# dwani-ai/tts-indic-server-f5

Hardware: AMD Instinct MI355X
Metric: mel-frames/sec + RTF, F5-TTS-Base 32-NFE, 10s utterance (higher is better)
Workload: dtype fp16/bf16 MFMA, fp32 accumulate

## Files before the change

include/f5hip.h:

```cpp
#ifndef F5HIP_H
#define F5HIP_H

#include <stdint.h>

#ifdef __cplusplus
extern "C" {
#endif

#define F5HIP_ABI_VERSION 1

int f5hip_abi_version(void);
const char* f5hip_last_error(void);


typedef struct f5hip_dit_config {
    int32_t dim, depth, heads, ff_mult, text_dim, conv_layers, mel_dim, text_num_embeds;
    int32_t gemm_planes;
    int32_t arch;
} f5hip_dit_config;

typedef struct f5hip_dit f5hip_dit;

f5hip_dit* f5hip_dit_create(const f5hip_dit_config* cfg);
void f5hip_dit_destroy(f5hip_dit* m);

int f5hip_dit_load_param(f5hip_dit* m, const char* name, const float* data, int64_t numel);
int f5hip_dit_finalize(f5hip_dit* m);

int f5hip_dit_forward(f5hip_dit* m, int32_t n_seq, const int32_t* seq_len, const int32_t* kv_len,
                      const float* x_dev, const float* cond_dev, const int32_t* text, int32_t nt_max, float time,
                      const uint8_t* drop_audio_cond, const uint8_t* drop_text, int32_t n_blocks,
                      float* out_dev, float* h_out_dev, void* stream);

int f5hip_dit_read_tap(f5hip_dit* m, const char* tap, float* dst_dev, int64_t numel, void* stream);

int f5hip_cfm_sample(f5hip_dit* m, int32_t n_utt, const int32_t* dur, const float* cond_dev,
                     const uint8_t* cond_mask, const int32_t* text, int32_t nt_max, const float* y0_dev,
                     const float* t_grid, int32_t steps, float cfg_strength, float* out_dev, void* stream);

int f5hip_cfm_sample_masked(f5hip_dit* m, int32_t n_utt, const int32_t* dur, const int32_t* kv_len, const float* cond_dev,
                            const uint8_t* cond_mask, const int32_t* text, int32_t nt_max, const float* y0_dev,
                            const float* t_grid, int32_t steps, float cfg_strength, float* out_dev, void* stream);

int f5hip_cfm_sample_units(f5hip_dit* m, int32_t n_utt, const int32_t* dur, const int32_t* kv_len, const float* cond_dev,
                           const uint8_t* cond_mask, const int32_t* text, int32_t nt_max, const float* y0_dev,
                           const float* t_grid, int32_t steps, const float* cfg_strength, float* out_dev, void* stream);

int f5hip_cfm_sample_grids(f5hip_dit* m, int32_t n_utt, const int32_t* dur, const int32_t* kv_len, const float* cond_dev,
                           const uint8_t* cond_mask, const int32_t* text, int32_t nt_max, const float* y0_dev,
                           const int32_t* steps, const float* t_grids, const float* cfg_strength, float* out_dev, void* stream);

int f5hip_cfm_sample_span(f5hip_dit* m, int32_t n_utt, const int32_t* dur, const int32_t* kv_len, const float* cond_dev,
                          const uint8_t* cond_mask, const int32_t* text, int32_t nt_max, const float* y0_dev,
                          const int32_t* steps, const float* t_grids, const float* cfg_strength, const uint8_t* last,
                          float* out_dev, void* stream);

int f5hip_cfm_sample_methods(f5hip_dit* m, int32_t n_utt, const int32_t* dur, const int32_t* kv_len, const float* cond_dev,
                             const uint8_t* cond_mask, const int32_t* text, int32_t nt_max, const float* y0_dev,
                             const int32_t* steps, const float* t_grids, const float* cfg_strength,
                             const int32_t* method ,
                             const uint8_t* last ,
                             float* out_dev, void* stream);

int f5hip_dit_set_ode_method(f5hip_dit* m, int32_t method);

int f5hip_set_attention_shape_invariant(int32_t on);
int f5hip_dit_set_attention_shape_invariant(f5hip_dit* m, int32_t on);
int f5hip_dit_set_profiling(f5hip_dit* m, int32_t enabled);
int f5hip_dit_get_profile(f5hip_dit* m, const char* kernel_class, double* total_ms, int64_t* launches);
int f5hip_set_profiling(int32_t enabled);
int f5hip_get_profile(const char* kernel_class, double* total_ms, int64_t* launches);
int f5hip_get_counter(const char* name, int64_t* value);

int f5hip_op_gemm(int32_t M, int32_t N, int32_t K, const float* a_dev, const float* w_dev, const float* bias_dev, int32_t prec,
                  int32_t act, const float* mul_dev, const float* res_dev, const uint8_t* row_keep_host, float* out_dev,
                  uint16_t* out16_dev, int32_t w_copies, int32_t iters, double* avg_us, void* stream, int32_t bn);
int f5hip_op_gemm_rowmul(int32_t M, int32_t N, int32_t K, const float* a_dev, const float* w_dev, const float* bias_dev, int32_t prec,
                         const float* mul_dev, const int32_t* row_mod_host, int32_t mod_ld, int32_t n_mod_rows, const float* res_dev,
                         const uint8_t* row_keep_host, float* out_dev, void* stream, int32_t bn);
int f5hip_op_qkv(int32_t M, int32_t D, const float* a_dev, const float* w_dev, const float* bias_dev, const int32_t* row_pos,
                 int32_t prec, uint16_t* qk_dev, uint16_t* vt_dev, int32_t iters, double* avg_us, void* stream);
int f5hip_op_attention(int32_t n_seq, const int32_t* seq_len, const int32_t* kv_len, int32_t heads, const float* q_dev, const float* k_dev,
                       const float* v_dev, float* out_dev, int32_t impl, int32_t iters, double* avg_us, void* stream, int32_t shape_invariant,
                       int32_t out_format);
int f5hip_op_joint_attention(int32_t n_seq, const int32_t* x_len, const int32_t* x_kvlen, const int32_t* c_len, int32_t heads,
                             const float* q_dev, const float* k_dev, const float* v_dev, float* out_dev, void* stream, int32_t shape_invariant,
                             int32_t out_format);
int f5hip_op_layernorm(int32_t M, int32_t D, const float* x_dev, const float* scale_dev, const float* shift_dev, float gain_off, float eps,
                       int32_t rms, float* out_dev, void* stream);
int f5hip_op_layernorm_planes(int32_t M, int32_t D, const float* x_dev, const float* scale_dev, const float* shift_dev,
                              const int32_t* row_mod_host, int32_t mod_ld, int32_t n_mod_rows, float gain_off, float eps, int32_t out_format,
                              float* out_dev, void* stream);
int f5hip_op_cfg_step(int32_t method, int32_t stage, int32_t U, int32_t mel, int32_t rows, float* xout_dev, float* xbase_dev,
                      const float* pred_dev, const int32_t* urow_c_host, const int32_t* urow_u_host, float cfg, const float* cfg_frame_dev,
                      float dt, const int32_t* frame_unit_host, const float* unit_dt_host, int32_t n_units, int32_t n_act, float* k1_dev,
                      float* k2_dev, float* k3_dev, float* xs_dev, const uint8_t* final_flags_host, const float* cond_dev, float* out_dev,
                      void* stream);
int f5hip_op_cfg_mixed(int32_t U, int32_t mel, int32_t rows, float* xstate_dev, const float* pred_dev, const int32_t* urow_c_host,
                       const int32_t* urow_u_host, const float* cfg_frame_dev, const int32_t* frame_unit_host, const int32_t* unit_op_host,
                       const float* unit_dt_host, int32_t n_units, int32_t n_act, float* k1_dev, float* k2_dev, float* k3_dev, float* xs_dev,
                       void* stream);
int f5hip_op_row_tp(int32_t R, const int32_t* row_unit_host, int32_t n_units, const int32_t* unit_tp_host, int32_t* row_tp_host,
                    void* stream);
int f5hip_op_time_table(f5hip_dit* m, const float* t_host, int32_t n_t, float* sinus_dev, float* mod_dev, int32_t mod_cols, float* temb_dev,
                        void* stream);
int f5hip_op_conv1d(int32_t batch, int32_t P, int32_t T, int32_t c_in, int32_t c_out, int32_t k, int32_t dil, const float* x_dev,
                    const float* w_host, const float* bias_host, const float* res_dev, float* out_dev, int32_t prec, int32_t impl,
                    int32_t iters, double* avg_us, uint64_t* stamps_host, int32_t stamp_blocks, void* stream);
int f5hip_op_bigvgan_snake(int32_t batch, int32_t P, int32_t T, int32_t C, const float* x_dev, const float* alpha_log_dev,
                           const float* beta_log_dev, int32_t out_format, float* out_dev, int64_t out_rows, void* stream);
int f5hip_op_bigvgan_upsample(int32_t batch, int32_t P, int32_t T, int32_t c_in, int32_t c_out, int32_t r, const float* x_dev,
                              const float* w_host, const float* bias_host, float* out_dev, int32_t prec, void* stream);
int f5hip_op_bigvgan_conv_post(int32_t batch, int32_t P, int32_t T, int32_t C, const float* a_dev, const float* w_dev, int32_t variant,
                               float* wave_dev, void* stream);
int f5hip_op_conv1d_ragged(int32_t n_items, const int32_t* item_row0, const int32_t* item_rows, const int32_t* item_valid, int32_t M,
                           int32_t blk, int32_t c_in, int32_t c_out, int32_t k, int32_t dil, int32_t ups_rate, const float* x_dev,
                           const float* w_host, const float* bias_host, const float* res_dev, float* out_dev, int32_t prec, int32_t impl,
                           void* stream);
int f5hip_op_bigvgan_snake_ragged(int32_t n_items, const int32_t* item_row0, const int32_t* item_valid, int32_t scale, int32_t M, int32_t C,
                                  const float* x_dev, const float* alpha_log_dev, const float* beta_log_dev, int32_t out_format,
                                  float* out_dev, int64_t out_rows, void* stream);
int f5hip_op_bigvgan_conv_post_ragged(int32_t n_items, const int32_t* item_row0, const int32_t* item_valid, const int32_t* item_wave_off,
                                      int32_t scale, int32_t M, int32_t C, const float* a_dev, const float* w_dev, int32_t variant,
                                      float* wave_dev, int64_t wave_len, void* stream);
int f5hip_op_bigvgan_mean3(int64_t rows, int32_t C, int32_t n_in, const float* y0_dev, const float* y1_dev, const float* y2_dev, int32_t mode,
                           int32_t ldo, float* out_f32_dev, float* planes_dev, void* stream);
int f5hip_op_bigvgan_mel_rows(int32_t n, const int32_t* item_row0, const int32_t* item_frames, int32_t T, int32_t M0, int32_t C,
                              const float* mel_dev, int32_t f16, float* out_dev, void* stream);
int f5hip_op_conv_pos_embed(int32_t n_seq, const int32_t* seq_len, int32_t lead, int32_t D, const float* x_dev, const float* w1_host,
                            const float* b1_host, const float* w2_host, const float* b2_host, int32_t impl, int32_t prec, int32_t pad_nan,
                            float* out_dev, float* c1_dev, void* stream);
int f5hip_op_convnext_block(int32_t n_seq, const int32_t* seq_len, int32_t Td, const float* x_dev, const float* const* params_host,
                            int32_t pad_nan, float* out_dev, float* tap_ln_dev, float* tap_ty_dev, float* tap_grn_dev, void* stream);


typedef struct f5hip_vocos_config {
    int32_t in_channels, dim, intermediate_dim, num_layers, n_fft, hop_length;
    int32_t gemm_planes;
} f5hip_vocos_config;
typedef struct f5hip_vocos f5hip_vocos;

f5hip_vocos* f5hip_vocos_create(const f5hip_vocos_config* cfg);
void f5hip_vocos_destroy(f5hip_vocos* v);
int f5hip_vocos_load_param(f5hip_vocos* v, const char* name, const float* data, int64_t numel);
int f5hip_vocos_finalize(f5hip_vocos* v);
int f5hip_vocos_decode(f5hip_vocos* v, int32_t batch, int32_t frames, const float* mel_dev, float* wave_dev,
                       void* stream);
int f5hip_vocos_decode_ragged(f5hip_vocos* v, int32_t n, const int32_t* frames, const float* mel_dev, float* wave_dev,
                              void* stream);
int f5hip_vocos_decode_taps(f5hip_vocos* v, int32_t n, const int32_t* frames, const float* mel_dev, int32_t n_blocks,
                            float* x_dev, float* y_dev, float* fw_dev, float* wave_dev, void* stream);


typedef struct f5hip_bigvgan_config {
    int32_t num_mels, num_upsamples;
    int32_t upsample_rates[8], upsample_kernel_sizes[8];
    int32_t upsample_initial_channel;
    int32_t resblock_kernel_sizes[3];
    int32_t resblock_dilations[9];
    int32_t gemm_planes;
} f5hip_bigvgan_config;
typedef struct f5hip_bigvgan f5hip_bigvgan;

f5hip_bigvgan* f5hip_bigvgan_create(const f5hip_bigvgan_config* cfg);
void f5hip_bigvgan_destroy(f5hip_bigvgan* v);
int f5hip_bigvgan_load_param(f5hip_bigvgan* v, const char* name, const float* data, int64_t numel);
int f5hip_bigvgan_finalize(f5hip_bigvgan* v);
int f5hip_bigvgan_forward(f5hip_bigvgan* v, int32_t batch, int32_t frames, const float* mel_dev, float* wave_dev, void* stream);
int f5hip_bigvgan_forward_ragged(f5hip_bigvgan* v, int32_t n, const int32_t* frames, const float* mel_dev, float* wave_dev,
                                 void* stream);


int f5hip_mel_spectrogram(int32_t batch, int32_t n_samples, const float* wave_dev, float* mel_dev, int32_t n_fft,
                          int32_t hop_length, int32_t n_mels, int32_t sample_rate, void* stream);

int f5hip_mel_spectrogram_bigvgan(int32_t batch, int32_t n_samples, const float* wave_dev, float* mel_dev, int32_t n_fft,
                                  int32_t hop_length, int32_t n_mels, int32_t sample_rate, void* stream);

int f5hip_mel_spectrogram_ragged(int32_t n, const int32_t* n_samples, const float* const* wave_dev, float* mel_dev, int32_t n_fft, int32_t hop_length,
                                 int32_t n_mels, int32_t sample_rate, int32_t variant, void* stream);


int f5hip_ref_frontend(int32_t n, const int32_t* n_in, const int32_t* channels, const float* wave_dev, int32_t orig_freq, int32_t new_freq,
                       const float* taps_dev, float rms_floor, float* out_dev, float* rms_dev, void* stream);


int f5hip_wave_finish(int32_t n, const int32_t* chunks_per_request, const float* const* chunk_dev, const int32_t* chunk_len, int32_t fade,
                      const uint8_t* remove_silence, int32_t sample_rate, int16_t* pcm_dev, int32_t* len_dev, void* stream);

int f5hip_wave_finish_joins(int32_t n, const int32_t* chunks_per_request, const float* const* chunk_dev, const int32_t* chunk_len, int32_t fade,
                            const uint8_t* chunk_fade, const uint8_t* remove_silence, int32_t sample_rate, int16_t* pcm_dev, int32_t* len_dev,
                            void* stream);

int f5hip_wave_encode(int32_t n, const int16_t* pcm_dev, const int64_t* in_off, const int32_t* max_len, const int32_t* len_dev, int32_t new_freq,
                      int32_t encoding, const float* taps_dev, uint8_t* out_dev, const int64_t* out_off, int32_t* out_len_dev, void* stream);

int f5hip_wave_encode_tile(int32_t new_freq);

int f5hip_wave_flac(int32_t n, const int16_t* pcm_dev, const int64_t* in_off, const int32_t* max_len, const int32_t* len_dev, int32_t sample_rate,
                    uint8_t* out_dev, const int64_t* out_off, int32_t* out_len_dev, void* stream);

int f5hip_wave_flac_levels(int32_t n, const int16_t* pcm_dev, const int64_t* in_off, const int32_t* max_len, const int32_t* len_dev,
                           int32_t sample_rate, const int32_t* level, uint8_t* out_dev, const int64_t* out_off, int32_t* out_len_dev, void* stream);

int64_t f5hip_wave_flac_bound(int32_t max_len);

int f5hip_wave_loudness(int32_t n, int16_t* pcm_dev, const int64_t* in_off, const int32_t* max_len, const int32_t* len_dev, const double* gain_k,
                        int64_t* stats_dev, void* stream);

int f5hip_wave_loudness_tile(void);

int f5hip_wave_prosody(int32_t n, const int16_t* pcm_dev, const int64_t* in_off, const int32_t* max_len, const int32_t* len_dev,
                       const int32_t* stretch_p, const int32_t* stretch_q, const int32_t* pitch, const float* taps_dev, int16_t* out_dev,
                       const int64_t* out_off, int32_t* out_len_dev, void* stream);

int64_t f5hip_wave_prosody_tap_offset(int32_t pitch);

int f5hip_flac_decode(int32_t n, const uint8_t* data_dev, int64_t nbytes, const int64_t* begin, const int64_t* end, const int32_t* info,
                      const int64_t* total, const int64_t* max_samples, int32_t* out_dev, const int64_t* out_off, int32_t* status_dev, void* stream);

int64_t f5hip_flac_decode_bound(int64_t total, int64_t stream_bytes, int64_t max_samples);

int f5hip_ref_prestep(int32_t n, const int32_t* n_in, const int32_t* channels, const uint8_t* clip_short, const int16_t* frames_dev, int64_t n_samples,
                      int32_t rate, float* out_dev, int32_t* info_dev, void* stream);

int64_t f5hip_ref_prestep_bound(int32_t n, const int32_t* n_in, const int32_t* channels, int32_t rate);

int f5hip_ref_denoise(int32_t n, const int64_t* offset, const int32_t* n_samples, float* wave_dev, void* stream);

int f5hip_wave_mark(int32_t n, int16_t* pcm_dev, const int64_t* in_off, const int32_t* max_len, const int32_t* len_dev, const int32_t* key_index,
                    const int16_t* carriers_dev, int32_t n_keys, void* stream);

int f5hip_wave_mark_tile(void);

int f5hip_watermark_carrier(uint64_t key, int16_t* carrier);

int f5hip_watermark_detect(int32_t n, const float* wave_dev, const int64_t* offset, const int32_t* n_samples, int32_t n_keys,
                           const int16_t* carriers_dev, float* scores_dev, void* stream);

int f5hip_watermark_detect_launches(void);

int f5hip_ref_assess(int32_t n, const float* raw_dev, const int64_t* raw_offset, const int32_t* channels, const int32_t* raw_len,
                     const float* wave_dev, const int64_t* offset, const int32_t* n_samples, int64_t* rows_dev, void* stream);

int f5hip_ref_assess_launches(void);

#ifdef __cplusplus
}
#endif
#endif
```

tts-indic-server-f5_amd/_lib.py:

```python
from __future__ import annotations

import ctypes as C
import os

HERE = os.path.dirname(os.path.abspath(__file__))
LIB_PATH = os.environ.get("F5HIP_LIB") or os.path.join(HERE, "csrc", "libf5hip.so")

_lib = None


class DitConfig(C.Structure):
    _fields_ = [(n, C.c_int32) for n in ("dim", "depth", "heads", "ff_mult", "text_dim", "conv_layers", "mel_dim",
                                          "text_num_embeds", "gemm_planes", "arch")]


class VocosConfig(C.Structure):
    _fields_ = [(n, C.c_int32) for n in ("in_channels", "dim", "intermediate_dim", "num_layers", "n_fft", "hop_length",
                                          "gemm_planes")]


class BigVGANConfig(C.Structure):
    _fields_ = [("num_mels", C.c_int32), ("num_upsamples", C.c_int32), ("upsample_rates", C.c_int32 * 8),
                ("upsample_kernel_sizes", C.c_int32 * 8), ("upsample_initial_channel", C.c_int32),
                ("resblock_kernel_sizes", C.c_int32 * 3), ("resblock_dilations", C.c_int32 * 9), ("gemm_planes", C.c_int32)]


SYMBOLS = {
    "f5hip_abi_version": (C.c_int, []),
    "f5hip_last_error": (C.c_char_p, []),
    "f5hip_dit_create": (C.c_void_p, [C.POINTER(DitConfig)]),
    "f5hip_dit_destroy": (None, [C.c_void_p]),
    "f5hip_dit_load_param": (C.c_int, [C.c_void_p, C.c_char_p, C.c_void_p, C.c_int64]),
    "f5hip_dit_finalize": (C.c_int, [C.c_void_p]),
    "f5hip_dit_forward": (C.c_int, [C.c_void_p, C.c_int32, C.c_void_p, C.c_void_p, C.c_void_p, C.c_void_p, C.c_void_p,
                                    C.c_int32, C.c_float, C.c_void_p, C.c_void_p, C.c_int32, C.c_void_p, C.c_void_p,
                                    C.c_void_p]),
    "f5hip_dit_read_tap": (C.c_int, [C.c_void_p, C.c_char_p, C.c_void_p, C.c_int64, C.c_void_p]),
    "f5hip_cfm_sample": (C.c_int, [C.c_void_p, C.c_int32, C.c_void_p, C.c_void_p, C.c_void_p, C.c_void_p, C.c_int32,
                                   C.c_void_p, C.c_void_p, C.c_int32, C.c_float, C.c_void_p, C.c_void_p]),
    "f5hip_cfm_sample_masked": (C.c_int, [C.c_void_p, C.c_int32, C.c_void_p, C.c_void_p, C.c_void_p, C.c_void_p, C.c_void_p, C.c_int32,
                                          C.c_void_p, C.c_void_p, C.c_int32, C.c_float, C.c_void_p, C.c_void_p]),
    "f5hip_cfm_sample_units": (C.c_int, [C.c_void_p, C.c_int32, C.c_void_p, C.c_void_p, C.c_void_p, C.c_void_p, C.c_void_p, C.c_int32,
                                         C.c_void_p, C.c_void_p, C.c_int32, C.c_void_p, C.c_void_p, C.c_void_p]),
    "f5hip_cfm_sample_grids": (C.c_int, [C.c_void_p, C.c_int32, C.c_void_p, C.c_void_p, C.c_void_p, C.c_void_p, C.c_void_p, C.c_int32,
                                         C.c_void_p, C.c_void_p, C.c_void_p, C.c_void_p, C.c_void_p, C.c_void_p]),
    "f5hip_cfm_sample_span": (C.c_int, [C.c_void_p, C.c_int32, C.c_void_p, C.c_void_p, C.c_void_p, C.c_void_p, C.c_void_p, C.c_int32,
                                        C.c_void_p, C.c_void_p, C.c_void_p, C.c_void_p, C.c_void_p, C.c_void_p, C.c_void_p]),
    "f5hip_cfm_sample_methods": (C.c_int, [C.c_void_p, C.c_int32, C.c_void_p, C.c_void_p, C.c_void_p, C.c_void_p, C.c_void_p, C.c_int32,
                                           C.c_void_p, C.c_void_p, C.c_void_p, C.c_void_p, C.c_void_p, C.c_void_p, C.c_void_p, C.c_void_p]),
    "f5hip_dit_set_ode_method": (C.c_int, [C.c_void_p, C.c_int32]),
    "f5hip_dit_set_attention_shape_invariant": (C.c_int, [C.c_void_p, C.c_int32]),
    "f5hip_dit_set_profiling": (C.c_int, [C.c_void_p, C.c_int32]),
    "f5hip_dit_get_profile": (C.c_int, [C.c_void_p, C.c_char_p, C.POINTER(C.c_double), C.POINTER(C.c_int64)]),
    "f5hip_set_profiling": (C.c_int, [C.c_int32]),
    "f5hip_set_attention_shape_invariant": (C.c_int, [C.c_int32]),
    "f5hip_get_profile": (C.c_int, [C.c_char_p, C.POINTER(C.c_double), C.POINTER(C.c_int64)]),
    "f5hip_get_counter": (C.c_int, [C.c_char_p, C.POINTER(C.c_int64)]),
    "f5hip_op_gemm": (C.c_int, [C.c_int32, C.c_int32, C.c_int32, C.c_void_p, C.c_void_p, C.c_void_p, C.c_int32, C.c_int32, C.c_void_p, C.c_void_p,
                                C.c_void_p, C.c_void_p, C.c_void_p, C.c_int32, C.c_int32, C.POINTER(C.c_double), C.c_void_p, C.c_int32]),
    "f5hip_op_qkv": (C.c_int, [C.c_int32, C.c_int32, C.c_void_p, C.c_void_p, C.c_void_p, C.c_void_p, C.c_int32, C.c_void_p, C.c_void_p, C.c_int32,
                               C.POINTER(C.c_double), C.c_void_p]),
    "f5hip_op_attention": (C.c_int, [C.c_int32, C.c_void_p, C.c_void_p, C.c_int32, C.c_void_p, C.c_void_p, C.c_void_p, C.c_void_p, C.c_int32, C.c_int32,
                                     C.POINTER(C.c_double), C.c_void_p, C.c_int32, C.c_int32]),
    "f5hip_op_layernorm": (C.c_int, [C.c_int32, C.c_int32, C.c_void_p, C.c_void_p, C.c_void_p, C.c_float, C.c_float, C.c_int32, C.c_void_p, C.c_void_p]),
    "f5hip_op_gemm_rowmul": (C.c_int, [C.c_int32] * 3 + [C.c_void_p] * 3 + [C.c_int32, C.c_void_p, C.c_void_p, C.c_int32, C.c_int32] + [C.c_void_p] * 4 +
                             [C.c_int32]),
    "f5hip_op_layernorm_planes": (C.c_int, [C.c_int32, C.c_int32] + [C.c_void_p] * 4 + [C.c_int32, C.c_int32, C.c_float, C.c_float, C.c_int32, C.c_void_p,
                                            C.c_void_p]),
    "f5hip_op_cfg_step": (C.c_int, [C.c_int32] * 5 + [C.c_void_p] * 5 + [C.c_float, C.c_void_p, C.c_float, C.c_void_p, C.c_void_p, C.c_int32, C.c_int32] +
                          [C.c_void_p] * 8),
    "f5hip_op_cfg_mixed": (C.c_int, [C.c_int32] * 3 + [C.c_void_p] * 8 + [C.c_int32, C.c_int32] + [C.c_void_p] * 5),
    "f5hip_op_row_tp": (C.c_int, [C.c_int32, C.c_void_p, C.c_int32, C.c_void_p, C.c_void_p, C.c_void_p]),
    "f5hip_op_time_table": (C.c_int, [C.c_void_p, C.c_void_p, C.c_int32, C.c_void_p, C.c_void_p, C.c_int32, C.c_void_p, C.c_void_p]),
    "f5hip_op_joint_attention": (C.c_int, [C.c_int32, C.c_void_p, C.c_void_p, C.c_void_p, C.c_int32, C.c_void_p, C.c_void_p, C.c_void_p, C.c_void_p, C.c_void_p,
                                           C.c_int32, C.c_int32]),
    "f5hip_op_conv1d": (C.c_int, [C.c_int32] * 7 + [C.c_void_p] * 5 + [C.c_int32] * 3 + [C.c_void_p, C.c_void_p, C.c_int32, C.c_void_p]),
    "f5hip_op_bigvgan_snake": (C.c_int, [C.c_int32] * 4 + [C.c_void_p] * 3 + [C.c_int32, C.c_void_p, C.c_int64, C.c_void_p]),
    "f5hip_op_bigvgan_upsample": (C.c_int, [C.c_int32] * 6 + [C.c_void_p] * 4 + [C.c_int32, C.c_void_p]),
    "f5hip_op_bigvgan_conv_post": (C.c_int, [C.c_int32] * 4 + [C.c_void_p] * 2 + [C.c_int32, C.c_void_p, C.c_void_p]),
    "f5hip_op_conv1d_ragged": (C.c_int, [C.c_int32] + [C.c_void_p] * 3 + [C.c_int32] * 7 + [C.c_void_p] * 5 + [C.c_int32, C.c_int32, C.c_void_p]),
    "f5hip_op_bigvgan_snake_ragged": (C.c_int, [C.c_int32, C.c_void_p, C.c_void_p] + [C.c_int32] * 3 + [C.c_void_p] * 3 +
                                      [C.c_int32, C.c_void_p, C.c_int64, C.c_void_p]),
    "f5hip_op_bigvgan_conv_post_ragged": (C.c_int, [C.c_int32] + [C.c_void_p] * 3 + [C.c_int32] * 3 + [C.c_void_p] * 2 +
                                          [C.c_int32, C.c_void_p, C.c_int64, C.c_void_p]),
    "f5hip_op_bigvgan_mean3": (C.c_int, [C.c_int64, C.c_int32, C.c_int32] + [C.c_void_p] * 3 + [C.c_int32, C.c_int32] + [C.c_void_p] * 3),
    "f5hip_op_bigvgan_mel_rows": (C.c_int, [C.c_int32, C.c_void_p, C.c_void_p] + [C.c_int32] * 3 + [C.c_void_p, C.c_int32, C.c_void_p, C.c_void_p]),
    "f5hip_op_conv_pos_embed": (C.c_int, [C.c_int32, C.c_void_p, C.c_int32, C.c_int32] + [C.c_void_p] * 5 + [C.c_int32] * 3 + [C.c_void_p] * 3),
    "f5hip_op_convnext_block": (C.c_int, [C.c_int32, C.c_void_p, C.c_int32, C.c_void_p, C.c_void_p, C.c_int32] + [C.c_void_p] * 5),
    "f5hip_vocos_create": (C.c_void_p, [C.POINTER(VocosConfig)]),
    "f5hip_vocos_destroy": (None, [C.c_void_p]),
    "f5hip_vocos_load_param": (C.c_int, [C.c_void_p, C.c_char_p, C.c_void_p, C.c_int64]),
    "f5hip_vocos_finalize": (C.c_int, [C.c_void_p]),
    "f5hip_vocos_decode": (C.c_int, [C.c_void_p, C.c_int32, C.c_int32, C.c_void_p, C.c_void_p, C.c_void_p]),
    "f5hip_vocos_decode_ragged": (C.c_int, [C.c_void_p, C.c_int32, C.c_void_p, C.c_void_p, C.c_void_p, C.c_void_p]),
    "f5hip_vocos_decode_taps": (C.c_int, [C.c_void_p, C.c_int32, C.c_void_p, C.c_void_p, C.c_int32] + [C.c_void_p] * 5),
    "f5hip_bigvgan_create": (C.c_void_p, [C.POINTER(BigVGANConfig)]),
    "f5hip_bigvgan_destroy": (None, [C.c_void_p]),
    "f5hip_bigvgan_load_param": (C.c_int, [C.c_void_p, C.c_char_p, C.c_void_p, C.c_int64]),
    "f5hip_bigvgan_finalize": (C.c_int, [C.c_void_p]),
    "f5hip_bigvgan_forward": (C.c_int, [C.c_void_p, C.c_int32, C.c_int32, C.c_void_p, C.c_void_p, C.c_void_p]),
    "f5hip_bigvgan_forward_ragged": (C.c_int, [C.c_void_p, C.c_int32, C.c_void_p, C.c_void_p, C.c_void_p, C.c_void_p]),
    "f5hip_mel_spectrogram_bigvgan": (C.c_int, [C.c_int32, C.c_int32, C.c_void_p, C.c_void_p, C.c_int32, C.c_int32, C.c_int32,
                                                C.c_int32, C.c_void_p]),
    "f5hip_mel_spectrogram_ragged": (C.c_int, [C.c_int32, C.c_void_p, C.c_void_p, C.c_void_p, C.c_int32, C.c_int32, C.c_int32, C.c_int32, C.c_int32,
                                               C.c_void_p]),
    "f5hip_mel_spectrogram": (C.c_int, [C.c_int32, C.c_int32, C.c_void_p, C.c_void_p, C.c_int32, C.c_int32, C.c_int32,
                                        C.c_int32, C.c_void_p]),
    "f5hip_ref_frontend": (C.c_int, [C.c_int32, C.c_void_p, C.c_void_p, C.c_void_p, C.c_int32, C.c_int32, C.c_void_p, C.c_float, C.c_void_p, C.c_void_p,
                                     C.c_void_p]),
    "f5hip_wave_finish": (C.c_int, [C.c_int32, C.c_void_p, C.c_void_p, C.c_void_p, C.c_int32, C.c_void_p, C.c_int32, C.c_void_p, C.c_void_p, C.c_void_p]),
    "f5hip_wave_finish_joins": (C.c_int, [C.c_int32, C.c_void_p, C.c_void_p, C.c_void_p, C.c_int32, C.c_void_p, C.c_void_p, C.c_int32, C.c_void_p, C.c_void_p,
                                          C.c_void_p]),
    "f5hip_wave_encode": (C.c_int, [C.c_int32, C.c_void_p, C.c_void_p, C.c_void_p, C.c_void_p, C.c_int32, C.c_int32, C.c_void_p, C.c_void_p, C.c_void_p,
                                    C.c_void_p, C.c_void_p]),
    "f5hip_wave_encode_tile": (C.c_int, [C.c_int32]),
    "f5hip_wave_flac": (C.c_int, [C.c_int32, C.c_void_p, C.c_void_p, C.c_void_p, C.c_void_p, C.c_int32, C.c_void_p, C.c_void_p, C.c_void_p, C.c_void_p]),
    "f5hip_wave_flac_levels": (C.c_int, [C.c_int32, C.c_void_p, C.c_void_p, C.c_void_p, C.c_void_p, C.c_int32, C.c_void_p, C.c_void_p, C.c_void_p, C.c_void_p,
                                         C.c_void_p]),
    "f5hip_wave_flac_bound": (C.c_int64, [C.c_int32]),
    "f5hip_wave_loudness": (C.c_int, [C.c_int32, C.c_void_p, C.c_void_p, C.c_void_p, C.c_void_p, C.c_void_p, C.c_void_p, C.c_void_p]),
    "f5hip_wave_loudness_tile": (C.c_int, []),
    "f5hip_wave_prosody": (C.c_int, [C.c_int32] + [C.c_void_p] * 12),
    "f5hip_wave_prosody_tap_offset": (C.c_int64, [C.c_int32]),
    "f5hip_flac_decode": (C.c_int, [C.c_int32, C.c_void_p, C.c_int64] + [C.c_void_p] * 9),
    "f5hip_flac_decode_bound": (C.c_int64, [C.c_int64, C.c_int64, C.c_int64]),
    "f5hip_ref_prestep": (C.c_int, [C.c_int32, C.c_void_p, C.c_void_p, C.c_void_p, C.c_void_p, C.c_int64, C.c_int32, C.c_void_p, C.c_void_p, C.c_void_p]),
    "f5hip_ref_prestep_bound": (C.c_int64, [C.c_int32, C.c_void_p, C.c_void_p, C.c_int32]),
    "f5hip_ref_denoise": (C.c_int, [C.c_int32, C.c_void_p, C.c_void_p, C.c_void_p, C.c_void_p]),
    "f5hip_wave_mark": (C.c_int, [C.c_int32, C.c_void_p, C.c_void_p, C.c_void_p, C.c_void_p, C.c_void_p, C.c_void_p, C.c_int32, C.c_void_p]),
    "f5hip_wave_mark_tile": (C.c_int, []),
    "f5hip_watermark_carrier": (C.c_int, [C.c_uint64, C.c_void_p]),
    "f5hip_watermark_detect": (C.c_int, [C.c_int32, C.c_void_p, C.c_void_p, C.c_void_p, C.c_int32, C.c_void_p, C.c_void_p, C.c_void_p]),
    "f5hip_watermark_detect_launches": (C.c_int, []),
    "f5hip_ref_assess": (C.c_int, [C.c_int32, C.c_void_p, C.c_void_p, C.c_void_p, C.c_void_p, C.c_void_p, C.c_void_p, C.c_void_p, C.c_void_p, C.c_void_p]),
    "f5hip_ref_assess_launches": (C.c_int, []),
}


class F5HipError(RuntimeError):
    pass


def lib():
    global _lib
    if _lib is None:
        if not os.path.exists(LIB_PATH):
            raise F5HipError(f"{LIB_PATH} is missing: run `python -c 'import __graft_entry__ as g; g.build()'` "
                             "(this package has no CPU fallback)")
        import torch
        l = C.CDLL(LIB_PATH)
        for name, (res, args) in SYMBOLS.items():
            fn = getattr(l, name)
            fn.restype = res
            fn.argtypes = args
        if l.f5hip_abi_version() != 1:
            raise F5HipError("libf5hip ABI version mismatch")
        _lib = l
    return _lib


def check(rc: int, what: str):
    if rc != 0:
        raise F5HipError(f"{what} failed ({rc}): {lib().f5hip_last_error().decode(errors='replace')}")


def current_stream_ptr():
    import torch
    return C.c_void_p(torch.cuda.current_stream().cuda_stream)
```

tts-indic-server-f5_amd/csrc/cfm_sample.h:

```cpp
#pragma once

struct OdeRule { const char* name; int forwards, points; };
static const OdeRule kOdeRules[3] = {{"euler", 1, 1}, {"midpoint", 2, 2}, {"rk4", 4, 3}};

static void stage_times(int method, float t0, float t1, float t[4]) {
#pragma clang fp contract(off)
    const float dt = t1 - t0;
    t[0] = t0;
    if (method == 1) t[1] = t0 + 0.5f * dt;
    if (method == 2) { t[1] = t0 + dt * (1.0f / 3.0f); t[2] = t0 + dt * (2.0f / 3.0f); t[3] = t1; }
}

struct SampleArgs {
    int32_t n_utt; const int32_t *dur, *kv_len; const float* cond_dev; const uint8_t* cond_mask; const int32_t* text; int32_t nt_max;
    const float* y0_dev; float* out_dev; void* stream;
    const uint8_t* last = nullptr;
    bool ok() const { return n_utt > 0 && dur && cond_dev && cond_mask && text && y0_dev && out_dev; }
};

struct UnitLayout {
    std::vector<SeqDesc> seqs;
    std::vector<float> frame_cfg;
    std::vector<int> frame_unit;
    std::vector<uint8_t> frame_final;
// ... 34 lines not shown
            L.seq_unit.push_back(k);
            m->h_seq_len.push_back(a.dur[u]);
        }
        L.seq_end[k] = (int)L.seqs.size();
    }
    return 0;
}

struct TimePlan {
    int forwards = 0, cols = 1;
    std::vector<float> pts, dt;
    std::vector<int> tp, op;
};

static int unit_forwards(const int32_t* steps, const int32_t* method, int u) { return steps[u] * kOdeRules[method[u]].forwards; }

static int plan_times(const std::vector<int>& order, const int32_t* steps, const int32_t* method, const float* t_grid, bool per_unit, TimePlan& P) {
    static const int kFirstOp[3] = {CFG_OP_EULER, CFG_OP_MID_HALF, CFG_OP_RK4_1};
    const int n = (int)order.size();
    bool mixed = false;
    for (int u = 0; u < n; u++) mixed = mixed || method[u] != method[0];
    if (!per_unit) {
        const OdeRule& rule = kOdeRules[method[0]];
        const int end_pt = rule.forwards > rule.points ? 1 : 0;
        if ((long long)steps[0] * rule.points + end_pt > kMaxGridPoints) {
            if (method[0] == 0) return fail(-8, "at most %d time points per call (got %d)", kMaxGridPoints, steps[0]);
            return fail(-8, "%s: at most %d steps per call (got %d)", rule.name, (kMaxGridPoints - end_pt) / rule.points, steps[0]);
        }
    }
    std::map<uint32_t, int> pt_index;
    auto point = [&](float v) {
        uint32_t bits;
        memcpy(&bits, &v, sizeof(bits));
        auto it = pt_index.find(bits);
        if (it != pt_index.end()) return it->second;
        pt_index[bits] = (int)P.pts.size();
        P.pts.push_back(v);
        return (int)P.pts.size() - 1;
    };
    P.cols = per_unit ? n : 1;
    P.forwards = unit_forwards(steps, method, order[0]);
    const size_t cells = (size_t)P.forwards * P.cols;
    P.tp.assign(cells, 0);
    P.op.assign(cells, CFG_OP_NONE);
    P.dt.assign(cells, 0.0f);
    std::vector<size_t> grid0(n, 0);
    for (int u = 1; per_unit && u < n; u++) grid0[u] = grid0[u - 1] + (size_t)steps[u - 1] + 1;
    float t[4];
    for (int k = 0; k < P.cols; k++) {
        const int u = order[k], mu = method[u];
        const OdeRule& rule = kOdeRules[mu];
        const float* tg = t_grid + grid0[u];
        for (int i = 0; i < steps[u]; i++) {
            const float dt = tg[i + 1] - tg[i];
            stage_times(mu, tg[i], tg[i + 1], t);
            for (int s = 0; s < rule.forwards; s++) {
                const size_t at = ((size_t)i * rule.forwards + s) * P.cols + k;
                if (per_unit) P.tp[at] = point(t[s]);
                else {
                    if (s < rule.points) P.pts.push_back(t[s]);
                    P.tp[at] = i * rule.points + s;
                }
                P.op[at] = kFirstOp[mu] + s;
                P.dt[at] = mu == 1 && s == 0 ? 0.5f * dt : dt;
            }
        }
        if (!per_unit && rule.forwards > rule.points) P.pts.push_back(tg[steps[u]]);
    }
    if ((int)P.pts.size() > kMaxTimePoints)
        return fail(-8, "%s: the units' grids need %d distinct time points, at most %d per call", mixed ? "cfm_sample_methods" : "cfm_sample_grids",
                    (int)P.pts.size(), kMaxTimePoints);
    return 0;
}

struct GridLayout {
    size_t row_unit, frame_unit, tp, op, dt, row_tp, total = 0;
    GridLayout(size_t R, size_t U, size_t cells) {
        auto take = [&](size_t n) { const size_t at = total; total += n; return at; };
        row_unit = take(R); frame_unit = take(U); tp = take(cells); op = take(cells); dt = take(cells); row_tp = take(R);
    }
};
struct GridTables { const int *row_unit = nullptr, *frame_unit = nullptr, *tp = nullptr, *op = nullptr; const float* dt = nullptr; int* row_tp = nullptr; };

static int upload_grid_tables(f5hip_dit* m, const UnitLayout& L, const TimePlan& P, hipStream_t st, GridTables& T) {
    const int R = m->Rtot, S = (int)L.seqs.size();
    const GridLayout g(R, L.n_frames, P.tp.size());
    if (g.total > m->grid_cap) {
        dev_free(m->grid_meta);
        m->grid_cap = 0;
        if (hipMalloc((void**)&m->grid_meta, sizeof(int) * g.total) != hipSuccess) { m->grid_meta = nullptr; return fail(-5, "hipMalloc grid tables"); }
        m->grid_cap = g.total;
    }
    std::vector<int> hb(g.row_tp, 0);
    for (int s = 0; s < S; s++) {
        for (int r = m->h_seq_row0[s]; r < m->h_seq_row0[s + 1]; r++) hb[g.row_unit + r] = L.seq_unit[s];
        for (int r = m->h_seqc_row0[s]; r < m->h_seqc_row0[s + 1]; r++) hb[g.row_unit + r] = L.seq_unit[s];
    }
    memcpy(&hb[g.frame_unit], L.frame_unit.data(), sizeof(int) * L.frame_unit.size());
    memcpy(&hb[g.tp], P.tp.data(), sizeof(int) * P.tp.size());
    memcpy(&hb[g.op], P.op.data(), sizeof(int) * P.op.size());
    memcpy(&hb[g.dt], P.dt.data(), sizeof(float) * P.dt.size());
    CK(m->up_grid.upload(m->grid_meta, hb.data(), sizeof(int) * hb.size(), st));
    int* const d = m->grid_meta;
    T = {d + g.row_unit, d + g.frame_unit, d + g.tp, d + g.op, reinterpret_cast<const float*>(d + g.dt), d + g.row_tp};
    return 0;
}

struct CfgBufs {
    float *xstate, *k1, *k2, *k3;
    const float* pred;
    const int *urow_c, *urow_u;
    const float* frame_cfg;
    Plane2 xs;
    int mel;
};
static CfgBufs cfg_bufs(const f5hip_dit* m) {
    return {m->xstate, m->xmid, m->rk_k2, m->rk_k3, m->pred, m->d_urow_c, m->d_urow_u, m->d_frame_cfg, m->xs, m->cfg.mel_dim};
}

static void launch_cfg_step(const CfgBufs& b, int f0, int op, float dt, const int* frame_unit, const int* unit_op, const float* unit_dt, int n_act,
                            hipStream_t st) {
    auto* kernel = frame_unit ? cfg_step_kernel<true> : cfg_step_kernel<false>;
    hipLaunchKernelGGL(kernel, dim3(f0), dim3(128), 0, st, b.xstate, b.mel, f0, b.pred, 128, b.urow_c, b.urow_u, b.frame_cfg, op, dt, b.k1, b.k2, b.k3,
                       b.xs.hi, b.xs.lo, 128, frame_unit, unit_op, unit_dt, n_act);
}

struct GridScope {
    f5hip_dit* m;
    ~GridScope() { m->d_row_tp = nullptr; m->M = m->row_c0; m->Mc = m->Rtot - m->row_c0; m->n_seq = (int)m->h_seq_row0.size() - 1; }
};

static int run_sampler(f5hip_dit* m, const SampleArgs& a, const int32_t* steps, const int32_t* method, const float* t_grid, bool per_unit,
                       float cfg_strength, const float* cfg_unit) {
    const int n = a.n_utt;
    std::vector<int> order(n);
    for (int u = 0; u < n; u++) order[u] = u;
    std::stable_sort(order.begin(), order.end(), [&](int x, int y) { return unit_forwards(steps, method, x) > unit_forwards(steps, method, y); });
    ProfScope prof_scope(m->prof);
    hipStream_t st = (hipStream_t)a.stream;
    UnitLayout L;
    TimePlan P;
    CK(layout_units(m, a, order, cfg_strength, cfg_unit, L));
    CK(plan_times(order, steps, method, t_grid, per_unit, P));
    const int mel = m->cfg.mel_dim, U = L.n_frames;
    CK(setup_sequences(m, L.seqs, U, a.text, a.nt_max, a.cond_mask, st, L.frame_cfg.data(), a.last ? L.frame_final.data() : nullptr));
    GridScope scope{m};
    GridTables T;
    if (per_unit) CK(upload_grid_tables(m, L, P, st, T));

    if (hipMemcpyAsync(m->xstate, a.y0_dev, sizeof(float) * (size_t)U * mel, hipMemcpyDeviceToDevice, st) != hipSuccess) return fail(-6, "y0 copy");
    hipLaunchKernelGGL(split_rows_kernel, dim3(m->M), dim3(256), 0, st, m->xstate, mel, mel, m->M, m->d_row_frame, m->xs.hi, m->xs.lo, 128, 0);
    CKL("split x");
    CK(precompute_text_and_ce(m, a.cond_dev, st));
    CK(precompute_time(m, P.pts.data(), (int)P.pts.size(), st));

    m->d_row_tp = T.row_tp;
    int n_act = n;
    for (int f = 0; f < P.forwards; f++) {
        const size_t at = (size_t)f * P.cols;
        if (per_unit) {
            while (P.op[at + n_act - 1] == CFG_OP_NONE) n_act--;
            const int s_act = L.seq_end[n_act - 1];
            m->M = m->h_seq_row0[s_act]; m->Mc = m->h_seqc_row0[s_act] - m->row_c0; m->n_seq = s_act;
            prof_begin(PROF_OTHER, st);
            hipLaunchKernelGGL(row_tp_kernel, dim3((m->Rtot + 255) / 256), dim3(256), 0, st, T.row_unit, T.tp + at, m->Rtot, T.row_tp);
            prof_end(PROF_OTHER, st);
            CKL("row_tp");
        }
        CK(forward_step(m, per_unit ? 0 : P.tp[at], -1, st));
        prof_begin(PROF_OTHER, st);
        launch_cfg_step(cfg_bufs(m), U, P.op[at], P.dt[at], T.frame_unit, per_unit ? T.op + at : nullptr, per_unit ? T.dt + at : nullptr, n_act, st);
        prof_end(PROF_OTHER, st);
        CKL("cfg step");
    }
    hipLaunchKernelGGL(final_select_kernel, dim3(U), dim3(128), 0, st, m->xstate, a.cond_dev, m->d_frame_is_cond, mel, U, a.out_dev);
    CKL("final_select");
    return 0;
}

static int sample_one_grid(f5hip_dit* m, const SampleArgs& a, int method, const float* t_grid, int32_t steps, float cfg_strength, const float* cfg_unit) {
    if (!m || !m->finalized) return fail(-1, "model not finalized");
    if (!a.ok() || !t_grid || steps <= 0) return fail(-1, "cfm_sample: bad argument");
    const std::vector<int32_t> unit_steps(a.n_utt, steps), unit_method(a.n_utt, method);
    return run_sampler(m, a, unit_steps.data(), unit_method.data(), t_grid, false, cfg_strength, cfg_unit);
}

int f5hip_cfm_sample(f5hip_dit* m, int32_t n_utt, const int32_t* dur, const float* cond_dev, const uint8_t* cond_mask,
                     const int32_t* text, int32_t nt_max, const float* y0_dev, const float* t_grid, int32_t steps,
                     float cfg_strength, float* out_dev, void* stream) {
    return sample_one_grid(m, {n_utt, dur, nullptr, cond_dev, cond_mask, text, nt_max, y0_dev, out_dev, stream}, m ? m->ode_method : 0, t_grid, steps, cfg_strength, nullptr);
}

int f5hip_cfm_sample_masked(f5hip_dit* m, int32_t n_utt, const int32_t* dur, const int32_t* kv_len, const float* cond_dev, const uint8_t* cond_mask,
                            const int32_t* text, int32_t nt_max, const float* y0_dev, const float* t_grid, int32_t steps,
                            float cfg_strength, float* out_dev, void* stream) {
    return sample_one_grid(m, {n_utt, dur, kv_len, cond_dev, cond_mask, text, nt_max, y0_dev, out_dev, stream}, m ? m->ode_method : 0, t_grid, steps, cfg_strength, nullptr);
}

int f5hip_cfm_sample_units(f5hip_dit* m, int32_t n_utt, const int32_t* dur, const int32_t* kv_len, const float* cond_dev, const uint8_t* cond_mask,
                           const int32_t* text, int32_t nt_max, const float* y0_dev, const float* t_grid, int32_t steps,
                           const float* cfg_strength, float* out_dev, void* stream) {
    if (!cfg_strength) return fail(-1, "cfm_sample_units: cfg_strength is null");
    return sample_one_grid(m, {n_utt, dur, kv_len, cond_dev, cond_mask, text, nt_max, y0_dev, out_dev, stream}, m ? m->ode_method : 0, t_grid, steps, 0.0f, cfg_strength);
}

static int sample_grids(const char* name, f5hip_dit* m, const SampleArgs& a, const int32_t* steps, const float* t_grids, const float* cfg_strength,
                        const int32_t* unit_method) {
    if (!m || !m->finalized) return fail(-1, "model not finalized");
    if (!a.ok() || !steps || !t_grids || !cfg_strength) return fail(-1, "%s: bad argument", name);
    const std::vector<int32_t> handle_method(a.n_utt, m->ode_method);
    const int32_t* method = unit_method ? unit_method : handle_method.data();
    bool one = true;
    size_t g0 = 0;
    for (int u = 0; u < a.n_utt; u++) {
        if (method[u] < 0 || method[u] > 2) return fail(-1, "%s: method[%d] = %d (0 euler, 1 midpoint, 2 rk4)", name, u, method[u]);
        one = one && method[u] == method[0];
    }
    for (int u = 0; u < a.n_utt; u++) {
        if (steps[u] < 1) return fail(-1, "%s: steps[%d] = %d (need >= 1)", name, u, steps[u]);
        one = one && steps[u] == steps[0] && !memcmp(t_grids + g0, t_grids, sizeof(float) * ((size_t)steps[0] + 1));
        g0 += (size_t)steps[u] + 1;
    }
    if (one) return sample_one_grid(m, a, method[0], t_grids, steps[0], 0.0f, cfg_strength);
    return run_sampler(m, a, steps, method, t_grids, true, 0.0f, cfg_strength);
}

int f5hip_cfm_sample_grids(f5hip_dit* m, int32_t n_utt, const int32_t* dur, const int32_t* kv_len, const float* cond_dev, const uint8_t* cond_mask,
                           const int32_t* text, int32_t nt_max, const float* y0_dev, const int32_t* steps, const float* t_grids,
                           const float* cfg_strength, float* out_dev, void* stream) {
    return sample_grids("cfm_sample_grids", m, {n_utt, dur, kv_len, cond_dev, cond_mask, text, nt_max, y0_dev, out_dev, stream}, steps, t_grids, cfg_strength, nullptr);
}

int f5hip_cfm_sample_span(f5hip_dit* m, int32_t n_utt, const int32_t* dur, const int32_t* kv_len, const float* cond_dev, const uint8_t* cond_mask,
                          const int32_t* text, int32_t nt_max, const float* y0_dev, const int32_t* steps, const float* t_grids,
                          const float* cfg_strength, const uint8_t* last, float* out_dev, void* stream) {
    if (!last) return fail(-1, "cfm_sample_span: last is null");
    return sample_grids("cfm_sample_span", m, {n_utt, dur, kv_len, cond_dev, cond_mask, text, nt_max, y0_dev, out_dev, stream, last}, steps, t_grids, cfg_strength, nullptr);
}

int f5hip_cfm_sample_methods(f5hip_dit* m, int32_t n_utt, const int32_t* dur, const int32_t* kv_len, const float* cond_dev, const uint8_t* cond_mask,
                             const int32_t* text, int32_t nt_max, const float* y0_dev, const int32_t* steps, const float* t_grids,
                             const float* cfg_strength, const int32_t* method, const uint8_t* last, float* out_dev, void* stream) {
    if (!method) return fail(-1, "cfm_sample_methods: method is null");
    return sample_grids("cfm_sample_methods", m, {n_utt, dur, kv_len, cond_dev, cond_mask, text, nt_max, y0_dev, out_dev, stream, last}, steps, t_grids,
                        cfg_strength, method);
}
```

tts-indic-server-f5_amd/csrc/elementwise.h:

```cpp
#pragma once
#include "common.h"

#include "ln_row.h"

template <int NV, bool ROW_MOD = false>
__global__ __launch_bounds__(256) void ln_kernel(const LnArgs p) {
    unsigned b = blockIdx.x;
    if ((gridDim.x & 7) == 0) b = (b & 7) * (gridDim.x >> 3) + (b >> 3);
    ln_row<NV, ROW_MOD>(p, b * 4 + (threadIdx.x >> 6), threadIdx.x & 63);
}

__global__ __launch_bounds__(256) void row_tp_kernel(const int* row_unit, const int* unit_tp, int R, int* row_tp) {
    const int r = blockIdx.x * 256 + threadIdx.x;
    if (r < R) row_tp[r] = unit_tp[row_unit[r]];
}

__global__ __launch_bounds__(256) void rope_rows_kernel(const int* row_pos, const float* rope_cos, const float* rope_sin, int R, int max_pos, float* out_cos, float* out_sin) {
    const int i = blockIdx.x * 256 + threadIdx.x;
    if (i >= R * 32) return;
    const int r = i >> 5, j = i & 31;
    const int pos = min(max(row_pos[r], 0), max_pos - 1);
    out_cos[i] = rope_cos[pos * 32 + j];
    out_sin[i] = rope_sin[pos * 32 + j];
}

__global__ __launch_bounds__(256) void grn_stats_kernel(const float* y, int ldy, int C, const int* seq_row0,
                                                        const int* seq_len, float* gx ) {
    const int seq = blockIdx.y, c = blockIdx.x * 256 + threadIdx.x;
    if (c >= C) return;
    const int r0 = seq_row0[seq], n = seq_len[seq];
    float a8[8] = {0.f, 0.f, 0.f, 0.f, 0.f, 0.f, 0.f, 0.f};
    const float* col = y + (size_t)r0 * ldy + c;
    int r = 0;
    for (; r + 8 <= n; r += 8) {
        float t[8];
#pragma unroll
        for (int u = 0; u < 8; u++) t[u] = col[(size_t)(r + u) * ldy];
#pragma unroll
        for (int u = 0; u < 8; u++) a8[u] += t[u] * t[u];
    }
    for (; r < n; r++) {
        const float t = col[(size_t)r * ldy];
        a8[0] += t * t;
    }
    const float acc = ((a8[0] + a8[1]) + (a8[2] + a8[3])) + ((a8[4] + a8[5]) + (a8[6] + a8[7]));
    gx[(size_t)seq * C + c] = sqrtf(acc);
}

__global__ __launch_bounds__(256) void grn_apply_kernel(const float* y, int ldy, int C, int M, const int* row_seq,
                                                        const float* gx, const float* gamma, const float* beta,
                                                        __bf16* out_hi, __bf16* out_lo, int ldo) {
    const int lane = threadIdx.x & 63;
    const int row = blockIdx.x * 4 + (threadIdx.x >> 6);
    if (row >= M) return;
    const int seq = row_seq[row];
    if (seq < 0) return;
    const float* g = gx + (size_t)seq * C;
    float s = 0.0f;
    for (int c = lane; c < C; c += 64) s += g[c];
    const float denom = wave_sum(s) / (float)C + 1e-6f;
    for (int c = lane * 4; c < C; c += 256) {
        const float4 yv = *reinterpret_cast<const float4*>(y + (size_t)row * ldy + c);
        const float yy[4] = {yv.x, yv.y, yv.z, yv.w};
        bf16x4 hi, lo;
        float ov[4];
#pragma unroll
        for (int e = 0; e < 4; e++) {
            const float nx = g[c + e] / denom;
            ov[e] = gamma[c + e] * (yy[e] * nx) + beta[c + e] + yy[e];
        }
        split_bf16x4(ov, hi, lo);
        *reinterpret_cast<bf16x4*>(out_hi + (size_t)row * ldo + c) = hi;
        if (out_lo) *reinterpret_cast<bf16x4*>(out_lo + (size_t)row * ldo + c) = lo;
    }
}

__global__ __launch_bounds__(256) void text_gather_kernel(const float* emb, const float* pos_table, int C, int M,
                                                          const int* row_token, const int* row_pos, int add_pos,
                                                          float* out, int ldo, int max_pos) {
    const int row = blockIdx.x;
    if (row >= M) return;
    const int tok = row_token[row];
    if (tok < 0) return;
    const int pos = min(row_pos[row], max_pos);
    for (int c = threadIdx.x; c < C; c += 256) {
        float v = emb[(size_t)tok * C + c];
        if (add_pos) v += pos_table[(size_t)pos * C + c];
        out[(size_t)row * ldo + c] = v;
    }
}

__global__ __launch_bounds__(256) void split_rows_kernel(const float* x, int ldx, int C, int M, const int* row_src,
                                                         __bf16* out_hi, __bf16* out_lo, int ldo, int col0) {
    const int row = blockIdx.x;
    if (row >= M) return;
    const int src = row_src ? row_src[row] : row;
    for (int c = threadIdx.x; c < C; c += 256) {
        __bf16 hi, lo;
        const float v = src >= 0 ? x[(size_t)src * ldx + c] : 0.0f;
        split_bf16(v, hi, lo);
        out_hi[(size_t)row * ldo + col0 + c] = hi;
        if (out_lo) out_lo[(size_t)row * ldo + col0 + c] = lo;
    }
}

enum CfgOp : int {
    CFG_OP_NONE = 0,
    CFG_OP_EULER = 1,
    CFG_OP_MID_HALF = 2,
    CFG_OP_MID_FULL = 3,
    CFG_OP_RK4_1 = 4,
    CFG_OP_COUNT = 8
};

__device__ __forceinline__ float cfg_velocity(const float* pred, int ldp, int rc, int ru, int c, float cfg) {
    const float pc = pred[(size_t)rc * ldp + c];
    float v = pc;
    if (ru >= 0) v = pc + (pc - pred[(size_t)ru * ldp + c]) * cfg;
    return v;
}

__device__ __forceinline__ float euler_update(float* xout, const float* xbase, size_t i, float dt, float v) {
    const float xn = xbase[i] + dt * v;
    xout[i] = xn;
    return xn;
}

__device__ __forceinline__ float rk4_stage_update(float* xstate, float* k1, float* k2, float* k3, size_t i, int stage, float dt, float v) {
    const float y0 = xstate[i];
    float xn;
    if (stage == 1) {
        k1[i] = v;
        xn = y0 + dt * v * (1.0f / 3.0f);
    } else if (stage == 2) {
        k2[i] = v;
        xn = y0 + dt * (v - k1[i] * (1.0f / 3.0f));
    } else if (stage == 3) {
        k3[i] = v;
        xn = y0 + dt * (k1[i] - k2[i] + v);
    } else {
        xn = y0 + (k1[i] + 3.0f * (k2[i] + k3[i]) + v) * dt * 0.125f;
        xstate[i] = xn;
    }
    return xn;
}

__device__ __forceinline__ void store_x_split(__bf16* xs_hi, __bf16* xs_lo, int ldx, int rc, int ru, int c, float xn) {
    __bf16 hi, lo;
    split_bf16(xn, hi, lo);
    xs_hi[(size_t)rc * ldx + c] = hi;
    xs_lo[(size_t)rc * ldx + c] = lo;
    if (ru >= 0) {
        xs_hi[(size_t)ru * ldx + c] = hi;
        xs_lo[(size_t)ru * ldx + c] = lo;
    }
}

template <bool kPerUnit>
__global__ __launch_bounds__(128) void cfg_step_kernel(float* xstate , int mel, int U, const float* pred, int ldp, const int* urow_c,
                                                       const int* urow_u, const float* cfg_frame, int op, float dt, float* k1, float* k2, float* k3,
                                                       __bf16* xs_hi, __bf16* xs_lo, int ldx, const int* frame_unit, const int* unit_op,
                                                       const float* unit_dt, int n_act) {
    const int u = blockIdx.x;
    if (u >= U) return;
    const int c = threadIdx.x;
    if (c >= mel) return;
    if (kPerUnit) {
        const int un = frame_unit[u];
        if (un >= n_act) return;
        op = unit_op[un];
        dt = unit_dt[un];
    }
    if (op <= CFG_OP_NONE || op >= CFG_OP_COUNT) return;
    const int rc = urow_c[u], ru = urow_u[u];
    const float v = cfg_velocity(pred, ldp, rc, ru, c, cfg_frame[u]);
    const size_t i = (size_t)u * mel + c;
    float xn;
    if (op >= CFG_OP_RK4_1) xn = rk4_stage_update(xstate, k1, k2, k3, i, op - CFG_OP_RK4_1 + 1, dt, v);
    else xn = euler_update(op == CFG_OP_MID_HALF ? k1 : xstate, xstate, i, dt, v);
    store_x_split(xs_hi, xs_lo, ldx, rc, ru, c, xn);
}

__global__ __launch_bounds__(128) void final_select_kernel(const float* xstate, const float* cond, const int* frame_is_cond,
                                                           int mel, int U, float* out) {
    const int u = blockIdx.x, c = threadIdx.x;
    if (u >= U || c >= mel) return;
    out[(size_t)u * mel + c] = frame_is_cond[u] ? cond[(size_t)u * mel + c] : xstate[(size_t)u * mel + c];
}

__global__ __launch_bounds__(256) void pack_weight_kernel(const float* w, int R, int C, int ldw, __bf16* hi, __bf16* lo,
                                                          int C_pad) {
    const int r = blockIdx.x;
    for (int c = threadIdx.x; c < C_pad; c += 256) {
        float v = (r < R && c < C) ? w[(size_t)r * ldw + c] : 0.0f;
        if (!lo) {
            reinterpret_cast<_Float16*>(hi)[(size_t)r * C_pad + c] = sat_f16(v);
            continue;
        }
        __bf16 h, l;
// ... 37 lines not shown
```

tts-indic-server-f5_amd/csrc/f5hip.hip:

```cpp
#include "../../include/f5hip.h"

#include <math.h>
#include <stdio.h>
#include <stdlib.h>
#include <string.h>

#include <map>
#include <string>
#include <algorithm>
#include <vector>

#include "common.h"
#include "elementwise.h"
#include "gemm_launch.h"
#include "host_util.h"

static constexpr int kMaxTimePoints = 256;
static constexpr int kMaxGridPoints = 128;
static_assert(kMaxGridPoints <= kMaxTimePoints, "a one-grid call's points are rows of the same tables");


struct TextBlock {
    float *dw_w = nullptr, *dw_b = nullptr, *ln_w = nullptr, *ln_b = nullptr, *gamma = nullptr, *beta = nullptr;
    PackedW pw1, pw2;
};

struct BlockWeights {
    std::vector<PackedW> qkv, out, ff1, ff2;
    void resize(int n) { qkv.resize(n); out.resize(n); ff1.resize(n); ff2.resize(n); }
};

struct f5hip_dit {
    f5hip_dit_config cfg;
    int nsplit = 2;
    int attn_invariant = -1;
    ProfState* prof = nullptr;
    HostStage up_meta, up_time[2], up_grid;
    bool blk_f16 = false;
    ParamStore params;
    bool finalized = false;
    PackedW time1, time2, adaln, wx, wct, conv1, conv2, proj_out;
    BlockWeights blk;
    BlockWeights blk_c;
    std::vector<PackedW> wskip;
    std::vector<int> mod_c, mod_x;
    int mod_final = 0;
    std::vector<float*> g_attn, g_ff;
    float *g_out = nullptr, *zeros = nullptr;
    std::vector<TextBlock> tblk;
    float *text_emb = nullptr, *text_pos = nullptr, *rope_cos = nullptr, *rope_sin = nullptr;
    float *rope_row_cos = nullptr, *rope_row_sin = nullptr;
    int rope_max_pos = 0;
    int arch = 0;
    int td_pad = 0;
    int gw = 0;
    int n_adaln = 0;
    int cap_rows = 0, cap_frames = 0, cap_seq = 0;
    DevBuf ws;
    float *h = nullptr, *h0 = nullptr, *ce = nullptr, *pred = nullptr, *te = nullptr, *ty = nullptr, *gx = nullptr,
          *mod = nullptr, *xstate = nullptr, *xmid = nullptr, *temb = nullptr, *rk_k2 = nullptr, *rk_k3 = nullptr;
    int ode_method = 0;
    std::vector<Plane2> skipbuf;
    Plane2 hn, c1, ao, ff, xs, tn, tg, act, sinp, t1, st;
    __bf16 *qk = nullptr, *vt = nullptr;
    int *meta = nullptr;
    int meta_cap = 0;
    int *d_row_pos, *d_row_start, *d_row_end, *d_row_seq, *d_row_token, *d_row_frame, *d_row_condframe, *d_row_keep,
        *d_seq_row0, *d_seq_len, *d_seq_kvlen, *d_urow_c, *d_urow_u, *d_frame_is_cond;
    float* d_frame_cfg = nullptr;
    int M = 0, n_seq = 0, n_frames = 0, max_len = 0;
    int Mc = 0, Rtot = 0;
    int row_c0 = 0;
    std::vector<int> h_seq_row0, h_seqc_row0;
    int* d_row_tp = nullptr;
    int* grid_meta = nullptr;
    size_t grid_cap = 0;
    int *d_j_row0 = nullptr, *d_j_len = nullptr, *d_j_kvlen = nullptr, *d_j_kv_row0 = nullptr, *d_j_kv2_row0 = nullptr, *d_j_kv2_len = nullptr;
    bool any_masked = false;
    std::vector<int> h_seq_len;
};

static int ceil_to(int v, int m) { return (v + m - 1) / m * m; }

f5hip_dit* f5hip_dit_create(const f5hip_dit_config* cfg) {
    if (!cfg) { set_error("null config"); return nullptr; }
    if (cfg->dim % 128 || cfg->dim != cfg->heads * 64 || cfg->dim % 16 || cfg->text_dim % 4 || cfg->mel_dim > 128 || cfg->mel_dim % 4 ||
        cfg->dim / 16 > 64 || cfg->gemm_planes < 1 || cfg->gemm_planes > 3 || cfg->arch < 0 || cfg->arch > 2 ||
        (cfg->arch == 1 && (cfg->conv_layers != 0 || cfg->depth % 2)) || (cfg->conv_layers > 0 && cfg->text_dim % 32) ||
        (cfg->arch == 2 && (cfg->conv_layers != 0 || cfg->text_dim != cfg->dim || cfg->depth < 1))) {
        set_error("unsupported backbone geometry (need dim %% 128 == 0, dim == 64*heads, dim/16 <= 64, mel_dim <= 128, text conv needs text_dim %% 32 == 0; UNetT: even depth, no text conv)");
        return nullptr;
    }
    int dev_count = 0;
    if (hipGetDeviceCount(&dev_count) != hipSuccess || dev_count == 0) {
        set_error("no HIP device: libf5hip has no CPU fallback");
        return nullptr;
    }
    f5hip_dit* m = new f5hip_dit();
    m->cfg = *cfg;
    m->nsplit = cfg->gemm_planes == 3 ? 2 : cfg->gemm_planes;
    m->blk_f16 = cfg->gemm_planes == 3;
    m->arch = cfg->arch;
    m->td_pad = cfg->arch == 2 ? 0 : ceil_to(cfg->text_dim, 32);
    m->gw = cfg->dim / 16;
    if (cfg->arch != 1) {
        int off = 0;
        for (int l = 0; l < cfg->depth; l++) {
            if (cfg->arch == 2) { m->mod_c.push_back(off); off += (l == cfg->depth - 1 ? 2 : 6) * cfg->dim; }
            m->mod_x.push_back(off); off += 6 * cfg->dim;
        }
        m->mod_final = off;
        m->n_adaln = off + 2 * cfg->dim;
    }
    return m;
}

static void free_packed(PackedW& w) { dev_free(w.hi); dev_free(w.lo); dev_free(w.bias); dev_free(w.frag); w = PackedW(); }

void f5hip_dit_destroy(f5hip_dit* m) {
    if (!m) return;
    for (PackedW* w : {&m->time1, &m->time2, &m->adaln, &m->wx, &m->wct, &m->conv1, &m->conv2, &m->proj_out}) free_packed(*w);
    for (BlockWeights* b : {&m->blk, &m->blk_c})
        for (auto* v : {&b->qkv, &b->out, &b->ff1, &b->ff2}) for (auto& w : *v) free_packed(w);
    for (auto& w : m->wskip) free_packed(w);
    for (auto* v : {&m->g_attn, &m->g_ff}) for (float* g : *v) dev_free(g);
    dev_free(m->g_out); dev_free(m->zeros);
    for (auto& b : m->tblk) {
        for (float* p : {b.dw_w, b.dw_b, b.ln_w, b.ln_b, b.gamma, b.beta}) dev_free(p);
        free_packed(b.pw1); free_packed(b.pw2);
    }
    for (float* p : {m->text_emb, m->text_pos, m->rope_cos, m->rope_sin}) dev_free(p);
    dev_free(m->ws.ptr);
    dev_free(m->meta);
    delete m->prof;
    dev_free(m->grid_meta);
    m->up_meta.release(); m->up_time[0].release(); m->up_time[1].release(); m->up_grid.release();
    delete m;
}

int f5hip_dit_load_param(f5hip_dit* m, const char* name, const float* data, int64_t numel) {
    return m ? m->params.load(m->finalized, name, data, numel) : fail(-1, "load_param: bad argument");
}

#define CK(x) do { int _r = (x); if (_r) return _r; } while (0)
#define CKL(name) do { hipError_t _e = hipGetLastError(); if (_e != hipSuccess) return fail(-7, "%s launch: %s", name, hipGetErrorString(_e)); } while (0)

static int pack_conv_pos(PackedW& out, const float* w, const float* b, int D) {
    const int gw = D / 16, K = 31 * 64;
    std::vector<float> wp((size_t)16 * 64 * K, 0.0f), bp(16 * 64, 0.0f);
    for (int g = 0; g < 16; g++)
        for (int co = 0; co < gw; co++) {
            bp[g * 64 + co] = b[g * gw + co];
            for (int ci = 0; ci < gw; ci++)
                for (int tap = 0; tap < 31; tap++)
                    wp[((size_t)(g * 64 + co)) * K + tap * 64 + ci] = w[((size_t)(g * gw + co) * gw + ci) * 31 + tap];
        }
    return pack_linear(out, wp.data(), 16 * 64, K, K, bp.data());
}

static int pack_block(f5hip_dit* m, BlockWeights& w, int l, const std::string& attn, const char* qkv_sfx, const std::string& out, const std::string& ff) {
    const int D = m->cfg.dim, F = m->cfg.ff_mult * D;
    const ParamStore& P = m->params;
    std::vector<float> wq((size_t)3 * D * D), bq(3 * D);
    const char* nm[3] = {"to_q", "to_k", "to_v"};
    for (int i = 0; i < 3; i++) {
        GET_PARAM(wi, P, attn + nm[i] + qkv_sfx + ".weight", (int64_t)D * D);
        GET_PARAM(bi, P, attn + nm[i] + qkv_sfx + ".bias", D);
        memcpy(&wq[(size_t)i * D * D], wi->data(), sizeof(float) * D * D);
        memcpy(&bq[(size_t)i * D], bi->data(), sizeof(float) * D);
    }
    if (pack_linear(w.qkv[l], wq.data(), 3 * D, D, D, bq.data(), 128, m->blk_f16) || pack_frag(w.qkv[l])) return -4;
    if (out.empty()) return 0;
    GET_PARAM(wo, P, out + ".weight", (int64_t)D * D); GET_PARAM(bo, P, out + ".bias", D);
    if (pack_linear(w.out[l], wo->data(), D, D, D, bo->data(), 128, m->blk_f16)) return -4;
    GET_PARAM(w1, P, ff + "ff.0.0.weight", (int64_t)F * D); GET_PARAM(b1, P, ff + "ff.0.0.bias", F);
    if (pack_linear(w.ff1[l], w1->data(), F, D, D, b1->data(), 128, m->blk_f16) || pack_frag(w.ff1[l])) return -4;
    GET_PARAM(w2, P, ff + "ff.2.weight", (int64_t)D * F); GET_PARAM(b2, P, ff + "ff.2.bias", D);
    if (pack_linear(w.ff2[l], w2->data(), D, F, F, b2->data(), 128, m->blk_f16)) return -4;
    return 0;
}

static void rope_tables(std::vector<float>& rc, std::vector<float>& rs) {
    rc.resize((size_t)4097 * 32); rs.resize((size_t)4097 * 32);
    for (int pos = 0; pos < 4097; pos++)
        for (int i = 0; i < 32; i++) {
            float inv = 1.0f / powf(10000.0f, (float)(2 * i) / 64.0f);
            float ang = (float)pos * inv;
            rc[(size_t)pos * 32 + i] = (float)cos((double)ang);
            rs[(size_t)pos * 32 + i] = (float)sin((double)ang);
        }
}

int f5hip_dit_finalize(f5hip_dit* m) {
    if (!m) return fail(-1, "null model");
    if (m->finalized) return 0;
    const f5hip_dit_config& c = m->cfg;
    const ParamStore& P = m->params;
    const int D = c.dim, Td = c.text_dim, mel = c.mel_dim;
    const std::string T = "transformer.";
    {
        GET_PARAM(w0, P, T + "time_embed.time_mlp.0.weight", (int64_t)D * 256);
        GET_PARAM(b0, P, T + "time_embed.time_mlp.0.bias", D);
        GET_PARAM(w2, P, T + "time_embed.time_mlp.2.weight", (int64_t)D * D);
        GET_PARAM(b2, P, T + "time_embed.time_mlp.2.bias", D);
        if (pack_linear(m->time1, w0->data(), D, 256, 256, b0->data())) return -4;
        if (pack_linear(m->time2, w2->data(), D, D, D, b2->data())) return -4;
    }
    if (m->arch != 1) {
        std::vector<float> wa((size_t)m->n_adaln * D), ba(m->n_adaln);
        auto put = [&](int off, const std::string& name, int rows) {
            const std::vector<float>* w = P.get(name + "weight", (int64_t)rows * D);
            const std::vector<float>* b = w ? P.get(name + "bias", rows) : nullptr;
            if (!b) return false;
            memcpy(&wa[(size_t)off * D], w->data(), sizeof(float) * (size_t)rows * D);
            memcpy(&ba[off], b->data(), sizeof(float) * rows);
            return true;
        };
        for (int l = 0; l < c.depth; l++) {
            const std::string p = T + "transformer_blocks." + std::to_string(l) + ".";
            if (m->arch == 2 && !put(m->mod_c[l], p + "attn_norm_c.linear.", (l == c.depth - 1 ? 2 : 6) * D)) return -3;
            if (!put(m->mod_x[l], p + (m->arch == 2 ? "attn_norm_x.linear." : "attn_norm.linear."), 6 * D)) return -3;
        }
        if (!put(m->mod_final, T + "norm_out.linear.", 2 * D)) return -3;
        if (pack_linear(m->adaln, wa.data(), m->n_adaln, D, D, ba.data())) return -4;
    }
    {
        GET_PARAM(e, P, T + "text_embed.text_embed.weight", (int64_t)(c.text_num_embeds + 1) * Td);
        if (upload_f32(&m->text_emb, e->data(), e->size())) return -4;
        std::vector<float> tab((size_t)4096 * Td);
        for (int pos = 0; pos < 4096; pos++)
            for (int j = 0; j < Td / 2; j++) {
                float w = 1.0f / powf(10000.0f, (float)(2 * j) / (float)Td);
                float ang = (float)pos * w;
                tab[(size_t)pos * Td + j] = (float)cos((double)ang);
                tab[(size_t)pos * Td + Td / 2 + j] = (float)sin((double)ang);
            }
        if (upload_f32(&m->text_pos, tab.data(), tab.size())) return -4;
        m->tblk.resize(c.conv_layers);
        for (int i = 0; i < c.conv_layers; i++) {
            std::string p = T + "text_embed.text_blocks." + std::to_string(i) + ".";
            TextBlock& b = m->tblk[i];
            GET_PARAM(dw, P, p + "dwconv.weight", (int64_t)Td * 7); GET_PARAM(db, P, p + "dwconv.bias", Td);
            GET_PARAM(lw, P, p + "norm.weight", Td); GET_PARAM(lb, P, p + "norm.bias", Td);
            GET_PARAM(w1, P, p + "pwconv1.weight", (int64_t)2 * Td * Td); GET_PARAM(b1, P, p + "pwconv1.bias", 2 * Td);
            GET_PARAM(gg, P, p + "grn.gamma", 2 * Td); GET_PARAM(gb, P, p + "grn.beta", 2 * Td);
            GET_PARAM(w2, P, p + "pwconv2.weight", (int64_t)2 * Td * Td); GET_PARAM(b2, P, p + "pwconv2.bias", Td);
            if (upload_f32(&b.dw_w, dw->data(), dw->size()) || upload_f32(&b.dw_b, db->data(), db->size()) ||
                upload_f32(&b.ln_w, lw->data(), lw->size()) || upload_f32(&b.ln_b, lb->data(), lb->size()) ||
                upload_f32(&b.gamma, gg->data(), gg->size()) || upload_f32(&b.beta, gb->data(), gb->size())) return -4;
            if (pack_linear(b.pw1, w1->data(), 2 * Td, Td, Td, b1->data())) return -4;
            if (pack_linear(b.pw2, w2->data(), Td, 2 * Td, 2 * Td, b2->data())) return -4;
        }
    }
    {
        const bool mm = m->arch == 2;
        const int Kin = 2 * mel + (mm ? 0 : Td);
        GET_PARAM(w, P, T + (mm ? "audio_embed.linear.weight" : "input_embed.proj.weight"), (int64_t)D * Kin);
        GET_PARAM(b, P, T + (mm ? "audio_embed.linear.bias" : "input_embed.proj.bias"), D);
        const int Kct = 128 + m->td_pad;
        std::vector<float> wx((size_t)D * 128, 0.0f), wct((size_t)D * Kct, 0.0f);
        for (int n = 0; n < D; n++) {
            for (int k = 0; k < mel; k++) {
                wx[(size_t)n * 128 + k] = (*w)[(size_t)n * Kin + k];
                wct[(size_t)n * Kct + k] = (*w)[(size_t)n * Kin + mel + k];
            }
            for (int k = 0; k < (mm ? 0 : Td); k++) wct[(size_t)n * Kct + 128 + k] = (*w)[(size_t)n * Kin + 2 * mel + k];
        }
        if (pack_linear(m->wx, wx.data(), D, 128, 128, nullptr)) return -4;
        if (pack_linear(m->wct, wct.data(), D, Kct, Kct, b->data())) return -4;
    }
    for (int which = 0; which < 2; which++) {
        std::string p = T + (m->arch == 2 ? "audio_embed" : "input_embed") + ".conv_pos_embed.conv1d." + std::to_string(which * 2) + ".";
        GET_PARAM(w, P, p + "weight", (int64_t)D * m->gw * 31);
        GET_PARAM(b, P, p + "bias", D);
        if (pack_conv_pos(which ? m->conv2 : m->conv1, w->data(), b->data(), D)) return -4;
    }
    m->blk.resize(c.depth);
    if (m->arch == 2) m->blk_c.resize(c.depth);
    if (m->arch == 1) { m->wskip.resize(c.depth); m->g_attn.assign(c.depth, nullptr); m->g_ff.assign(c.depth, nullptr); }
    for (int l = 0; l < c.depth; l++) {
        const std::string p = T + (m->arch != 1 ? "transformer_blocks." : "layers.") + std::to_string(l) + ".";
        const std::string pa = p + (m->arch != 1 ? "attn." : "2."), pf = p + (m->arch == 0 ? "ff." : (m->arch == 2 ? "ff_x." : "4."));
        CK(pack_block(m, m->blk, l, pa, "", pa + "to_out.0", pf));
        if (m->arch == 2) CK(pack_block(m, m->blk_c, l, pa, "_c", l < c.depth - 1 ? pa + "to_out_c" : "", p + "ff_c."));
        if (m->arch == 1) {
            GET_PARAM(ga, P, p + "1.g", D); GET_PARAM(gf, P, p + "3.g", D);
            if (upload_f32(&m->g_attn[l], ga->data(), D) || upload_f32(&m->g_ff[l], gf->data(), D)) return -4;
            if (l >= c.depth / 2) {
                GET_PARAM(ws, P, p + "0.weight", (int64_t)D * 2 * D);
                if (pack_linear(m->wskip[l], ws->data(), D, 2 * D, 2 * D, nullptr)) return -4;
            }
        }
    }
    if (m->arch == 1) {
        GET_PARAM(go, P, T + "norm_out.g", D);
        if (upload_f32(&m->g_out, go->data(), D)) return -4;
    }
    {
        std::vector<float> z(std::max(D, 4096), 0.0f);
        if (upload_f32(&m->zeros, z.data(), z.size())) return -4;
    }
    {
        GET_PARAM(w, P, T + "proj_out.weight", (int64_t)mel * D); GET_PARAM(b, P, T + "proj_out.bias", mel);
        if (pack_linear(m->proj_out, w->data(), mel, D, D, b->data())) return -4;
    }
    {
        std::vector<float> rc, rs;
        rope_tables(rc, rs);
        if (upload_f32(&m->rope_cos, rc.data(), rc.size()) || upload_f32(&m->rope_sin, rs.data(), rs.size())) return -4;
    }
    const hipError_t e = hipDeviceSynchronize();
    if (e != hipSuccess) return fail(-4, "finalize: weight packing: %s", hipGetErrorString(e));
    m->params.host.clear();
    m->finalized = true;
    return 0;
}

struct MetaLayout {
    size_t row_pos, row_start, row_end, row_seq, row_token, row_frame, row_condframe, row_keep;
    size_t seq_row0, seq_len, seq_kvlen;
    size_t urow_c, urow_u, frame_is_cond;
    size_t j_row0, j_len, j_kvlen, j_kv_row0, j_kv2_row0, j_kv2_len;
    size_t frame_cfg;
    size_t total = 0;
    MetaLayout(size_t R, size_t S, size_t U, bool mmdit) {
        auto take = [&](size_t n) { const size_t at = total; total += n; return at; };
        for (size_t* o : {&row_pos, &row_start, &row_end, &row_seq, &row_token, &row_frame, &row_condframe, &row_keep}) *o = take(R);
        for (size_t* o : {&seq_row0, &seq_len, &seq_kvlen}) *o = take(S);
        for (size_t* o : {&urow_c, &urow_u, &frame_is_cond}) *o = take(U);
        for (size_t* o : {&j_row0, &j_len, &j_kvlen, &j_kv_row0, &j_kv2_row0, &j_kv2_len}) *o = take(mmdit ? 2 * S : 0);
        frame_cfg = take(U);
    }
};
static_assert(sizeof(float) == sizeof(int), "frame_cfg rides in the int arena");

static int ensure_workspace(f5hip_dit* m, int rows_pad, int frames, int n_seq) {
    if (rows_pad <= m->cap_rows && frames <= m->cap_frames && n_seq <= m->cap_seq) return 0;
    const f5hip_dit_config& c = m->cfg;
    const int D = c.dim, Td = c.text_dim, F = c.ff_mult * D;
    const size_t R = (size_t)std::max(rows_pad, m->cap_rows), U = (size_t)std::max(frames, m->cap_frames),
                 S = (size_t)std::max(n_seq, m->cap_seq);
    if (alloc_workspace(&m->ws.ptr, "workspace", [&](Arena& a) {
            m->h = a.f32(R * D); m->h0 = a.f32(R * D); m->ce = a.f32(R * D); m->pred = a.f32(R * 128);
            m->te = a.f32(R * Td); m->ty = a.f32(R * 2 * Td); m->gx = a.f32(S * 2 * Td);
            m->rope_row_cos = a.f32(R * 32); m->rope_row_sin = a.f32(R * 32);
            m->mod = a.f32((size_t)kMaxTimePoints * m->n_adaln + 64); m->xstate = a.f32(U * c.mel_dim); m->xmid = a.f32(U * c.mel_dim);
            m->temb = a.f32((size_t)kMaxTimePoints * D);
            m->hn = a.plane2(R * D + 256); m->c1 = a.plane2(R * D + 256); m->ao = a.plane2(R * D); m->ff = a.plane2(R * F);
            m->xs = a.plane2(R * 128); m->tn = a.plane2(R * Td); m->tg = a.plane2(R * 2 * Td); m->act = a.plane2(R * (128 + m->td_pad));
            m->sinp = a.plane2(kMaxTimePoints * 256); m->t1 = a.plane2((size_t)kMaxTimePoints * D); m->st = a.plane2((size_t)kMaxTimePoints * D);
            m->skipbuf.resize(m->arch == 1 ? c.depth / 2 : 0);
            for (auto& sb : m->skipbuf) sb = a.plane2(R * 2 * D);
            m->qk = a.bf16((R + 256) * 2 * D); m->vt = a.bf16((size_t)D * R);
            m->rk_k2 = a.f32(U * c.mel_dim); m->rk_k3 = a.f32(U * c.mel_dim);
        })) { m->cap_rows = 0; return -5; }
    m->cap_rows = (int)R; m->cap_frames = (int)U; m->cap_seq = (int)S;
    const int need = (int)MetaLayout(R, S, U, m->arch == 2).total;
    if (need > m->meta_cap) {
        dev_free(m->meta);
        if (hipMalloc((void**)&m->meta, sizeof(int) * need) != hipSuccess) { m->meta = nullptr; m->meta_cap = 0; return fail(-5, "hipMalloc meta"); }
        m->meta_cap = need;
    }
    return 0;
}

static int seq_rows(int len, int lead) { return ceil_to(len + lead, 128); }
static void set_seq_bounds(int* row_start, int* row_end, int* row_seq, int r0, int lead, int len, int s) {
    for (int j = 0; j < lead; j++) row_seq[r0 + j] = s;
    for (int i = 0; i < len; i++) {
        const int r = r0 + lead + i;
        row_start[r] = r0 + lead; row_end[r] = r0 + lead + len; row_seq[r] = s;
    }
}

struct SeqDesc { int len, kvlen, frame0 , text_row, drop_audio, drop_text, branch ;
                 int c_len = 0 ; };

static int setup_sequences(f5hip_dit* m, const std::vector<SeqDesc>& seqs, int n_frames, const int32_t* text, int nt_max,
                           const uint8_t* frame_is_cond, hipStream_t st, const float* frame_cfg = nullptr, const uint8_t* frame_final = nullptr) {
    const int extra = m->arch == 1 ? 1 : 0;
    const bool mm = m->arch == 2;
    int rows = 0, rows_x = 0;
    for (auto& s : seqs) rows += seq_rows(s.len, extra);
    rows_x = rows;
    if (mm) for (auto& s : seqs) {
        if (s.c_len <= 0 || s.c_len > 4096) return fail(-1, "MMDiT: a sequence needs 1..4096 text positions (got %d)", s.c_len);
        rows += seq_rows(s.c_len, 0);
    }
    if (ensure_workspace(m, rows, n_frames, (int)seqs.size())) return -5;
    const int R = rows, S = (int)seqs.size(), U = n_frames;
    const MetaLayout ml(R, S, U, mm);
    std::vector<int> hbuf(ml.total, 0);
    if (frame_cfg) memcpy(&hbuf[ml.frame_cfg], frame_cfg, sizeof(float) * U);
    int* const hb = hbuf.data();
    int* row_pos = hb + ml.row_pos; int* row_start = hb + ml.row_start; int* row_end = hb + ml.row_end; int* row_seq = hb + ml.row_seq;
    int* row_token = hb + ml.row_token; int* row_frame = hb + ml.row_frame; int* row_condframe = hb + ml.row_condframe; int* row_keep = hb + ml.row_keep;
    int* seq_row0 = hb + ml.seq_row0; int* seq_len = hb + ml.seq_len; int* seq_kvlen = hb + ml.seq_kvlen;
    int* urow_c = hb + ml.urow_c; int* urow_u = hb + ml.urow_u; int* fic = hb + ml.frame_is_cond;
    int r0 = 0;
    m->any_masked = false;
    m->h_seq_row0.assign(S + 1, 0); m->h_seqc_row0.assign(S + 1, rows_x);
    for (int r = 0; r < R; r++) { row_seq[r] = -1; row_token[r] = -1; row_frame[r] = -1; row_condframe[r] = -1; }
    for (int u = 0; u < U; u++) { urow_c[u] = -1; urow_u[u] = -1; fic[u] = frame_final ? frame_final[u] : frame_is_cond ? frame_is_cond[u] : 0; }
    m->max_len = 0;
    for (int s = 0; s < S; s++) {
        const SeqDesc& q = seqs[s];
        seq_row0[s] = r0; seq_len[s] = q.len + extra; seq_kvlen[s] = q.kvlen + extra;
        m->max_len = std::max(m->max_len, q.len + extra);
        if (q.kvlen < q.len) m->any_masked = true;
        if (extra) { row_pos[r0] = 0; row_keep[r0] = 1; }
        set_seq_bounds(row_start, row_end, row_seq, r0, extra, q.len, s);
        for (int i = 0; i < q.len; i++) {
            const int r = r0 + extra + i;
            row_pos[r] = i + extra;
            int tok = 0;
            if (!q.drop_text && i < nt_max) tok = text[(size_t)q.text_row * nt_max + i] + 1;
            if (tok < 0 || tok > m->cfg.text_num_embeds) return fail(-1, "text token %d of sequence %d is outside the vocabulary (0..%d)", tok - 1, s, m->cfg.text_num_embeds - 1);
            row_token[r] = tok;
            row_frame[r] = q.frame0 + i;
            const bool is_c = frame_is_cond ? frame_is_cond[q.frame0 + i] != 0 : true;
            row_condframe[r] = (!q.drop_audio && is_c) ? q.frame0 + i : -1;
            row_keep[r] = i < q.kvlen ? 1 : 0;
            (q.branch ? urow_u : urow_c)[q.frame0 + i] = r;
        }
        r0 += seq_rows(q.len, extra);
        m->h_seq_row0[s + 1] = r0;
    }
    if (mm) {
        int rc0 = rows_x;
        for (int s = 0; s < S; s++) {
            const SeqDesc& q = seqs[s];
            set_seq_bounds(row_start, row_end, row_seq, rc0, 0, q.c_len, s);
            for (int i = 0; i < q.c_len; i++) {
                const int r = rc0 + i;
                int tok = 0;
                if (!q.drop_text && i < nt_max) tok = text[(size_t)q.text_row * nt_max + i] + 1;
                if (tok < 0 || tok > m->cfg.text_num_embeds) return fail(-1, "text token %d of sequence %d is outside the vocabulary (0..%d)", tok - 1, s, m->cfg.text_num_embeds - 1);
                row_pos[r] = i; row_token[r] = tok; row_keep[r] = 1;
            }
            for (int qd = 0; qd < 2; qd++) {
                const int j = 2 * s + qd;
                hb[ml.j_row0 + j] = qd ? rc0 : seq_row0[s];
                hb[ml.j_len + j] = qd ? q.c_len : q.len;
                hb[ml.j_kvlen + j] = q.kvlen;
                hb[ml.j_kv_row0 + j] = seq_row0[s];
                hb[ml.j_kv2_row0 + j] = rc0;
                hb[ml.j_kv2_len + j] = q.c_len;
            }
            m->max_len = std::max(m->max_len, q.c_len);
            rc0 += seq_rows(q.c_len, 0);
            m->h_seqc_row0[s + 1] = rc0;
        }
    }
    if (const int r_ = m->up_meta.upload(m->meta, hbuf.data(), sizeof(int) * hbuf.size(), st)) return r_;
    int* const d = m->meta;
    m->d_row_pos = d + ml.row_pos; m->d_row_start = d + ml.row_start; m->d_row_end = d + ml.row_end; m->d_row_seq = d + ml.row_seq;
    m->d_row_token = d + ml.row_token; m->d_row_frame = d + ml.row_frame; m->d_row_condframe = d + ml.row_condframe; m->d_row_keep = d + ml.row_keep;
    m->d_seq_row0 = d + ml.seq_row0; m->d_seq_len = d + ml.seq_len; m->d_seq_kvlen = d + ml.seq_kvlen;
    m->d_urow_c = d + ml.urow_c; m->d_urow_u = d + ml.urow_u; m->d_frame_is_cond = d + ml.frame_is_cond;
    m->d_j_row0 = d + ml.j_row0; m->d_j_len = d + ml.j_len; m->d_j_kvlen = d + ml.j_kvlen; m->d_j_kv_row0 = d + ml.j_kv_row0;
    m->d_j_kv2_row0 = d + ml.j_kv2_row0; m->d_j_kv2_len = d + ml.j_kv2_len;
    m->d_frame_cfg = reinterpret_cast<float*>(d + ml.frame_cfg);
    hipLaunchKernelGGL(rope_rows_kernel, dim3((R * 32 + 255) / 256), dim3(256), 0, st, m->d_row_pos, m->rope_cos, m->rope_sin, R, 4097, m->rope_row_cos, m->rope_row_sin);
    if (hipGetLastError() != hipSuccess) return fail(-7, "rope_rows_kernel launch");
    m->M = rows_x; m->Mc = R - rows_x; m->Rtot = R; m->n_seq = S; m->n_frames = U; m->row_c0 = rows_x;
    return 0;
}

static Plane2 rows_from(const Plane2& p, size_t off) { return {p.hi + off, p.lo + off}; }

static GemmArgs gemm_base(const Plane2& A, int lda, const PackedW& W, int M) {
    GemmArgs a;
    memset(&a, 0, sizeof(a));
    a.A[0] = A.hi; a.A[1] = A.lo; a.lda = lda;
    a.W[0] = W.hi; a.W[1] = W.lo; a.Wf = W.frag;
    a.M = M; a.N = W.n; a.K = W.k_pad; a.ldw = W.ld;
    a.bias = W.bias;
    return a;
}

enum { CNT_GEMM5_RB11, CNT_GEMM5_RB8, CNT_GEMM5_WIDE, CNT_GEMM3_WIDE, CNT_CONV5, CNT_GEMM6, CNT_GEMM6_R176, CNT_GEMM6_R256, CNT_GEMM5_CB12,
       CNT_GEMM3, CNT_GEMM_REG_BN64, CNT_GEMM_REG_BN128, CNT_DIT_ROWS, CNT_REF_LAUNCHES, CNT_REF_TAPS_LDS, CNT_REF_TAPS_L2, CNT_WAVE_LAUNCHES,
       CNT_WAVE_REQUESTS, CNT_WAVE_ENCODE_LAUNCHES, CNT_WAVE_ENCODE_REQUESTS, CNT_MEL_RAGGED_LAUNCHES, CNT_MEL_RAGGED_ITEMS, CNT_WAVE_FLAC_LAUNCHES,
       CNT_WAVE_FLAC_REQUESTS, CNT_WAVE_LOUDNESS_LAUNCHES, CNT_WAVE_LOUDNESS_REQUESTS, CNT_FLAC_DECODE_LAUNCHES, CNT_FLAC_DECODE_STREAMS,
       CNT_REF_PRESTEP_LAUNCHES, CNT_REF_PRESTEP_CLIPS, CNT_WAVE_PROSODY_LAUNCHES, CNT_WAVE_PROSODY_REQUESTS,
       CNT_REF_DENOISE_LAUNCHES, CNT_REF_DENOISE_CLIPS, CNT_WAVE_MARK_LAUNCHES, CNT_WAVE_MARK_REQUESTS, CNT_WATERMARK_DETECT_LAUNCHES,
       CNT_WATERMARK_DETECT_CLIPS, CNT_REF_ASSESS_LAUNCHES, CNT_REF_ASSESS_CLIPS, CNT_COUNT };
static long long g_counters[CNT_COUNT] = {};

static int run_gemm_n(int nsplit, int mp, GemmArgs& a, const PackedW& W, int epi, bool conv, int bn, hipStream_t st) {
    hipError_t e;
    const int np = W.n_pad;
    if (mp % 128 || np % bn || a.K % 32) return fail(-7, "gemm: bad padded shape %d x %d x %d", mp, np, a.K);
    prof_begin(PROF_GEMM, st);
    const long long tiles128 = (long long)(mp / 128) * (np / 128);
    if (nsplit == 3 && !conv) {
        const Gemm5Choice c5 = gemm5_choose(a.M, np);
        const bool legal6 = a.K % 64 == 0 && np % 256 == 0 && (epi != EPI_QKV || a.D % 256 == 0);
        const int rows6 = legal6 ? gemm6_choose_rows(a.M, np) : 0;
        if (rows6) {
            e = f5_launch_gemm6(epi, rows6, a, np, st);
            g_counters[CNT_GEMM6]++;
            g_counters[rows6 == 176 ? CNT_GEMM6_R176 : CNT_GEMM6_R256]++;
        } else if (a.K % 64 == 0 && c5.rb) {
            e = epi == EPI_QKV ? f5_launch_gemm5_qkv(a, c5.rb, c5.cb, np, st)
              : epi == EPI_GENERIC_ROWMUL ? f5_launch_gemm5_rowmul(a, c5.rb, c5.cb, np, st) : f5_launch_gemm5_generic(a, c5.rb, c5.cb, np, st);
            g_counters[c5.rb == 11 ? CNT_GEMM5_RB11 : CNT_GEMM5_RB8]++;
            if (c5.cb >= 8) g_counters[CNT_GEMM5_WIDE]++;
            if (c5.cb == 12) g_counters[CNT_GEMM5_CB12]++;
        } else {
            const bool wide = tiles128 >= 1024 && np % 256 == 0;
            if (wide) g_counters[CNT_GEMM3_WIDE]++;
            g_counters[CNT_GEMM3]++;
            e = f5_launch_gemm3(3, epi, wide ? 256 : 128, a, mp, np, st);
        }
    } else if (!conv && tiles128 <= 256 && epi != EPI_QKV) {
        g_counters[CNT_GEMM3]++;
        e = f5_launch_gemm3(nsplit, epi, 128, a, mp, np, st);
    } else {
        g_counters[bn == 64 ? CNT_GEMM_REG_BN64 : CNT_GEMM_REG_BN128]++;
        e = f5_launch_gemm_reg(nsplit, bn, conv, epi, a, mp, np, st);
    }
    prof_end(PROF_GEMM, st);
    if (e != hipSuccess) return fail(-7, "gemm launch: %s", hipGetErrorString(e));
    return 0;
}
static int run_conv(int nsplit, GemmArgs& g, const PackedW& W, bool conv5, bool fallback, int bn, hipStream_t st) {
    if (conv5) {
        prof_begin(PROF_GEMM, st);
        const hipError_t e = f5_launch_conv5(nsplit, g, W.n_pad, st);
        prof_end(PROF_GEMM, st);
        if (e == hipSuccess) { g_counters[CNT_CONV5]++; return 0; }
        if (e != hipErrorInvalidValue || !fallback)
            return fail(-7, "conv5 launch: %s", e == hipErrorInvalidValue ? "does not cover this shape" : hipGetErrorString(e));
    }
    return run_gemm_n(nsplit, g.M, g, W, EPI_GENERIC, true, bn, st);
}
static int run_gemm(f5hip_dit* m, GemmArgs& a, const PackedW& W, int epi, bool conv, int bn, hipStream_t st, int m_pad = -1) {
    return run_gemm_n(W.f16 ? 3 : m->nsplit, m_pad > 0 ? m_pad : m->M, a, W, epi, conv, bn, st);
}

static LnArgs ln_args(const float* x, int ldx, int M, int D, const float* scale, const float* shift, float gain_off, float eps) {
    LnArgs a;
    memset(&a, 0, sizeof(a));
    a.x = x; a.ldx = ldx; a.M = M; a.D = D; a.scale = scale; a.shift = shift; a.gain_off = gain_off; a.eps = eps;
    return a;
}

template <bool ROW_MOD>
static bool launch_ln(const LnArgs& a, hipStream_t st) {
    dim3 grid((a.M + 3) / 4), blk(256);
    switch ((a.D + 255) / 256) {
        case 1: hipLaunchKernelGGL((ln_kernel<1, ROW_MOD>), grid, blk, 0, st, a); return true;
        case 2: hipLaunchKernelGGL((ln_kernel<2, ROW_MOD>), grid, blk, 0, st, a); return true;
        case 3: hipLaunchKernelGGL((ln_kernel<3, ROW_MOD>), grid, blk, 0, st, a); return true;
        case 4: hipLaunchKernelGGL((ln_kernel<4, ROW_MOD>), grid, blk, 0, st, a); return true;
        case 5: case 6: hipLaunchKernelGGL((ln_kernel<6, ROW_MOD>), grid, blk, 0, st, a); return true;
        default: return false;
    }
}

static int run_ln(const LnArgs& a, hipStream_t st, bool row_mod = false) {
    prof_begin(PROF_LN, st);
    const bool launched = row_mod ? launch_ln<true>(a, st) : launch_ln<false>(a, st);
    prof_end(PROF_LN, st);
    if (!launched) return fail(-7, "ln: D=%d unsupported", a.D);
    hipError_t e = hipGetLastError();
    if (e != hipSuccess) return fail(-7, "ln launch: %s", hipGetErrorString(e));
    return 0;
}

extern "C" int f5hip_get_counter(const char* name, int64_t* value) {
    static const char* names[CNT_COUNT] = {"gemm5_rb11", "gemm5_rb8", "gemm5_wide", "gemm3_wide", "conv5", "gemm6", "gemm6_r176", "gemm6_r256",
                                           "gemm5_cb12", "gemm3", "gemm_reg_bn64", "gemm_reg_bn128", "dit_rows", "ref_frontend_launches",
                                           "ref_taps_lds", "ref_taps_l2", "wave_finish_launches", "wave_finish_requests",
                                           "wave_encode_launches", "wave_encode_requests", "mel_ragged_launches", "mel_ragged_items",
                                           "wave_flac_launches", "wave_flac_requests", "wave_loudness_launches", "wave_loudness_requests",
                                           "flac_decode_launches", "flac_decode_streams", "ref_prestep_launches", "ref_prestep_clips",
                                           "wave_prosody_launches", "wave_prosody_requests", "ref_denoise_launches", "ref_denoise_clips",
                                           "wave_mark_launches", "wave_mark_requests", "watermark_detect_launches", "watermark_detect_clips",
                                           "ref_assess_launches", "ref_assess_clips"};
    static const char* attn_names[F5_ATTN_CNT_COUNT] = {"attn_bal8", "attn_nw8_deep", "attn_nw8", "attn_nw6_deep", "attn_nw6", "attn_nw4", "attn_seg2"};
    long long* attn = f5_attn_counters();
    if (!name) return fail(-1, "get_counter: null name");
    if (!strcmp(name, "reset")) {
        for (auto& c : g_counters) c = 0;
        for (int i = 0; i < F5_ATTN_CNT_COUNT; i++) attn[i] = 0;
        return 0;
    }
    for (int i = 0; i < CNT_COUNT; i++)
        if (!strcmp(name, names[i])) { if (value) *value = g_counters[i]; return 0; }
    for (int i = 0; i < F5_ATTN_CNT_COUNT; i++)
        if (!strcmp(name, attn_names[i])) { if (value) *value = attn[i]; return 0; }
    return fail(-1, "unknown counter %s", name);
}

static int run_text_block(int nsplit, const TextBlock& b, int Td, int M, int n_seq, float* te, const Plane2& tn, float* ty, const Plane2& tg,
                          float* gx, const int* row_start, const int* row_end, const int* row_seq, const int* seq_row0, const int* seq_len,
                          __bf16* out_hi, __bf16* out_lo, int ldob, hipStream_t st) {
    LnArgs ln = ln_args(te, Td, M, Td, b.ln_w, b.ln_b, 0.0f, 1e-6f);
    ln.dw_w = b.dw_w; ln.dw_b = b.dw_b; ln.row_seq_start = row_start; ln.row_seq_end = row_end;
    ln.out_hi = tn.hi; ln.out_lo = tn.lo; ln.ldo = Td;
    CK(run_ln(ln, st));
    GemmArgs g1 = gemm_base(tn, Td, b.pw1, M);
    g1.act = ACT_GELU_ERF; g1.out_f32 = ty; g1.ldo = 2 * Td;
    CK(run_gemm_n(b.pw1.f16 ? 3 : nsplit, M, g1, b.pw1, EPI_GENERIC, false, 128, st));
    prof_begin(PROF_OTHER, st);
    hipLaunchKernelGGL(grn_stats_kernel, dim3((2 * Td + 255) / 256, n_seq), dim3(256), 0, st, ty, 2 * Td, 2 * Td, seq_row0, seq_len, gx);
    CKL("grn_stats");
    hipLaunchKernelGGL(grn_apply_kernel, dim3((M + 3) / 4), dim3(256), 0, st, ty, 2 * Td, 2 * Td, M, row_seq, gx, b.gamma, b.beta, tg.hi, tg.lo,
                       2 * Td);
    CKL("grn_apply");
    prof_end(PROF_OTHER, st);
    GemmArgs g2 = gemm_base(tg, 2 * Td, b.pw2, M);
    g2.res = te; g2.ldres = Td; g2.out_f32 = te; g2.ldo = Td;
    if (out_hi) { g2.out_hi = out_hi; g2.out_lo = out_lo; g2.ldob = ldob; }
    return run_gemm_n(b.pw2.f16 ? 3 : nsplit, M, g2, b.pw2, EPI_GENERIC, false, 128, st);
}

static int precompute_text_and_ce(f5hip_dit* m, const float* cond_dev, hipStream_t st) {
    const f5hip_dit_config& c = m->cfg;
    const int D = c.dim, Td = c.text_dim, M = m->M, Kct = 128 + m->td_pad;
    prof_begin(PROF_OTHER, st);
    if (m->arch == 2) {
        const int C0 = m->row_c0;
        hipLaunchKernelGGL(text_gather_kernel, dim3(m->Mc), dim3(256), 0, st, m->text_emb, m->text_pos, D, m->Mc, m->d_row_token + C0,
                           m->d_row_pos + C0, 1, m->te + (size_t)C0 * D, D, 1023);
    } else {
        hipLaunchKernelGGL(text_gather_kernel, dim3(M), dim3(256), 0, st, m->text_emb, m->text_pos, Td, M, m->d_row_token,
                           m->d_row_pos, c.conv_layers > 0 ? 1 : 0, m->te, Td, 4095);
    }
    CKL("text_gather");
    hipLaunchKernelGGL(split_rows_kernel, dim3(M), dim3(256), 0, st, cond_dev, c.mel_dim, c.mel_dim, M, m->d_row_condframe,
                       m->act.hi, m->act.lo, Kct, 0);
    CKL("split cond");
    prof_end(PROF_OTHER, st);
    for (int i = 0; i < c.conv_layers; i++) {
        const bool last = i == c.conv_layers - 1;
        CK(run_text_block(m->nsplit, m->tblk[i], Td, M, m->n_seq, m->te, m->tn, m->ty, m->tg, m->gx, m->d_row_start, m->d_row_end, m->d_row_seq,
                          m->d_seq_row0, m->d_seq_len, last ? m->act.hi + 128 : nullptr, last ? m->act.lo + 128 : nullptr, Kct, st));
    }
    if (c.conv_layers == 0 && m->arch != 2) {
        prof_begin(PROF_OTHER, st);
        hipLaunchKernelGGL(split_rows_kernel, dim3(M), dim3(256), 0, st, m->te, Td, Td, M, (const int*)nullptr, m->act.hi,
                           m->act.lo, Kct, 128);
        CKL("split text");
        prof_end(PROF_OTHER, st);
    }
    GemmArgs g = gemm_base(m->act, Kct, m->wct, M);
    g.out_f32 = m->ce; g.ldo = D;
    CK(run_gemm(m, g, m->wct, EPI_GENERIC, false, 128, st));
    return 0;
}

static int precompute_time(f5hip_dit* m, const float* t_host, int n_t, hipStream_t st) {
    const f5hip_dit_config& c = m->cfg;
    const int D = c.dim;
    if (n_t > kMaxTimePoints) return fail(-8, "at most %d time points per call (got %d)", kMaxTimePoints, n_t);
    const int t_pad = ceil_to(n_t, 128);
    std::vector<uint16_t> hi((size_t)t_pad * 256, 0), lo((size_t)t_pad * 256, 0);
    const float emb = logf(10000.0f) / (float)(128 - 1);
    for (int i = 0; i < n_t; i++)
        for (int k = 0; k < 128; k++) {
            const float f = expf((float)k * -emb);
            const float e = 1000.0f * t_host[i] * f;
            const float sv = (float)sin((double)e), cv = (float)cos((double)e);
            host_split_bf16(sv, hi[(size_t)i * 256 + k], lo[(size_t)i * 256 + k]);
            host_split_bf16(cv, hi[(size_t)i * 256 + 128 + k], lo[(size_t)i * 256 + 128 + k]);
        }
    CK(m->up_time[0].upload(m->sinp.hi, hi.data(), hi.size() * 2, st));
    CK(m->up_time[1].upload(m->sinp.lo, lo.data(), lo.size() * 2, st));
    for (int t0 = 0; t0 < n_t; t0 += 128) {
        const int nb = std::min(128, n_t - t0);
        GemmArgs g1 = gemm_base(rows_from(m->sinp, (size_t)t0 * 256), 256, m->time1, nb);
        g1.act = ACT_SILU; g1.out_hi = m->t1.hi + (size_t)t0 * D; g1.out_lo = m->t1.lo + (size_t)t0 * D; g1.ldob = D;
        CK(run_gemm(m, g1, m->time1, EPI_GENERIC, false, 128, st, 128));
        GemmArgs g2 = gemm_base(rows_from(m->t1, (size_t)t0 * D), D, m->time2, nb);
        if (m->arch == 1) {
            g2.out_f32 = m->temb + (size_t)t0 * D; g2.ldo = D;
            CK(run_gemm(m, g2, m->time2, EPI_GENERIC, false, 128, st, 128));
            continue;
        }
        g2.act = ACT_SILU; g2.out_hi = m->st.hi + (size_t)t0 * D; g2.out_lo = m->st.lo + (size_t)t0 * D; g2.ldob = D;
        CK(run_gemm(m, g2, m->time2, EPI_GENERIC, false, 128, st, 128));
        GemmArgs g3 = gemm_base(rows_from(m->st, (size_t)t0 * D), D, m->adaln, nb);
        g3.out_f32 = m->mod + (size_t)t0 * m->n_adaln; g3.ldo = m->n_adaln;
        CK(run_gemm(m, g3, m->adaln, EPI_GENERIC, false, 128, st, 128));
    }
    return 0;
}

static void set_rope(GemmArgs& q, const f5hip_dit* m, int row_off) {
    q.row_pos = nullptr; q.rope_cos = m->rope_row_cos + (size_t)row_off * 32; q.rope_sin = m->rope_row_sin + (size_t)row_off * 32;
}

struct Stream { int row0, rows; const BlockWeights* w; bool keep; };
static Stream audio_stream(const f5hip_dit* m) { return {0, m->M, &m->blk, true}; }

static int block_residual(f5hip_dit* m, const Stream& s, const Plane2& A, int lda, const PackedW& W, const float* gate, const int* keep, hipStream_t st) {
    const int D = m->cfg.dim;
    GemmArgs g = gemm_base(A, lda, W, s.rows);
    g.mul = gate; g.res = m->h + (size_t)s.row0 * D; g.ldres = D; g.out_f32 = m->h + (size_t)s.row0 * D; g.ldo = D; g.row_keep = keep;
    const bool per_row = gate && m->d_row_tp;
    if (per_row) { g.row_mod = m->d_row_tp + s.row0; g.mod_ld = m->n_adaln; }
    return run_gemm(m, g, W, per_row ? EPI_GENERIC_ROWMUL : EPI_GENERIC, false, 64, st, s.rows);
}

static int block_qkv(f5hip_dit* m, const Stream& s, int l, hipStream_t st) {
    const int D = m->cfg.dim;
    const size_t r0 = s.row0;
    GemmArgs q = gemm_base(rows_from(m->hn, r0 * D), D, s.w->qkv[l], s.rows);
    q.D = D; set_rope(q, m, s.row0); q.qk = m->qk + r0 * 2 * D; q.vt = m->vt + r0; q.ldvt = m->Rtot;
    return run_gemm(m, q, s.w->qkv[l], EPI_QKV, false, 128, st, s.rows);
}

static int block_out(f5hip_dit* m, const Stream& s, int l, const float* gate, hipStream_t st) {
    const int D = m->cfg.dim;
    return block_residual(m, s, rows_from(m->ao, (size_t)s.row0 * D), D, s.w->out[l], gate, s.keep && m->any_masked ? m->d_row_keep : nullptr, st);
}

static int block_ff(f5hip_dit* m, const Stream& s, int l, const float* gate, hipStream_t st) {
    const int D = m->cfg.dim, F = m->cfg.ff_mult * D;
    const Plane2 ff = rows_from(m->ff, (size_t)s.row0 * F);
    GemmArgs f1 = gemm_base(rows_from(m->hn, (size_t)s.row0 * D), D, s.w->ff1[l], s.rows);
    f1.act = ACT_GELU_TANH; f1.out_hi = ff.hi; f1.out_lo = ff.lo; f1.ldob = F; f1.f16_out = m->blk_f16 ? 1 : 0;
    CK(run_gemm(m, f1, s.w->ff1[l], EPI_GENERIC, false, 128, st, s.rows));
    return block_residual(m, s, ff, F, s.w->ff2[l], gate, nullptr, st);
}

static int run_adaln(f5hip_dit* m, const Stream& s, const float* shift, const float* scale, bool f16, hipStream_t st) {
    const int D = m->cfg.dim;
    LnArgs ln = ln_args(m->h + (size_t)s.row0 * D, D, s.rows, D, scale, shift, 1.0f, 1e-6f);
    ln.out_hi = m->hn.hi + (size_t)s.row0 * D; ln.out_lo = m->hn.lo + (size_t)s.row0 * D; ln.ldo = D; ln.f16_out = f16 ? 1 : 0;
    if (m->d_row_tp) { ln.row_mod = m->d_row_tp + s.row0; ln.mod_ld = m->n_adaln; }
    return run_ln(ln, st, m->d_row_tp != nullptr);
}

static int run_proj_out(f5hip_dit* m, hipStream_t st) {
    GemmArgs po = gemm_base(m->hn, m->cfg.dim, m->proj_out, m->M);
    po.out_f32 = m->pred; po.ldo = 128;
    return run_gemm(m, po, m->proj_out, EPI_GENERIC, false, 128, st);
}

static int launch_attention(f5hip_dit* m, hipStream_t st) {
    const f5hip_dit_config& c = m->cfg;
    AttnArgs at; memset(&at, 0, sizeof(at));
    at.qk = m->qk; at.vt = m->vt; at.D = c.dim; at.ldvt = m->Rtot; at.seq_row0 = m->d_seq_row0; at.seq_len = m->d_seq_len;
    at.seq_kvlen = m->d_seq_kvlen; at.out_hi = m->ao.hi; at.out_lo = m->nsplit == 2 ? m->ao.lo : nullptr; at.f16_out = m->blk_f16 ? 1 : 0;
    at.shape_invariant = m->attn_invariant;
    int n_att = m->n_seq;
    if (m->arch == 2) {
        at.seq_row0 = m->d_j_row0; at.seq_len = m->d_j_len; at.seq_kvlen = m->d_j_kvlen;
        at.seq_kv_row0 = m->d_j_kv_row0; at.seq_kv2_row0 = m->d_j_kv2_row0; at.seq_kv2_len = m->d_j_kv2_len;
        n_att = 2 * m->n_seq;
    }
    prof_begin(PROF_ATTN, st);
    const hipError_t e = f5_launch_attn3(at, m->max_len, c.heads, n_att, st);
    if (e != hipSuccess) { prof_end(PROF_ATTN, st); return fail(-7, "attention launch: %s", hipGetErrorString(e)); }
    prof_end(PROF_ATTN, st);
    CKL("attention");
    return 0;
}

static int forward_unett_layers(f5hip_dit* m, int ti, int n_blocks, hipStream_t st) {
    const f5hip_dit_config& c = m->cfg;
    const int D = c.dim, M = m->M;
    const Stream x = audio_stream(m);
    prof_begin(PROF_OTHER, st);
    if (m->d_row_tp) hipLaunchKernelGGL(set_time_token_rows_kernel, dim3(m->n_seq), dim3(256), 0, st, m->h, D, m->d_seq_row0, m->temb, (const int*)m->d_row_tp);
    else hipLaunchKernelGGL(set_time_token_kernel, dim3(m->n_seq), dim3(256), 0, st, m->h, D, m->d_seq_row0, m->temb + (size_t)ti * D);
    prof_end(PROF_OTHER, st);
    CKL("set_time_token");
    const int nb = n_blocks < 0 ? c.depth : n_blocks;
    LnArgs ln = ln_args(m->h, D, M, D, nullptr, m->zeros, 0.0f, 0.0f);
    ln.rms = 1;
    ln.out_hi = m->hn.hi; ln.out_lo = m->hn.lo; ln.ldo = D;
    for (int l = 0; l < nb; l++) {
        if (l < c.depth / 2) {
            prof_begin(PROF_OTHER, st);
            hipLaunchKernelGGL(split_rows_kernel, dim3(M), dim3(256), 0, st, m->h, D, D, M, (const int*)nullptr, m->skipbuf[l].hi, m->skipbuf[l].lo, 2 * D, D);
            prof_end(PROF_OTHER, st);
            CKL("skip save");
        } else {
            const Plane2& sk = m->skipbuf[c.depth - 1 - l];
            prof_begin(PROF_OTHER, st);
            hipLaunchKernelGGL(split_rows_kernel, dim3(M), dim3(256), 0, st, m->h, D, D, M, (const int*)nullptr, sk.hi, sk.lo, 2 * D, 0);
            prof_end(PROF_OTHER, st);
            CKL("skip concat x");
            GemmArgs sp = gemm_base(sk, 2 * D, m->wskip[l], M);
            sp.bias = nullptr; sp.out_f32 = m->h; sp.ldo = D;
            CK(run_gemm(m, sp, m->wskip[l], EPI_GENERIC, false, 64, st));
        }
        ln.scale = m->g_attn[l];
        ln.f16_out = m->blk_f16 ? 1 : 0;
        CK(run_ln(ln, st));
        CK(block_qkv(m, x, l, st));
        CK(launch_attention(m, st));
        CK(block_out(m, x, l, nullptr, st));
        ln.scale = m->g_ff[l];
        CK(run_ln(ln, st));
        CK(block_ff(m, x, l, nullptr, st));
    }
    if (n_blocks >= 0) return 0;
    ln.scale = m->g_out;
    ln.f16_out = 0;
    CK(run_ln(ln, st));
    return run_proj_out(m, st);
}

static int forward_mmdit_layers(f5hip_dit* m, int ti, int n_blocks, hipStream_t st) {
    const f5hip_dit_config& c = m->cfg;
    const int D = c.dim, M = m->M, Mc = m->Mc, C0 = m->row_c0;
    const float* mod = m->mod + (size_t)ti * m->n_adaln;
    const Stream x = audio_stream(m), tx{C0, Mc, &m->blk_c, false};
    if (hipMemcpyAsync(m->h + (size_t)C0 * D, m->te + (size_t)C0 * D, sizeof(float) * (size_t)Mc * D, hipMemcpyDeviceToDevice, st) != hipSuccess) return fail(-6, "MMDiT: text stream copy");
    const int nb = n_blocks < 0 ? c.depth : n_blocks;
    for (int l = 0; l < nb; l++) {
        const bool last = l == c.depth - 1;
        const float* mc = mod + m->mod_c[l];
        const float* mx = mod + m->mod_x[l];
        CK(last ? run_adaln(m, tx, mc + D, mc, m->blk_f16, st) : run_adaln(m, tx, mc, mc + D, m->blk_f16, st));
        CK(run_adaln(m, x, mx, mx + D, m->blk_f16, st));
        CK(block_qkv(m, x, l, st));
        CK(block_qkv(m, tx, l, st));
        CK(launch_attention(m, st));
        CK(block_out(m, x, l, mx + 2 * D, st));
        if (!last) {
            CK(block_out(m, tx, l, mc + 2 * D, st));
            CK(run_adaln(m, tx, mc + 3 * D, mc + 4 * D, m->blk_f16, st));
            CK(block_ff(m, tx, l, mc + 5 * D, st));
        }
        CK(run_adaln(m, x, mx + 3 * D, mx + 4 * D, m->blk_f16, st));
        CK(block_ff(m, x, l, mx + 5 * D, st));
    }
    if (n_blocks >= 0) return 0;
    const float* mf = mod + m->mod_final;
    CK(run_adaln(m, x, mf + D, mf, false, st));
    return run_proj_out(m, st);
}

static int run_conv_pos_embed(int nsplit, bool conv5, int D, int M, const Plane2& hn, const Plane2& c1, const float* h0, float* h,
// ... 152 lines not shown
```

tts-indic-server-f5_amd/csrc/gemm3.h:

```cpp
#pragma once
#include "gemm_epilogue.h"

template <int NSPLIT, int EPI, int BN = 128>
__global__ __launch_bounds__(512) __attribute__((amdgpu_waves_per_eu(2, 2))) void gemm3_kernel(const GemmArgs p) {
    constexpr int NPL = NSPLIT == 2 ? 2 : 1;
    constexpr bool F16 = NSPLIT == 3;
    constexpr int BM = 128, TM = 2, TN = BN / 64, NST = 4;
    constexpr int A_PLANE = BM * 64, B_PLANE = BN * 64, STAGE = NPL * (A_PLANE + B_PLANE);
    constexpr int P = STAGE / 1024 / 4;
    extern __shared__ __attribute__((aligned(16))) char smem[];

    const int tid = threadIdx.x, lane = tid & 63;
    const int wave = __builtin_amdgcn_readfirstlane(tid >> 6);
    const int m0 = blockIdx.y * BM, n0 = blockIdx.x * BN;
    const int nk = p.K >> 5;

    if (wave >= 4) {
        const int pw = wave - 4;
        const char* gsrc[P];
#pragma unroll
        for (int j = 0; j < P; j++) {
            const int off = (pw * P + j) * 1024;
            const bool isA = off < NPL * A_PLANE;
            const int rel = isA ? off : off - NPL * A_PLANE;
            const int plane_bytes = isA ? A_PLANE : B_PLANE;
            const int pl = rel / plane_bytes;
            const int row = (rel - pl * plane_bytes) / 64 + (lane >> 2);
            const int chunk = (lane & 3) ^ ((row >> 2) & 3);
            const __bf16* ap = (NPL == 2 && pl) ? p.A[1] : p.A[0];
            const __bf16* wp = (NPL == 2 && pl) ? p.W[1] : p.W[0];
            const __bf16* base = isA ? ap + (size_t)(m0 + row) * p.lda : wp + (size_t)(n0 + row) * p.ldw;
            gsrc[j] = reinterpret_cast<const char*>(base + chunk * 8);
        }
        auto issue_tile = [&](int kt) {
            char* dst = smem + (kt % NST) * STAGE + pw * (P * 1024);
#pragma unroll
            for (int j = 0; j < P; j++)
                __builtin_amdgcn_global_load_lds((const __attribute__((address_space(1))) void*)(gsrc[j] + (size_t)kt * 64),
                                                 (__attribute__((address_space(3))) void*)(dst + j * 1024), 16, 0, 0);
        };
#pragma unroll
        for (int t = 0; t < NST - 1; t++)
            if (t < nk) issue_tile(t);
        for (int kt = 0; kt < nk; kt++) {
            const int newer = min(NST - 2, nk - 1 - kt);
            if (newer >= 2) wait_vmcnt<2 * P>();
            else if (newer == 1) wait_vmcnt<P>();
            else wait_vmcnt<0>();
            __builtin_amdgcn_s_barrier();
            if (kt + NST - 1 < nk) issue_tile(kt + NST - 1);
        }
        const int cw = pw, cwm = cw >> 1, cwn = cw & 1;
        gemm_epilogue8_producer<EPI, TN>(p, reinterpret_cast<const float*>(smem) + cw * (64 * 32 * TN), m0 + cwm * 64, n0 + cwn * (32 * TN), n0, lane);
        return;
    }

    const int wm = wave >> 1, wn = wave & 1;
    const int fr = lane & 31, fh = lane >> 5;
    f32x16 acc[TM][TN];
#pragma unroll
    for (int i = 0; i < TM; i++)
#pragma unroll
        for (int j = 0; j < TN; j++)
#pragma unroll
            for (int g = 0; g < 16; g++) acc[i][j][g] = 0.0f;

    bf16x8 fa[2][NPL][TM], fb[2][NPL][TN];
    auto read_frags = [&](int buf, const char* st, int s) {
        const int chunk = s * 2 + fh;
#pragma unroll
        for (int pl = 0; pl < NPL; pl++) {
#pragma unroll
            for (int i = 0; i < TM; i++)
                fa[buf][pl][i] = *reinterpret_cast<const bf16x8*>(st + pl * A_PLANE + lds_off2(wm * 64 + i * 32 + fr, chunk));
#pragma unroll
            for (int j = 0; j < TN; j++)
                fb[buf][pl][j] = *reinterpret_cast<const bf16x8*>(st + NPL * A_PLANE + pl * B_PLANE + lds_off2(wn * (32 * TN) + j * 32 + fr, chunk));
        }
    };
    auto mfma_frags = [&](int buf) {
#pragma unroll
        for (int i = 0; i < TM; i++)
#pragma unroll
            for (int j = 0; j < TN; j++) {
                if (NSPLIT == 2) {
                    acc[i][j] = __builtin_amdgcn_mfma_f32_32x32x16_bf16(fa[buf][1][i], fb[buf][0][j], acc[i][j], 0, 0, 0);
                    acc[i][j] = __builtin_amdgcn_mfma_f32_32x32x16_bf16(fa[buf][0][i], fb[buf][1][j], acc[i][j], 0, 0, 0);
                }
                acc[i][j] = mfma_32x32x16<F16>(fa[buf][0][i], fb[buf][0][j], acc[i][j]);
            }
    };
    __builtin_amdgcn_s_barrier();
    read_frags(0, smem, 0);
    for (int kt = 0; kt < nk; kt++) {
        const char* st = smem + (kt % NST) * STAGE;
        read_frags(1, st, 1);
        __builtin_amdgcn_sched_barrier(0);
        mfma_frags(0);
        __builtin_amdgcn_sched_barrier(0);
        if (kt + 1 < nk) {
            asm volatile("s_waitcnt lgkmcnt(0)" ::: "memory");
            __builtin_amdgcn_s_barrier();
            read_frags(0, smem + ((kt + 1) % NST) * STAGE, 0);
            __builtin_amdgcn_sched_barrier(0);
        }
        mfma_frags(1);
        __builtin_amdgcn_sched_barrier(0);
    }
    gemm_epilogue8_consumer<EPI, TN>(p, acc, reinterpret_cast<float*>(smem) + wave * (64 * 32 * TN), m0 + wm * 64, n0 + wn * (32 * TN), n0, lane);
}

template <int NSPLIT, int EPI, int BN = 128>
static hipError_t launch_gemm3_t(const GemmArgs& a, int m_pad, int n_pad, hipStream_t st) {
    constexpr int NPL = NSPLIT == 2 ? 2 : 1;
    constexpr int RING = 4 * NPL * (128 + BN) * 64, SLABS = 4 * 64 * (BN / 2) * 4;
    constexpr int LDS = RING > SLABS ? RING : SLABS;
    static_assert(LDS <= 160 * 1024, "tile does not fit the LDS");
    static unsigned attr_mask = 0;
    if (hipError_t e = f5_set_lds_attr(reinterpret_cast<const void*>(&gemm3_kernel<NSPLIT, EPI, BN>), LDS, attr_mask); e != hipSuccess) return e;
    dim3 grid(n_pad / BN, m_pad / 128);
    hipLaunchKernelGGL((gemm3_kernel<NSPLIT, EPI, BN>), grid, dim3(512), LDS, st, a);
    return hipGetLastError();
}
```

tts-indic-server-f5_amd/csrc/gemm_launch.h:

```cpp
#pragma once
#include <hip/hip_runtime.h>

#include "attn_common.h"
#include "gemm_epilogue.h"

hipError_t f5_launch_gemm_reg(int prec, int bn, bool conv, int epi, const GemmArgs& a, int m_pad, int n_pad, hipStream_t st);
hipError_t f5_launch_gemm3(int prec, int epi, int bn, const GemmArgs& a, int m_pad, int n_pad, hipStream_t st);
hipError_t f5_launch_gemm5_generic(const GemmArgs& a, int rb, int cb, int n_pad, hipStream_t st);
hipError_t f5_launch_gemm5_qkv(const GemmArgs& a, int rb, int cb, int n_pad, hipStream_t st);
hipError_t f5_launch_gemm5_rowmul(const GemmArgs& a, int rb, int cb, int n_pad, hipStream_t st);
hipError_t f5_launch_gemm6(int epi, int rows, const GemmArgs& a, int n_pad, hipStream_t st);
static inline int gemm6_choose_rows(int m_rows, int n_pad) {
    const long long t256 = (long long)((m_rows + 255) / 256) * (n_pad / 256), t176 = (long long)((m_rows + 175) / 176) * (n_pad / 256);
    if (t256 < 224 && t176 < 224) return 0;
    const double c256 = (double)((t256 + 255) / 256), c176 = 0.85 * (double)((t176 + 255) / 256);
    return c176 < c256 ? 176 : 256;
}
hipError_t f5_launch_conv5(int prec, const GemmArgs& a, int n_pad, hipStream_t st);
hipError_t f5_launch_attn3(const AttnArgs& a, int max_len, int heads, int n_seq, hipStream_t st);
void f5_set_attn_shape_invariant(int on);
enum { F5_ATTN_CNT_COUNT = 7 };
long long* f5_attn_counters();

struct Gemm5Choice { int rb, cb; };
static inline Gemm5Choice gemm5_choose(int m_rows, int n_pad) {
    static const int rbs[2] = {11, 8}, cbs[3] = {4, 8, 12};
    Gemm5Choice best = {0, 0};
    double best_cost = 1e30;
    for (int rb : rbs)
        for (int cb : cbs) {
            if (n_pad % (cb * 16)) continue;
            const long long tiles = (long long)((m_rows + rb * 16 - 1) / (rb * 16)) * (n_pad / (cb * 16));
            const double rounds = (double)((tiles + 255) / 256);
            const double cost = rounds * (rb * 16 + cb * 16);
            if (cost < best_cost - 1e-9 || (cost < best_cost + 1e-9 && rb * cb > best.rb * best.cb)) { best_cost = cost; best = {rb, cb}; }
        }
    return best;
}
```

tts-indic-server-f5_amd/csrc/tu_gemm3.hip:

```cpp
#include "gemm3.h"
#include "gemm_launch.h"

hipError_t f5_launch_gemm3(int prec, int epi, int bn, const GemmArgs& a, int m_pad, int n_pad, hipStream_t st) {
    const bool qkv = epi == EPI_QKV;
    if (epi == EPI_GENERIC_ROWMUL) {
        if (bn == 256) return prec == 3 ? launch_gemm3_t<3, EPI_GENERIC_ROWMUL, 256>(a, m_pad, n_pad, st) : hipErrorInvalidValue;
        if (prec == 3) return launch_gemm3_t<3, EPI_GENERIC_ROWMUL>(a, m_pad, n_pad, st);
        if (prec == 2) return launch_gemm3_t<2, EPI_GENERIC_ROWMUL>(a, m_pad, n_pad, st);
        return launch_gemm3_t<1, EPI_GENERIC_ROWMUL>(a, m_pad, n_pad, st);
    }
    if (bn == 256) {
        if (prec == 3) return qkv ? launch_gemm3_t<3, EPI_QKV, 256>(a, m_pad, n_pad, st) : launch_gemm3_t<3, EPI_GENERIC, 256>(a, m_pad, n_pad, st);
        return hipErrorInvalidValue;
    }
    if (prec == 3) return qkv ? launch_gemm3_t<3, EPI_QKV>(a, m_pad, n_pad, st) : launch_gemm3_t<3, EPI_GENERIC>(a, m_pad, n_pad, st);
    if (prec == 2) return qkv ? launch_gemm3_t<2, EPI_QKV>(a, m_pad, n_pad, st) : launch_gemm3_t<2, EPI_GENERIC>(a, m_pad, n_pad, st);
    return qkv ? launch_gemm3_t<1, EPI_QKV>(a, m_pad, n_pad, st) : launch_gemm3_t<1, EPI_GENERIC>(a, m_pad, n_pad, st);
}
```

tts-indic-server-f5_amd/csrc/unit_ops.h:

```cpp
#pragma once

struct OpBufs {
    std::vector<void*> ptrs;
    ~OpBufs() { for (void* p : ptrs) if (p) (void)hipFree(p); }
    template <typename T> T* get(size_t n) {
        void* p = nullptr;
        if (hipMalloc(&p, n * sizeof(T)) != hipSuccess) return nullptr;
        ptrs.push_back(p);
        return (T*)p;
    }
};

template <typename T> static T* op_filled(OpBufs& b, size_t n, int pad, hipStream_t st) {
    T* p = b.get<T>(n);
    if (p) (void)hipMemsetAsync(p, pad, n * sizeof(T), st);
    return p;
}

static void op_pack_planes(const float* src, int R, int C, int R_pad, __bf16* hi, __bf16* lo, bool f16, hipStream_t st) {
    hipLaunchKernelGGL(pack_weight_kernel, dim3(R_pad), dim3(256), 0, st, src, R, C, C, hi, f16 ? (__bf16*)nullptr : lo, C);
}

template <typename Launch>
static int collect_stamps(OpBufs& b, hipStream_t st, Launch launch, std::vector<unsigned long long>& h, int& ng, unsigned long long& tmin,
                          unsigned long long& tmax) {
    const int maxg = 4096;
    unsigned long long* d = b.get<unsigned long long>((size_t)maxg * 16);
    if (!d) return 0;
    (void)hipMemsetAsync(d, 0, sizeof(unsigned long long) * maxg * 16, st);
    for (int rep = 0; rep < 3; rep++) CK(launch(d, rep));
    (void)hipStreamSynchronize(st);
    h.resize((size_t)maxg * 16);
    (void)hipMemcpy(h.data(), d, h.size() * 8, hipMemcpyDeviceToHost);
    for (int g2 = 0; g2 < maxg; g2++) if (h[(size_t)g2 * 16]) { ng = g2 + 1; tmin = std::min(tmin, h[(size_t)g2 * 16]); tmax = std::max(tmax, std::max(h[(size_t)g2 * 16 + 6], h[(size_t)g2 * 16 + 14])); }
    return 0;
}

template <typename... Head>
static void print_spread(std::vector<double> v, const char* fmt, Head... head) {
    if (v.empty()) return;
    std::sort(v.begin(), v.end());
    fprintf(stderr, fmt, head..., v.front(), v[v.size() / 2], v.back());
}

template <typename Launch>
static int gemm5_stamp_report(OpBufs& b, int M, int N, int K, hipStream_t st, Launch launch) {
    std::vector<unsigned long long> h;
    int ng = 0;
    unsigned long long tmin = ~0ull, tmax = 0;
    CK(collect_stamps(b, st, launch, h, ng, tmin, tmax));
    if (h.empty()) return 0;
    const char* names[7] = {"start", "tile0 landed (loader)", "k-loop end", "E1 passed", "E2 passed (slab done)", "row phase issued", "stores drained"};
    fprintf(stderr, "[gemm5 stamps] M %d N %d K %d: %d workgroups, first start -> last end %.2f us\n", M, N, K, ng, (tmax - tmin) * 0.01);
    for (int w = 0; w < 2; w++)
        for (int i = 0; i < 7; i++) {
            std::vector<double> v;
            for (int g2 = 0; g2 < ng; g2++) { const unsigned long long t = h[(size_t)g2 * 16 + w * 8 + i]; if (t) v.push_back((t - tmin) * 0.01); }
            print_spread(v, "[gemm5 stamps]   wave %d  %-26s min %6.2f  median %6.2f  max %6.2f us after the first workgroup started\n", w * 4, names[i]);
        }
    if (ng == 256) {
        for (int tn = 0; tn < 16; tn++) {
            std::vector<double> v;
            for (int g2 = 0; g2 < ng; g2++) {
                const int tile = (g2 & 7) * (ng >> 3) + (g2 >> 3);
                if (tile % 16 == tn) v.push_back((h[(size_t)g2 * 16 + 5] - h[(size_t)g2 * 16 + 3]) * 0.01);
            }
            print_spread(v, "[gemm5 stamps]   column slab %2d: epilogue min %5.2f median %5.2f max %5.2f us\n", tn);
        }
    }
    return 0;
}

template <typename Launch>
static int gemm6_stamp_report(OpBufs& b, int M, int N, int K, hipStream_t st, Launch launch) {
    std::vector<unsigned long long> h;
    int ng = 0;
    unsigned long long tmin = ~0ull, tmax = 0;
    CK(collect_stamps(b, st, launch, h, ng, tmin, tmax));
    if (h.empty()) return 0;
    fprintf(stderr, "[gemm6 stamps] M %d N %d K %d: %d workgroups, first start -> last end %.2f us\n", M, N, K, ng, (tmax - tmin) * 0.01);
    const char* names[6] = {"k-loop", "quarter 0", "quarter 1", "quarter 2", "quarter 3", "store drain"};
    for (int w = 0; w < 2; w++)
        for (int i = 0; i < 6; i++) {
            std::vector<double> v;
            for (int g2 = 0; g2 < ng; g2++) {
                const unsigned long long t0 = h[(size_t)g2 * 16 + w * 8 + i], t1 = h[(size_t)g2 * 16 + w * 8 + i + 1];
                if (t0 && t1) v.push_back((t1 - t0) * 0.01);
            }
            print_spread(v, "[gemm6 stamps]   wave %d  %-12s duration min %6.2f  median %6.2f  max %6.2f us\n", w * 4, names[i]);
        }
    {
        std::vector<double> v;
        for (int g2 = 0; g2 < ng; g2++) {
            const unsigned long long cyc = h[(size_t)g2 * 16 + 7], t0 = h[(size_t)g2 * 16], t1 = h[(size_t)g2 * 16 + 1];
            if (cyc && t1 > t0) v.push_back((double)cyc / ((double)(t1 - t0) * 10.0));
        }
        print_spread(v, "[gemm6 stamps]   shader clock during the k-loop: min %.2f  median %.2f  max %.2f GHz  (the 2.5 PFLOP/s roof is 2.4 GHz x 4096 FLOP / clk / CU x 256 CUs)\n");
    }
    {
        std::vector<double> v;
        for (int g2 = 0; g2 < ng; g2++) v.push_back((h[(size_t)g2 * 16] - tmin) * 0.01);
        std::sort(v.begin(), v.end());
        fprintf(stderr, "[gemm6 stamps]   workgroup start: 25 %% %.2f  50 %% %.2f  75 %% %.2f  90 %% %.2f  last %.2f us\n", v[ng / 4], v[ng / 2], v[3 * ng / 4], v[9 * ng / 10], v.back());
    }
    return 0;
}

static int op_gemm_run(int32_t M, int32_t N, int32_t K, const float* a_dev, const float* w_dev, const float* bias_dev, int32_t prec, int32_t act,
                       const float* mul_dev, const int32_t* row_mod_host, int32_t mod_ld, const float* res_dev, const uint8_t* row_keep_host,
                       float* out_dev, uint16_t* out16_dev, int32_t w_copies, int32_t iters, double* avg_us, void* stream, int32_t bn) {
    const int epi = row_mod_host ? EPI_GENERIC_ROWMUL : EPI_GENERIC;
    if (M <= 0 || N <= 0 || K <= 0 || K % 32 || N % 4 || !a_dev || !w_dev || prec < 1 || prec > 3 || (!out_dev && !out16_dev))
        return fail(-1, "op_gemm: bad argument (need K %% 32 == 0, N %% 4 == 0, prec 1..3)");
    if (bn == 0) bn = 128;
    if (bn != 64 && bn != 128) return fail(-1, "op_gemm: bn must be 0, 64 or 128 (got %d)", bn);
    if (out16_dev && (res_dev || out_dev)) return fail(-1, "op_gemm: the 16-bit output is the (no residual, no fp32 output) epilogue");
    hipStream_t st = (hipStream_t)stream;
    const int M_pad = (M + 127) / 128 * 128, N_pad = (N + 127) / 128 * 128;
    const bool f16 = prec == 3;
    if (w_copies < 1) w_copies = 1;
    OpBufs b;
    Plane2 A;
    A.hi = b.get<__bf16>((size_t)M_pad * K); A.lo = b.get<__bf16>((size_t)M_pad * K);
    float* bias = b.get<float>(N_pad);
    int *keep = nullptr, *row_mod = nullptr;
    if (!A.hi || !A.lo || !bias) return fail(-5, "op_gemm: hipMalloc");
    std::vector<PackedW> Ws(w_copies);
    for (auto& W : Ws) {
        W.hi = b.get<__bf16>((size_t)N_pad * K); W.lo = f16 ? nullptr : b.get<__bf16>((size_t)N_pad * K);
        if (!W.hi || (!f16 && !W.lo)) return fail(-5, "op_gemm: hipMalloc weights");
        W.n = N; W.k = K; W.n_pad = N_pad; W.k_pad = K; W.ld = K; W.bias = bias; W.f16 = f16;
        op_pack_planes(w_dev, N, K, N_pad, W.hi, W.lo, f16, st);
        if (f16 && N >= 2048 && pack_frag(W, st)) return -5;
        if (W.frag) b.ptrs.push_back(W.frag);
    }
    op_pack_planes(a_dev, M, K, M_pad, A.hi, A.lo, f16, st);
    (void)hipMemsetAsync(bias, 0, sizeof(float) * N_pad, st);
    if (bias_dev) (void)hipMemcpyAsync(bias, bias_dev, sizeof(float) * N, hipMemcpyDeviceToDevice, st);
    if (row_keep_host) {
        keep = b.get<int>(M_pad);
        std::vector<int> hk(M_pad, 0);
        for (int i = 0; i < M; i++) hk[i] = row_keep_host[i];
        if (!keep || upload_sync(st, keep, hk) != hipSuccess) return fail(-6, "op_gemm: row_keep upload");
    }
    if (row_mod_host) {
        row_mod = b.get<int>(M_pad);
        std::vector<int> hm(M_pad, 0);
        std::copy(row_mod_host, row_mod_host + M, hm.begin());
        if (!row_mod || upload_sync(st, row_mod, hm) != hipSuccess) return fail(-6, "op_gemm: row_mod upload");
    }
    auto args_for = [&](const PackedW& W) {
        GemmArgs g = gemm_base(A, K, W, M);
        g.act = act; g.mul = mul_dev; g.res = res_dev; g.ldres = N; g.row_keep = keep;
        if (row_mod) { g.row_mod = row_mod; g.mod_ld = mod_ld; }
        if (out16_dev) { g.out_hi = (__bf16*)out16_dev; g.ldob = N; g.f16_out = 1; }
        else { g.out_f32 = out_dev; g.ldo = N; }
        return g;
    };
    {
        GemmArgs g = args_for(Ws[0]);
        CK(run_gemm_n(prec, M_pad, g, Ws[0], epi, false, bn, st));
    }
    auto stamped = [&](unsigned long long* d, int rep) {
        GemmArgs g = args_for(Ws[rep % w_copies]);
        g.stamps = d;
        return run_gemm_n(prec, M_pad, g, Ws[rep % w_copies], epi, false, bn, st);
    };
    if (getenv("F5HIP_GEMM5_STAMPS")) CK(gemm5_stamp_report(b, M, N, K, st, stamped));
    if (getenv("F5HIP_GEMM6_STAMPS")) CK(gemm6_stamp_report(b, M, N, K, st, stamped));
    if (iters > 0 && avg_us) {
        float* scratch = b.get<float>((size_t)M * N);
        if (!scratch) return fail(-5, "op_gemm: hipMalloc scratch");
        CK(time_launches(3, iters, avg_us, st, [&](int i) {
            const PackedW& W = Ws[i % w_copies];
            GemmArgs g = args_for(W);
            if (!out16_dev) { g.out_f32 = scratch; if (res_dev) g.res = scratch; }
            return run_gemm_n(prec, M_pad, g, W, epi, false, bn, st);
        }));
    }
    if (hipStreamSynchronize(st) != hipSuccess) return fail(-7, "op_gemm: %s", hipGetErrorString(hipGetLastError()));
    return 0;
}

extern "C" int f5hip_op_gemm(int32_t M, int32_t N, int32_t K, const float* a_dev, const float* w_dev, const float* bias_dev, int32_t prec,
                             int32_t act, const float* mul_dev, const float* res_dev, const uint8_t* row_keep_host, float* out_dev,
                             uint16_t* out16_dev, int32_t w_copies, int32_t iters, double* avg_us, void* stream, int32_t bn) {
    return op_gemm_run(M, N, K, a_dev, w_dev, bias_dev, prec, act, mul_dev, nullptr, 0, res_dev, row_keep_host, out_dev, out16_dev, w_copies, iters,
                       avg_us, stream, bn);
}

extern "C" int f5hip_op_gemm_rowmul(int32_t M, int32_t N, int32_t K, const float* a_dev, const float* w_dev, const float* bias_dev, int32_t prec,
                                    const float* mul_dev, const int32_t* row_mod_host, int32_t mod_ld, int32_t n_mod_rows, const float* res_dev,
                                    const uint8_t* row_keep_host, float* out_dev, void* stream, int32_t bn) {
    if (!mul_dev || !row_mod_host || !res_dev || !out_dev || mod_ld < N || mod_ld % 4 || n_mod_rows <= 0 || ((uintptr_t)mul_dev & 15))
        return fail(-1, "op_gemm_rowmul: bad argument (need mul, row_mod, res and out; mod_ld >= N, mod_ld %% 4 == 0, mul 16-byte aligned)");
    for (int i = 0; i < M; i++)
        if (row_mod_host[i] < 0 || row_mod_host[i] >= n_mod_rows) return fail(-1, "op_gemm_rowmul: row_mod[%d] = %d out of range", i, row_mod_host[i]);
    return op_gemm_run(M, N, K, a_dev, w_dev, bias_dev, prec, ACT_NONE, mul_dev, row_mod_host, mod_ld, res_dev, row_keep_host, out_dev, nullptr, 1, 0,
                       nullptr, stream, bn);
}

extern "C" int f5hip_op_qkv(int32_t M, int32_t D, const float* a_dev, const float* w_dev, const float* bias_dev, const int32_t* row_pos,
                            int32_t prec, uint16_t* qk_dev, uint16_t* vt_dev, int32_t iters, double* avg_us, void* stream) {
    if (M <= 0 || D <= 0 || D % 128 || !a_dev || !w_dev || !bias_dev || !row_pos || !qk_dev || !vt_dev || prec < 1 || prec > 3)
        return fail(-1, "op_qkv: bad argument (need D %% 128 == 0)");
    hipStream_t st = (hipStream_t)stream;
    const int M_pad = (M + 127) / 128 * 128, N = 3 * D, N_pad = (N + 127) / 128 * 128;
    const bool f16 = prec == 3;
    OpBufs b;
    Plane2 A; PackedW W;
    A.hi = b.get<__bf16>((size_t)M_pad * D); A.lo = b.get<__bf16>((size_t)M_pad * D);
    W.hi = b.get<__bf16>((size_t)N_pad * D); W.lo = f16 ? nullptr : b.get<__bf16>((size_t)N_pad * D);
    float* bias = b.get<float>(N_pad);
    std::vector<float> hc, hs;
    rope_tables(hc, hs);
    float* rc = b.get<float>(hc.size()); float* rs = b.get<float>(hs.size());
    int* pos = b.get<int>(M_pad);
    if (!A.hi || !A.lo || !W.hi || (!f16 && !W.lo) || !bias || !rc || !rs || !pos) return fail(-5, "op_qkv: hipMalloc");
    W.n = N; W.k = D; W.n_pad = N_pad; W.k_pad = D; W.ld = D; W.bias = bias; W.f16 = f16;
    std::vector<int> hp(M_pad, 0);
    for (int i = 0; i < M; i++) { if (row_pos[i] < 0 || row_pos[i] > 4096) return fail(-1, "op_qkv: row_pos out of range"); hp[i] = row_pos[i]; }
    if (upload_sync(st, rc, hc, rs, hs, pos, hp) != hipSuccess) return fail(-6, "op_qkv: table upload");
    op_pack_planes(w_dev, N, D, N_pad, W.hi, W.lo, f16, st);
    if (f16 && pack_frag(W, st)) return -5;
    if (W.frag) b.ptrs.push_back(W.frag);
    op_pack_planes(a_dev, M, D, M_pad, A.hi, A.lo, f16, st);
    (void)hipMemsetAsync(bias, 0, sizeof(float) * N_pad, st);
    (void)hipMemcpyAsync(bias, bias_dev, sizeof(float) * N, hipMemcpyDeviceToDevice, st);
    GemmArgs g = gemm_base(A, D, W, M);
    g.D = D; g.row_pos = pos; g.rope_cos = rc; g.rope_sin = rs; g.qk = (__bf16*)qk_dev; g.vt = (__bf16*)vt_dev; g.ldvt = M_pad;
    if (getenv("F5HIP_GEMM5_STAMPS"))
        CK(gemm5_stamp_report(b, M, N, D, st, [&](unsigned long long* d, int) {
            GemmArgs g2 = g;
            g2.stamps = d;
            return run_gemm_n(prec, M_pad, g2, W, EPI_QKV, false, 128, st);
        }));
    CK(time_launches(1, iters, avg_us, st, [&](int) { return run_gemm_n(prec, M_pad, g, W, EPI_QKV, false, 128, st); }));
    if (hipStreamSynchronize(st) != hipSuccess) return fail(-7, "op_qkv: %s", hipGetErrorString(hipGetLastError()));
    return 0;
}

extern "C" int f5hip_op_layernorm(int32_t M, int32_t D, const float* x_dev, const float* scale_dev, const float* shift_dev, float gain_off, float eps,
                                  int32_t rms, float* out_dev, void* stream) {
    if (M <= 0 || D <= 0 || D % 4 || !x_dev || !scale_dev || !shift_dev || !out_dev) return fail(-1, "op_layernorm: bad argument");
    hipStream_t st = (hipStream_t)stream;
    LnArgs ln = ln_args(x_dev, D, M, D, scale_dev, shift_dev, gain_off, eps);
    ln.rms = rms; ln.out_f32 = out_dev; ln.ldof = D;
    CK(run_ln(ln, st));
    return 0;
}

__global__ __launch_bounds__(256) void op_pack_qkv_kernel(const float* q, const float* k, const float* v, int D, const int* row_src, int M_pad,
                                                          __bf16* qk, __bf16* vt) {
    const int row = blockIdx.x, src = row_src[row];
    for (int c = threadIdx.x; c < D; c += 256) {
        const float qv = src >= 0 ? q[(size_t)src * D + c] * F5_Q_SCALE : 0.0f;
        const float kv = src >= 0 ? k[(size_t)src * D + c] : 0.0f;
        const float vv = src >= 0 ? v[(size_t)src * D + c] : 0.0f;
        reinterpret_cast<_Float16*>(qk)[(size_t)row * 2 * D + c] = sat_f16(qv);
        reinterpret_cast<_Float16*>(qk)[(size_t)row * 2 * D + D + c] = sat_f16(kv);
        reinterpret_cast<_Float16*>(vt)[(size_t)c * M_pad + vt_col(row)] = sat_f16(vv);
    }
}
__global__ __launch_bounds__(256) void op_unpack_planes_kernel(const __bf16* hi, const __bf16* lo, int f16, int D, const int* frame_row, float* out) {
    const int f = blockIdx.x, row = frame_row[f];
    for (int c = threadIdx.x; c < D; c += 256) {
        const size_t i = (size_t)row * D + c;
        out[(size_t)f * D + c] = f16 ? (float)reinterpret_cast<const _Float16*>(hi)[i] : (float)hi[i] + (lo ? (float)lo[i] : 0.0f);
    }
}

extern "C" int f5hip_op_layernorm_planes(int32_t M, int32_t D, const float* x_dev, const float* scale_dev, const float* shift_dev,
                                         const int32_t* row_mod_host, int32_t mod_ld, int32_t n_mod_rows, float gain_off, float eps,
// ... 323 lines not shown
                                                 int32_t scale, int32_t M, int32_t C, const float* a_dev, const float* w_dev, int32_t variant,
                                                 float* wave_dev, int64_t wave_len, void* stream) {
    if (M <= 0 || C <= 0 || !a_dev || !w_dev || !wave_dev || !item_wave_off || wave_len <= 0 || variant < 0 || variant > 2)
        return fail(-1, "op_bigvgan_conv_post_ragged: bad argument");
    std::vector<int> h;
    int t_max = 0;
    CK(op_item_table("op_bigvgan_conv_post_ragged", n_items, item_row0, item_valid, item_wave_off, scale, M, wave_len, h, t_max));
    hipStream_t st = (hipStream_t)stream;
    OpBufs b;
    int* items = b.get<int>(h.size());
    if (!items) return fail(-5, "op_bigvgan_conv_post_ragged: hipMalloc");
    if (upload_sync(st, items, h) != hipSuccess) return fail(-6, "op_bigvgan_conv_post_ragged: upload");
    int rc = bv_conv_post(a_dev, C, C, n_items, 0, t_max, w_dev, wave_dev, variant, st, reinterpret_cast<const int4*>(items), scale);
    if (hipStreamSynchronize(st) != hipSuccess && !rc) rc = fail(-7, "op_bigvgan_conv_post_ragged: %s", hipGetErrorString(hipGetLastError()));
    return rc;
}

extern "C" int f5hip_op_bigvgan_mean3(int64_t rows, int32_t C, int32_t n_in, const float* y0_dev, const float* y1_dev, const float* y2_dev,
                                      int32_t mode, int32_t ldo, float* out_f32_dev, float* planes_dev, void* stream) {
    if (rows <= 0 || C <= 0 || C % 4 || (n_in != 1 && n_in != 3) || !y0_dev || (n_in == 3 && (!y1_dev || !y2_dev)) || mode < 0 || mode > 3 ||
        (mode == 0 ? !out_f32_dev : (!planes_dev || ldo < C || ldo % 4)) || rows * (int64_t)std::max(C, ldo) / 4 > (int64_t)256 * 2147483647)
        return fail(-1, "op_bigvgan_mean3: bad argument");
    hipStream_t st = (hipStream_t)stream;
    OpBufs b;
    __bf16 *hi = nullptr, *lo = nullptr;
    const size_t n = mode ? (size_t)rows * ldo : 0;
    if (mode) {
        hi = b.get<__bf16>(n); lo = op_filled<__bf16>(b, n, 0, st);
        if (!hi || !lo) return fail(-5, "op_bigvgan_mean3: hipMalloc");
        hipLaunchKernelGGL(bv_mean3_kernel, dim3((unsigned)((n / 4 + 255) / 256)), dim3(256), 0, st, planes_dev, planes_dev, planes_dev, 1, (size_t)rows, ldo,
                           (float*)nullptr, hi, lo, ldo, mode);
    }
    const size_t n4 = (size_t)rows * C / 4;
    hipLaunchKernelGGL(bv_mean3_kernel, dim3((unsigned)((n4 + 255) / 256)), dim3(256), 0, st, y0_dev, n_in == 3 ? y1_dev : y0_dev, n_in == 3 ? y2_dev : y0_dev, n_in,
                       (size_t)rows, C, out_f32_dev, hi, lo, ldo, mode);
    if (mode) hipLaunchKernelGGL(op_planes_to_f32_kernel, dim3((unsigned)((n + 255) / 256)), dim3(256), 0, st, hi, lo, mode == 2 ? 1 : 0, n, planes_dev);
    if (hipStreamSynchronize(st) != hipSuccess) return fail(-7, "op_bigvgan_mean3: %s", hipGetErrorString(hipGetLastError()));
    return 0;
}

extern "C" int f5hip_op_bigvgan_mel_rows(int32_t n, const int32_t* item_row0, const int32_t* item_frames, int32_t T, int32_t M0, int32_t C,
                                         const float* mel_dev, int32_t f16, float* out_dev, void* stream) {
    if (n <= 0 || T <= 0 || M0 <= 0 || C <= 0 || C > 128 || !mel_dev || !out_dev || (item_row0 ? (!item_frames || M0 % 128) : (M0 % n || M0 / n < T)))
        return fail(-1, "op_bigvgan_mel_rows: bad argument");
    hipStream_t st = (hipStream_t)stream;
    OpBufs b;
    const size_t ne = (size_t)M0 * 128;
    __bf16* hi = op_filled<__bf16>(b, ne, 0xff, st); __bf16* lo = op_filled<__bf16>(b, ne, 0xff, st);
    if (!hi || !lo) return fail(-5, "op_bigvgan_mel_rows: hipMalloc");
    if (item_row0) {
        const int nblk = M0 / 128;
        std::vector<int> tab, h((size_t)3 * nblk, 0);
        for (int i = 0; i < n; i++)
            if (item_frames[i] > T) return fail(-1, "op_bigvgan_mel_rows: item %d has %d frames, the column stride is %d", i, item_frames[i], T);
        CK(op_block_table("op_bigvgan_mel_rows", n, item_row0, nullptr, item_frames, M0, 128, 128, tab));
        std::copy(tab.begin(), tab.end(), h.begin());
        for (int i = 0; i < n; i++)
            for (int r = item_row0[i]; r < item_row0[i] + item_frames[i]; r += 128) h[(size_t)2 * nblk + r / 128] = i;
        int* d = b.get<int>(h.size());
        if (!d) return fail(-5, "op_bigvgan_mel_rows: hipMalloc");
        if (upload_sync(st, d, h) != hipSuccess) return fail(-6, "op_bigvgan_mel_rows: upload");
        hipLaunchKernelGGL(bv_mel_rows_ragged_kernel, dim3(M0), dim3(128), 0, st, mel_dev, C, T, d, d + nblk, d + 2 * nblk, hi, lo, f16 ? 1 : 0);
    } else {
        hipLaunchKernelGGL(bv_mel_rows_kernel, dim3(M0), dim3(128), 0, st, mel_dev, C, T, M0 / n, hi, lo, f16 ? 1 : 0);
    }
    hipLaunchKernelGGL(op_planes_to_f32_kernel, dim3((unsigned)((ne + 255) / 256)), dim3(256), 0, st, hi, lo, f16 ? 1 : 0, ne, out_dev);
    if (hipStreamSynchronize(st) != hipSuccess) return fail(-7, "op_bigvgan_mel_rows: %s", hipGetErrorString(hipGetLastError()));
    return 0;
}

__global__ __launch_bounds__(256) void op_scatter_rows_kernel(const float* x, int C, int n, const int* frame_row, float* dst, __bf16* hi, __bf16* lo,
                                                              int ldd) {
    const int f = blockIdx.x;
    if (f >= n) return;
    const size_t r = (size_t)frame_row[f];
    for (int c = threadIdx.x; c < C; c += 256) {
        const float v = x[(size_t)f * C + c];
        if (dst) dst[r * ldd + c] = v;
        if (hi) {
            __bf16 h, l;
            split_bf16(v, h, l);
            hi[r * ldd + c] = h;
            lo[r * ldd + c] = l;
        }
    }
}

__global__ __launch_bounds__(256) void op_gather_planes_kernel(const __bf16* hi, const __bf16* lo, int lds, int C, int n, const int* frame_row, float* dst) {
    const int f = blockIdx.x;
    if (f >= n) return;
    const size_t r = (size_t)frame_row[f];
    for (int c = threadIdx.x; c < C; c += 256) dst[(size_t)f * C + c] = (float)hi[r * lds + c] + (lo ? (float)lo[r * lds + c] : 0.0f);
}

struct OpLayout { int R = 0, frames = 0; int *row_start = nullptr, *row_end, *row_seq, *frame_row, *seq_row0, *seq_len; std::vector<int> h; };
static int op_layout(OpBufs& b, int n_seq, const int32_t* seq_len, int lead, OpLayout& L, hipStream_t st) {
    L.R = 0; L.frames = 0;
    for (int s = 0; s < n_seq; s++) {
        if (seq_len[s] <= 0 || seq_len[s] > 4096) return fail(-1, "seq_len[%d] = %d out of range", s, seq_len[s]);
        L.R += seq_rows(seq_len[s], lead); L.frames += seq_len[s];
    }
    const int R = L.R, F = L.frames;
    L.h.assign((size_t)3 * R + F + 2 * n_seq, 0);
    int *rs = L.h.data(), *re = rs + R, *rq = re + R, *fr = rq + R, *s0 = fr + F, *sl = s0 + n_seq;
    for (int r = 0; r < R; r++) rq[r] = -1;
    for (int s = 0, r0 = 0, f0 = 0; s < n_seq; s++) {
        set_seq_bounds(rs, re, rq, r0, lead, seq_len[s], s);
        for (int i = 0; i < seq_len[s]; i++) fr[f0 + i] = r0 + lead + i;
        s0[s] = r0; sl[s] = lead + seq_len[s];
        r0 += seq_rows(seq_len[s], lead); f0 += seq_len[s];
    }
    int* d = b.get<int>(L.h.size());
    if (!d) return fail(-5, "op layout: hipMalloc");
    if (hipMemcpyAsync(d, L.h.data(), sizeof(int) * L.h.size(), hipMemcpyHostToDevice, st) != hipSuccess) return fail(-6, "op layout: upload");
    L.row_start = d; L.row_end = d + R; L.row_seq = d + 2 * R; L.frame_row = d + 3 * R; L.seq_row0 = L.frame_row + F; L.seq_len = L.seq_row0 + n_seq;
    return 0;
}

extern "C" int f5hip_op_conv_pos_embed(int32_t n_seq, const int32_t* seq_len, int32_t lead, int32_t D, const float* x_dev, const float* w1_host,
                                       const float* b1_host, const float* w2_host, const float* b2_host, int32_t impl, int32_t prec, int32_t pad_nan,
                                       float* out_dev, float* c1_dev, void* stream) {
    if (n_seq <= 0 || !seq_len || lead < 0 || lead > 1 || D <= 0 || D % 128 || D / 16 > 64 || !x_dev || !w1_host || !b1_host || !w2_host || !b2_host ||
        !out_dev || (impl != 0 && impl != 5) || (prec != 1 && prec != 2) || (impl == 5 && (prec != 2 || lead)))
        return fail(-1, "op_conv_pos_embed: bad argument");
    hipStream_t st = (hipStream_t)stream;
    OpBufs b;
    OpLayout L;
    CK(op_layout(b, n_seq, seq_len, lead, L, st));
    const size_t n = (size_t)L.R * D, slack = 256;
    const int pad = pad_nan ? 0xff : 0;
    float* h0 = op_filled<float>(b, n + slack, pad, st);
    float* h = op_filled<float>(b, n + slack, pad, st);
    Plane2 hn, c1;
    hn.hi = op_filled<__bf16>(b, n + slack, pad, st); hn.lo = op_filled<__bf16>(b, n + slack, pad, st);
    c1.hi = op_filled<__bf16>(b, n + slack, pad, st); c1.lo = op_filled<__bf16>(b, n + slack, pad, st);
    if (!h0 || !h || !hn.hi || !hn.lo || !c1.hi || !c1.lo) return fail(-5, "op_conv_pos_embed: hipMalloc");
    hipLaunchKernelGGL(op_scatter_rows_kernel, dim3(L.frames), dim3(256), 0, st, x_dev, D, L.frames, L.frame_row, h0, hn.hi, hn.lo, D);
    CKL("op scatter");
    PackedW w1, w2;
    int rc = pack_conv_pos(w1, w1_host, b1_host, D);
    if (!rc) rc = pack_conv_pos(w2, w2_host, b2_host, D);
    if (!rc) rc = run_conv_pos_embed(prec, impl == 5, D, L.R, hn, c1, h0, h, w1, w2, L.row_start, L.row_end, st);
    if (!rc) {
        hipLaunchKernelGGL(gather_rows_kernel, dim3(L.frames), dim3(128), 0, st, h, D, D, L.frames, L.frame_row, out_dev, D);
        if (c1_dev) hipLaunchKernelGGL(op_gather_planes_kernel, dim3(L.frames), dim3(256), 0, st, c1.hi, prec == 2 ? c1.lo : nullptr, D, D, L.frames,
                                       L.frame_row, c1_dev);
        if (hipGetLastError() != hipSuccess) rc = fail(-7, "op_conv_pos_embed: gather launch");
    }
    if (hipStreamSynchronize(st) != hipSuccess && !rc) rc = fail(-7, "op_conv_pos_embed: %s", hipGetErrorString(hipGetLastError()));
    free_packed(w1); free_packed(w2);
    return rc;
}

extern "C" int f5hip_op_convnext_block(int32_t n_seq, const int32_t* seq_len, int32_t Td, const float* x_dev, const float* const* params_host,
                                       int32_t pad_nan, float* out_dev, float* tap_ln_dev, float* tap_ty_dev, float* tap_grn_dev, void* stream) {
    if (n_seq <= 0 || !seq_len || Td <= 0 || Td % 32 || Td > 1536 || !x_dev || !params_host || !out_dev) return fail(-1, "op_convnext_block: bad argument");
    for (int i = 0; i < 10; i++) if (!params_host[i]) return fail(-1, "op_convnext_block: parameter %d is null", i);
    hipStream_t st = (hipStream_t)stream;
    OpBufs b;
    OpLayout L;
    CK(op_layout(b, n_seq, seq_len, 0, L, st));
    const size_t n = (size_t)L.R * Td;
    const int pad = pad_nan ? 0xff : 0;
    float* te = op_filled<float>(b, n, pad, st);
    float* ty = op_filled<float>(b, 2 * n, pad, st);
    float* gx = op_filled<float>(b, (size_t)n_seq * 2 * Td, pad, st);
    Plane2 tn, tg;
    tn.hi = op_filled<__bf16>(b, n, pad, st); tn.lo = op_filled<__bf16>(b, n, pad, st);
    tg.hi = op_filled<__bf16>(b, 2 * n, pad, st); tg.lo = op_filled<__bf16>(b, 2 * n, pad, st);
    if (!te || !ty || !gx || !tn.hi || !tn.lo || !tg.hi || !tg.lo) return fail(-5, "op_convnext_block: hipMalloc");
    hipLaunchKernelGGL(op_scatter_rows_kernel, dim3(L.frames), dim3(256), 0, st, x_dev, Td, L.frames, L.frame_row, te, (__bf16*)nullptr,
                       (__bf16*)nullptr, Td);
    CKL("op scatter");
    const float* const* P = params_host;
    TextBlock tb;
    int rc = upload_f32(&tb.dw_w, P[0], (size_t)Td * 7) || upload_f32(&tb.dw_b, P[1], Td) || upload_f32(&tb.ln_w, P[2], Td) ||
             upload_f32(&tb.ln_b, P[3], Td) || upload_f32(&tb.gamma, P[6], 2 * Td) || upload_f32(&tb.beta, P[7], 2 * Td) ||
             pack_linear(tb.pw1, P[4], 2 * Td, Td, Td, P[5]) || pack_linear(tb.pw2, P[8], Td, 2 * Td, 2 * Td, P[9]) ? -4 : 0;
    if (!rc) rc = run_text_block(2, tb, Td, L.R, n_seq, te, tn, ty, tg, gx, L.row_start, L.row_end, L.row_seq, L.seq_row0, L.seq_len, nullptr,
                                 nullptr, 0, st);
    if (!rc) {
        hipLaunchKernelGGL(gather_rows_kernel, dim3(L.frames), dim3(128), 0, st, te, Td, Td, L.frames, L.frame_row, out_dev, Td);
        if (tap_ln_dev) hipLaunchKernelGGL(op_gather_planes_kernel, dim3(L.frames), dim3(256), 0, st, tn.hi, tn.lo, Td, Td, L.frames, L.frame_row, tap_ln_dev);
        if (tap_ty_dev) hipLaunchKernelGGL(gather_rows_kernel, dim3(L.frames), dim3(128), 0, st, ty, 2 * Td, 2 * Td, L.frames, L.frame_row, tap_ty_dev, 2 * Td);
        if (tap_grn_dev) hipLaunchKernelGGL(op_gather_planes_kernel, dim3(L.frames), dim3(256), 0, st, tg.hi, tg.lo, 2 * Td, 2 * Td, L.frames, L.frame_row,
                                            tap_grn_dev);
        if (hipGetLastError() != hipSuccess) rc = fail(-7, "op_convnext_block: gather launch");
    }
    if (hipStreamSynchronize(st) != hipSuccess && !rc) rc = fail(-7, "op_convnext_block: %s", hipGetErrorString(hipGetLastError()));
    for (float* p : {tb.dw_w, tb.dw_b, tb.ln_w, tb.ln_b, tb.gamma, tb.beta}) dev_free(p);
    free_packed(tb.pw1); free_packed(tb.pw2);
    return rc;
}

static int op_cfg_launch(const char* name, CfgBufs cb, int U, int rows, const int32_t* urow_c_host, const int32_t* urow_u_host, float cfg, int op,
                         float dt, const int32_t* frame_unit_host, const int32_t* unit_op_host, const float* unit_dt_host, int n_units, int n_act,
                         float* xs_dev, hipStream_t st) {
    if (!frame_unit_host) n_units = 0;
    for (int u = 0; u < U; u++)
        if (urow_c_host[u] < 0 || urow_c_host[u] >= rows || urow_u_host[u] < -1 || urow_u_host[u] >= rows ||
            (frame_unit_host && (frame_unit_host[u] < 0 || frame_unit_host[u] >= n_units)))
            return fail(-1, "%s: frame %d: row or unit out of range", name, u);
    OpBufs b;
    const size_t n = (size_t)rows * 128, o_unit = 2 * (size_t)U, o_cfg = 3 * (size_t)U, o_op = 4 * (size_t)U, o_dt = o_op + n_units;
    cb.xs.hi = b.get<__bf16>(n); cb.xs.lo = b.get<__bf16>(n);
    int* meta = b.get<int>(o_dt + n_units);
    if (!cb.xs.hi || !cb.xs.lo || !meta) return fail(-5, "%s: hipMalloc", name);
    std::vector<int> hm(o_dt + n_units, 0);
    for (int u = 0; u < U; u++) {
        hm[u] = urow_c_host[u]; hm[U + u] = urow_u_host[u];
        if (frame_unit_host) hm[o_unit + u] = frame_unit_host[u];
        memcpy(&hm[o_cfg + u], &cfg, sizeof(float));
    }
    for (int k = 0; k < n_units; k++) hm[o_op + k] = unit_op_host ? unit_op_host[k] : op;
    if (n_units) memcpy(&hm[o_dt], unit_dt_host, sizeof(float) * n_units);
    if (upload_sync(st, meta, hm) != hipSuccess) return fail(-6, "%s: upload", name);
    hipLaunchKernelGGL(split_rows_kernel, dim3(rows), dim3(256), 0, st, (const float*)xs_dev, 128, 128, rows, (const int*)nullptr, cb.xs.hi, cb.xs.lo, 128, 0);
    CKL("op cfg split");
    cb.urow_c = meta; cb.urow_u = meta + U;
    if (!cb.frame_cfg) cb.frame_cfg = reinterpret_cast<const float*>(meta + o_cfg);
    launch_cfg_step(cb, U, op, dt, frame_unit_host ? meta + o_unit : nullptr, meta + o_op, reinterpret_cast<const float*>(meta + o_dt), n_act, st);
    CKL("op cfg step");
    hipLaunchKernelGGL(op_planes_to_f32_kernel, dim3((unsigned)((n + 255) / 256)), dim3(256), 0, st, cb.xs.hi, cb.xs.lo, 0, n, xs_dev);
    CKL("op cfg planes");
    if (hipStreamSynchronize(st) != hipSuccess) return fail(-7, "%s: %s", name, hipGetErrorString(hipGetLastError()));
    return 0;
}

extern "C" int f5hip_op_cfg_step(int32_t method, int32_t stage, int32_t U, int32_t mel, int32_t rows, float* xout_dev, float* xbase_dev,
                                 const float* pred_dev, const int32_t* urow_c_host, const int32_t* urow_u_host, float cfg, const float* cfg_frame_dev,
                                 float dt, const int32_t* frame_unit_host, const float* unit_dt_host, int32_t n_units, int32_t n_act, float* k1_dev,
                                 float* k2_dev, float* k3_dev, float* xs_dev, const uint8_t* final_flags_host, const float* cond_dev, float* out_dev,
                                 void* stream) {
    const bool step = method >= 0, rk4 = method == 2, unit_dt = frame_unit_host != nullptr;
    if (U <= 0 || mel <= 0 || mel > 128 || !xbase_dev || (method != -1 && method != 0 && method != 2))
        return fail(-1, "op_cfg_step: bad argument (method -1, 0 or 2; mel <= 128)");
    if (step && (rows <= 0 || !pred_dev || !urow_c_host || !urow_u_host || !xs_dev || (rk4 ? stage < 0 || stage > 3 || !k1_dev || !k2_dev || !k3_dev ||
                 (xout_dev && xout_dev != xbase_dev) : !xout_dev)))
        return fail(-1, "op_cfg_step: missing buffer of the step (rk4: stage 0..3, k1..k3, in place)");
    if (unit_dt && (!unit_dt_host || !cfg_frame_dev || n_units <= 0 || n_act < 0 || n_act > n_units))
        return fail(-1, "op_cfg_step: the per-unit form needs unit_dt, cfg_frame and 0 <= n_act <= n_units");
    if (final_flags_host && (!cond_dev || !out_dev)) return fail(-1, "op_cfg_step: the final select needs cond and out");
    hipStream_t st = (hipStream_t)stream;
    if (step) {
        const int op = rk4 ? CFG_OP_RK4_1 + stage : xout_dev == xbase_dev ? CFG_OP_EULER : CFG_OP_MID_HALF;
        const CfgBufs cb{xbase_dev, rk4 ? k1_dev : xout_dev, k2_dev, k3_dev, pred_dev, nullptr, nullptr, cfg_frame_dev, {}, mel};
        CK(op_cfg_launch("op_cfg_step", cb, U, rows, urow_c_host, urow_u_host, cfg, op, dt, frame_unit_host, nullptr, unit_dt_host, n_units, n_act, xs_dev, st));
    }
    if (final_flags_host) {
        OpBufs b;
        int* flags = b.get<int>(U);
        std::vector<int> hf(final_flags_host, final_flags_host + U);
        if (!flags || upload_sync(st, flags, hf) != hipSuccess) return fail(-6, "op_cfg_step: flag upload");
        hipLaunchKernelGGL(final_select_kernel, dim3(U), dim3(128), 0, st, (const float*)xbase_dev, cond_dev, (const int*)flags, mel, U, out_dev);
        CKL("op_cfg_step final_select");
        if (hipStreamSynchronize(st) != hipSuccess) return fail(-7, "op_cfg_step: %s", hipGetErrorString(hipGetLastError()));
    }
    return 0;
}

extern "C" int f5hip_op_cfg_mixed(int32_t U, int32_t mel, int32_t rows, float* xstate_dev, const float* pred_dev, const int32_t* urow_c_host,
                                  const int32_t* urow_u_host, const float* cfg_frame_dev, const int32_t* frame_unit_host, const int32_t* unit_op_host,
                                  const float* unit_dt_host, int32_t n_units, int32_t n_act, float* k1_dev, float* k2_dev, float* k3_dev, float* xs_dev,
                                  void* stream) {
    if (U <= 0 || mel <= 0 || mel > 128 || rows <= 0 || !xstate_dev || !pred_dev || !urow_c_host || !urow_u_host || !cfg_frame_dev || !frame_unit_host ||
        !unit_op_host || !unit_dt_host || !k1_dev || !k2_dev || !k3_dev || !xs_dev)
        return fail(-1, "op_cfg_mixed: bad argument (mel <= 128, every buffer)");
    if (n_units <= 0 || n_act < 0 || n_act > n_units) return fail(-1, "op_cfg_mixed: needs 0 <= n_act <= n_units");
    for (int k = 0; k < n_units; k++)
        if (unit_op_host[k] < CFG_OP_NONE || unit_op_host[k] >= CFG_OP_COUNT) return fail(-1, "op_cfg_mixed: unit_op[%d] = %d (0..7)", k, unit_op_host[k]);
    const CfgBufs cb{xstate_dev, k1_dev, k2_dev, k3_dev, pred_dev, nullptr, nullptr, cfg_frame_dev, {}, mel};
    return op_cfg_launch("op_cfg_mixed", cb, U, rows, urow_c_host, urow_u_host, 0.0f, CFG_OP_NONE, 0.0f, frame_unit_host, unit_op_host, unit_dt_host, n_units,
                         n_act, xs_dev, (hipStream_t)stream);
}

extern "C" int f5hip_op_row_tp(int32_t R, const int32_t* row_unit_host, int32_t n_units, const int32_t* unit_tp_host, int32_t* row_tp_host, void* stream) {
    if (R <= 0 || n_units <= 0 || !row_unit_host || !unit_tp_host || !row_tp_host) return fail(-1, "op_row_tp: bad argument");
    for (int r = 0; r < R; r++)
        if (row_unit_host[r] < 0 || row_unit_host[r] >= n_units) return fail(-1, "op_row_tp: row_unit[%d] = %d out of range", r, row_unit_host[r]);
    hipStream_t st = (hipStream_t)stream;
    OpBufs b;
    int* d = b.get<int>((size_t)2 * R + n_units);
    if (!d) return fail(-5, "op_row_tp: hipMalloc");
    std::vector<int> h((size_t)2 * R + n_units, -1);
    std::copy(row_unit_host, row_unit_host + R, h.begin());
    std::copy(unit_tp_host, unit_tp_host + n_units, h.begin() + 2 * (size_t)R);
    if (upload_sync(st, d, h) != hipSuccess) return fail(-6, "op_row_tp: upload");
    hipLaunchKernelGGL(row_tp_kernel, dim3((R + 255) / 256), dim3(256), 0, st, (const int*)d, (const int*)(d + 2 * (size_t)R), R, d + R);
    CKL("op_row_tp");
    if (hipMemcpyAsync(row_tp_host, d + R, sizeof(int) * R, hipMemcpyDeviceToHost, st) != hipSuccess || hipStreamSynchronize(st) != hipSuccess)
        return fail(-7, "op_row_tp: %s", hipGetErrorString(hipGetLastError()));
    return 0;
}

extern "C" int f5hip_op_time_table(f5hip_dit* m, const float* t_host, int32_t n_t, float* sinus_dev, float* mod_dev, int32_t mod_cols,
                                   float* temb_dev, void* stream) {
    if (!m || !m->finalized) return fail(-1, "model not finalized");
    if (!t_host || n_t <= 0 || !sinus_dev) return fail(-1, "op_time_table: bad argument");
    if (mod_dev && (m->arch == 1 || mod_cols != m->n_adaln)) return fail(-1, "op_time_table: mod has %d columns in this model (got %d)", m->n_adaln, mod_cols);
    if (temb_dev && m->arch != 1) return fail(-1, "op_time_table: only UNetT keeps the time embeddings");
    hipStream_t st = (hipStream_t)stream;
    CK(ensure_workspace(m, 128, 1, 1));
    CK(precompute_time(m, t_host, n_t, st));
    const size_t ns = (size_t)n_t * 256;
    hipLaunchKernelGGL(op_planes_to_f32_kernel, dim3((unsigned)((ns + 255) / 256)), dim3(256), 0, st, m->sinp.hi, m->sinp.lo, 0, ns, sinus_dev);
    CKL("op_time_table planes");
    if (mod_dev && hipMemcpyAsync(mod_dev, m->mod, sizeof(float) * (size_t)n_t * m->n_adaln, hipMemcpyDeviceToDevice, st) != hipSuccess)
        return fail(-6, "op_time_table: mod copy");
    if (temb_dev && hipMemcpyAsync(temb_dev, m->temb, sizeof(float) * (size_t)n_t * m->cfg.dim, hipMemcpyDeviceToDevice, st) != hipSuccess)
        return fail(-6, "op_time_table: temb copy");
    if (hipStreamSynchronize(st) != hipSuccess) return fail(-7, "op_time_table: %s", hipGetErrorString(hipGetLastError()));
    return 0;
}
```

tts-indic-server-f5_amd/ops.py:

```python
from __future__ import annotations

import ctypes as C

import numpy as np
import torch

from . import _lib, torch_ops
from .wave_codec import rate_pair

ACT = {"none": 0, "gelu_tanh": 1, "gelu_erf": 2, "mish": 3, "silu": 4}


def _p(t):
    if t is None:
        return None
    if isinstance(t, np.ndarray):
        return C.c_void_p(t.ctypes.data)
    return C.c_void_p(t.data_ptr())


def _f32(t, dev):
    return None if t is None else t.to(dev, torch.float32).contiguous()


# ... 81 lines not shown
        out = torch.zeros(M, Cc, dtype=torch.float32, device=dev)
    assert out.dtype == torch.float32 and out.is_contiguous() and out.shape[1] == Cc and out.shape[0] >= M
    _lib.check(_lib.lib().f5hip_op_bigvgan_snake(batch, M // batch, valid, Cc, _p(x), _p(alpha_log), _p(beta_log), out_format, _p(out),
                                                 out.shape[0], _lib.current_stream_ptr()), "f5hip_op_bigvgan_snake")
    return out


def bigvgan_upsample(x, weight, bias=None, *, batch, valid, rate, prec=2):
    dev = x.device
    x = _f32(x, dev)
    c_in, c_out, k = weight.shape
    assert k == 2 * rate
    M = x.shape[0]
    w = np.ascontiguousarray(weight.detach().to(torch.float32).cpu().numpy())
    b = None if bias is None else np.ascontiguousarray(bias.detach().to(torch.float32).cpu().numpy())
    out = torch.empty(M * rate, c_out, dtype=torch.float32, device=dev)
    _lib.check(_lib.lib().f5hip_op_bigvgan_upsample(batch, M // batch, valid, c_in, c_out, rate, _p(x), _p(w), _p(b), _p(out), prec,
                                                    _lib.current_stream_ptr()), "f5hip_op_bigvgan_upsample")
    return out


def bigvgan_conv_post(a, weight, *, batch, valid, variant=0):
    dev = a.device
    a = _f32(a, dev)
    M, Cc = a.shape
    w = _f32(weight.reshape(Cc, 7), dev)
    wave = torch.empty(batch, valid, dtype=torch.float32, device=dev)
    _lib.check(_lib.lib().f5hip_op_bigvgan_conv_post(batch, M // batch, valid, Cc, _p(a), _p(w), variant, _p(wave), _lib.current_stream_ptr()),
               "f5hip_op_bigvgan_conv_post")
    return wave


def conv1d_ragged(x, weight, bias=None, res=None, *, row0, valid, rows=None, blk, dilation=1, prec=2, impl=5, ups_rate=0):
    dev = x.device
    x = _f32(x, dev)
    M = x.shape[0]
    if ups_rate:
        c_in, c_out, k = weight.shape
        assert k == 2 * ups_rate
    else:
        c_out, c_in, k = weight.shape
    w = np.ascontiguousarray(weight.detach().to(torch.float32).cpu().numpy())
    b = None if bias is None else np.ascontiguousarray(bias.detach().to(torch.float32).cpu().numpy())
    r = None if res is None else _f32(res, dev)
    r0, rw, vl = _i32(row0), _i32(rows), _i32(valid)
    assert len(vl) == len(r0) and (rw is None or len(rw) == len(r0))
    out = torch.empty(M * max(ups_rate, 1), c_out, dtype=torch.float32, device=dev)
    _lib.check(_lib.lib().f5hip_op_conv1d_ragged(len(r0), _p(r0), _p(rw), _p(vl), M, blk, c_in, c_out, k, dilation, ups_rate, _p(x), _p(w), _p(b),
                                                 _p(r), _p(out), prec, impl, _lib.current_stream_ptr()), "f5hip_op_conv1d_ragged")
    return out


def bigvgan_snake_ragged(x, alpha_log, beta_log, *, row0, valid, scale, out_format=SNAKE_OUT_F32, out=None):
    dev = x.device
    x, alpha_log, beta_log = (_f32(t, dev) for t in (x, alpha_log, beta_log))
    M, Cc = x.shape
    if out is None:
        out = torch.zeros(M, Cc, dtype=torch.float32, device=dev)
    assert out.dtype == torch.float32 and out.is_contiguous() and out.shape[1] == Cc and out.shape[0] >= M
    r0, vl = _i32(row0), _i32(valid)
    assert len(vl) == len(r0)
    _lib.check(_lib.lib().f5hip_op_bigvgan_snake_ragged(len(r0), _p(r0), _p(vl), scale, M, Cc, _p(x), _p(alpha_log), _p(beta_log), out_format,
                                                        _p(out), out.shape[0], _lib.current_stream_ptr()), "f5hip_op_bigvgan_snake_ragged")
    return out


def bigvgan_conv_post_ragged(a, weight, wave, *, row0, valid, wave_off, scale, variant=0):
    dev = a.device
    a = _f32(a, dev)
    M, Cc = a.shape
    w = _f32(weight.reshape(Cc, 7), dev)
    assert wave.dtype == torch.float32 and wave.is_contiguous() and wave.dim() == 1 and wave.device == dev
    r0, vl, wo = _i32(row0), _i32(valid), _i32(wave_off)
    assert len(vl) == len(r0) == len(wo)
    _lib.check(_lib.lib().f5hip_op_bigvgan_conv_post_ragged(len(r0), _p(r0), _p(vl), _p(wo), scale, M, Cc, _p(a), _p(w), variant, _p(wave),
                                                            wave.numel(), _lib.current_stream_ptr()), "f5hip_op_bigvgan_conv_post_ragged")
    return wave


MEAN3_NONE, MEAN3_SPLIT, MEAN3_F16, MEAN3_BF16 = 0, 1, 2, 3


def bigvgan_mean3(ys, *, mode=MEAN3_NONE, planes=None, want_f32=True):
    dev = ys[0].device
    ys = [_f32(y, dev) for y in ys]
    rows, Cc = ys[0].shape
    out = torch.empty(rows, Cc, dtype=torch.float32, device=dev) if want_f32 or mode == 0 else None
    ldo = 0
    if mode:
        assert planes.dtype == torch.float32 and planes.is_contiguous() and planes.shape[0] == rows and planes.device == dev
        ldo = planes.shape[1]
    y = ys + [None, None]
    _lib.check(_lib.lib().f5hip_op_bigvgan_mean3(rows, Cc, len(ys), _p(y[0]), _p(y[1]), _p(y[2]), mode, ldo, _p(out), _p(planes) if mode else None,
                                                 _lib.current_stream_ptr()), "f5hip_op_bigvgan_mean3")
    return out, planes if mode else None


def bigvgan_mel_rows(mel, *, rows, row0=None, frames=None, f16=False):
    dev = mel.device
    mel = _f32(mel, dev)
    n, Cc, T = mel.shape
    out = torch.empty(rows, 128, dtype=torch.float32, device=dev)
    r0, fr = _i32(row0), _i32(frames)
    assert r0 is None or (fr is not None and len(r0) == len(fr) == n)
    _lib.check(_lib.lib().f5hip_op_bigvgan_mel_rows(n, _p(r0), _p(fr), T, rows, Cc, _p(mel), int(f16), _p(out), _lib.current_stream_ptr()),
               "f5hip_op_bigvgan_mel_rows")
    return out


def joint_attention(q, k, v, x_len, c_len, x_kvlen=None, *, heads, shape_invariant=-1, out_format=ATTN_OUT_SPLIT):
    dev = q.device
    q, k, v = (_f32(t, dev) for t in (q, k, v))
    out = torch.empty_like(q)
    xl = np.ascontiguousarray(np.asarray(x_len, dtype=np.int32))
    cl = np.ascontiguousarray(np.asarray(c_len, dtype=np.int32))
    kl = None if x_kvlen is None else np.ascontiguousarray(np.asarray(x_kvlen, dtype=np.int32))
    _lib.check(_lib.lib().f5hip_op_joint_attention(len(xl), _p(xl), _p(kl), _p(cl), heads, _p(q), _p(k), _p(v), _p(out), _lib.current_stream_ptr(),
                                                   int(shape_invariant), int(out_format)), "f5hip_op_joint_attention")
    return out


def _host_f32(t):
    return np.ascontiguousarray(t.detach().to(torch.float32).cpu().numpy())


def conv_pos_embed(x, w1, b1, w2, b2, *, seq_len, lead=0, impl=5, prec=2, taps=False, pad_nan=False):
    dev = x.device
    x = _f32(x, dev)
    frames, D = x.shape
    sl = np.ascontiguousarray(np.asarray(seq_len, dtype=np.int32))
    assert int(sl.sum()) == frames
    hw = [_host_f32(t) for t in (w1, b1, w2, b2)]
    out = torch.empty(frames, D, dtype=torch.float32, device=dev)
    c1 = torch.empty(frames, D, dtype=torch.float32, device=dev) if taps else None
    _lib.check(_lib.lib().f5hip_op_conv_pos_embed(len(sl), _p(sl), int(lead), D, _p(x), *(_p(a) for a in hw), int(impl), int(prec), int(pad_nan),
                                                  _p(out), _p(c1), _lib.current_stream_ptr()), "f5hip_op_conv_pos_embed")
    return (out, c1) if taps else out


CONVNEXT_PARAMS = ("dwconv.weight", "dwconv.bias", "norm.weight", "norm.bias", "pwconv1.weight", "pwconv1.bias", "grn.gamma", "grn.beta",
                   "pwconv2.weight", "pwconv2.bias")


def convnext_block(x, params, *, seq_len, taps=False, pad_nan=False):
    dev = x.device
    x = _f32(x, dev)
    n, Td = x.shape
    sl = np.ascontiguousarray(np.asarray(seq_len, dtype=np.int32))
    assert int(sl.sum()) == n
    hp = [_host_f32(params[k]).reshape(-1) for k in CONVNEXT_PARAMS]
    arr = (C.c_void_p * 10)(*(a.ctypes.data for a in hp))
    out = torch.empty(n, Td, dtype=torch.float32, device=dev)
    tp = {"ln": torch.empty(n, Td, dtype=torch.float32, device=dev), "ty": torch.empty(n, 2 * Td, dtype=torch.float32, device=dev),
          "grn": torch.empty(n, 2 * Td, dtype=torch.float32, device=dev)} if taps else {}
    _lib.check(_lib.lib().f5hip_op_convnext_block(len(sl), _p(sl), Td, _p(x), arr, int(pad_nan), _p(out), _p(tp.get("ln")), _p(tp.get("ty")),
                                                  _p(tp.get("grn")), _lib.current_stream_ptr()), "f5hip_op_convnext_block")
    return (out, tp) if taps else out


def _i32(a):
    return None if a is None else np.ascontiguousarray(np.asarray(a, dtype=np.int32))


def _col_ptr(table, col):
    assert table.dtype == torch.float32 and table.is_contiguous() and table.dim() == 2
    return C.c_void_p(table.data_ptr() + 4 * int(col))


def gemm_rowmul(a, w, bias, table, col, row_mod, res, *, prec=3, row_keep=None, bn=64):
    dev = a.device
    M, K = a.shape
    N = w.shape[0]
    a, w, bias, res = (_f32(t, dev) for t in (a, w, bias, res))
    assert table.device == a.device and col + N <= table.shape[1]
    out = torch.empty(M, N, device=dev, dtype=torch.float32)
    keep = None if row_keep is None else np.ascontiguousarray(row_keep.cpu().numpy().astype(np.uint8))
    rm = _i32(row_mod)
    assert rm.shape == (M,)
    _lib.check(_lib.lib().f5hip_op_gemm_rowmul(M, N, K, _p(a), _p(w), _p(bias), prec, _col_ptr(table, col), _p(rm), table.shape[1], table.shape[0],
                                               _p(res), _p(keep), _p(out), _lib.current_stream_ptr(), bn), "f5hip_op_gemm_rowmul")
    return out


LN_OUT_SPLIT, LN_OUT_F16 = 0, 1


def layernorm_planes(x, scale, shift, *, out_format=LN_OUT_SPLIT, gain_off=1.0, eps=1e-6, table=None, row_mod=None):
    dev = x.device
    M, D = x.shape
    x = _f32(x, dev)
    out = torch.empty_like(x)
    if table is None:
        scale, shift = _f32(scale, dev), _f32(shift, dev)
        ps, ph, rm, ld, nrow = _p(scale), _p(shift), None, 0, 0
    else:
        assert table.device == x.device and max(scale, shift) + D <= table.shape[1]
        rm = _i32(row_mod)
        assert rm.shape == (M,)
        ps, ph, ld, nrow = _col_ptr(table, scale), _col_ptr(table, shift), table.shape[1], table.shape[0]
    _lib.check(_lib.lib().f5hip_op_layernorm_planes(M, D, _p(x), ps, ph, _p(rm), ld, nrow, float(gain_off), float(eps), int(out_format), _p(out),
                                                    _lib.current_stream_ptr()), "f5hip_op_layernorm_planes")
    return out


CFG_EULER, CFG_RK4, CFG_NO_STEP = 0, 2, -1


def cfg_step(method, stage, xout, xbase, pred, urow_c, urow_u, xs, *, cfg=0.0, cfg_frame=None, dt=0.0, frame_unit=None, unit_dt=None, n_act=0,
             k=(None, None, None), final_flags=None, cond=None):
    U, mel = xbase.shape
    for t in (xout, xbase, pred, xs, cfg_frame, cond) + tuple(k):
        assert t is None or (t.dtype == torch.float32 and t.is_contiguous() and t.is_cuda)
    uc, uu = (None if a is None else _i32(a) for a in (urow_c, urow_u))
    fu = None if frame_unit is None else _i32(frame_unit)
    ud = None if unit_dt is None else np.ascontiguousarray(np.asarray(unit_dt, dtype=np.float32))
    ff = None if final_flags is None else np.ascontiguousarray(np.asarray(final_flags, dtype=np.uint8))
    out = torch.empty_like(xbase) if ff is not None else None
    _lib.check(_lib.lib().f5hip_op_cfg_step(int(method), int(stage), U, mel, 0 if pred is None else pred.shape[0], _p(xout), _p(xbase), _p(pred), _p(uc),
                                            _p(uu), float(cfg), _p(cfg_frame), float(dt), _p(fu), _p(ud), 0 if ud is None else len(ud), int(n_act),
                                            _p(k[0]), _p(k[1]), _p(k[2]), _p(xs), _p(ff), _p(cond), _p(out), _lib.current_stream_ptr()),
               "f5hip_op_cfg_step")
    return out


CFG_OP_NONE, CFG_OP_EULER, CFG_OP_MID_HALF, CFG_OP_MID_FULL, CFG_OP_RK4_1 = 0, 1, 2, 3, 4


def cfg_mixed(xstate, pred, urow_c, urow_u, xs, cfg_frame, frame_unit, unit_op, unit_dt, n_act, k):
    U, mel = xstate.shape
    for t in (xstate, pred, xs, cfg_frame) + tuple(k):
        assert t.dtype == torch.float32 and t.is_contiguous() and t.is_cuda
    uc, uu, fu, uo = (_i32(a) for a in (urow_c, urow_u, frame_unit, unit_op))
    ud = np.ascontiguousarray(np.asarray(unit_dt, dtype=np.float32))
    assert uo.shape == ud.shape and fu.shape == (U,)
    _lib.check(_lib.lib().f5hip_op_cfg_mixed(U, mel, pred.shape[0], _p(xstate), _p(pred), _p(uc), _p(uu), _p(cfg_frame), _p(fu), _p(uo), _p(ud), len(uo),
                                             int(n_act), _p(k[0]), _p(k[1]), _p(k[2]), _p(xs), _lib.current_stream_ptr()), "f5hip_op_cfg_mixed")


def row_tp(row_unit, unit_tp):
    ru, ut = _i32(row_unit), _i32(unit_tp)
    out = np.full(ru.shape, -1, dtype=np.int32)
    _lib.check(_lib.lib().f5hip_op_row_tp(len(ru), _p(ru), len(ut), _p(ut), _p(out), _lib.current_stream_ptr()), "f5hip_op_row_tp")
    return out


def time_table(model, t):
    from .model import MMDiTArch, UNetTArch
    arch, dev = model.arch, model.device
    th = np.ascontiguousarray(np.asarray(t, dtype=np.float32))
    n_t, D = len(th), arch.dim
    unett = isinstance(arch, UNetTArch)
    cols = 0 if unett else (6 * arch.depth + 2) * D + ((6 * (arch.depth - 1) + 2) * D if isinstance(arch, MMDiTArch) else 0)
    sinus = torch.empty(n_t, 256, device=dev, dtype=torch.float32)
    mod = None if unett else torch.empty(n_t, cols, device=dev, dtype=torch.float32)
    temb = torch.empty(n_t, D, device=dev, dtype=torch.float32) if unett else None
    _lib.check(_lib.lib().f5hip_op_time_table(model._h, _p(th), n_t, _p(sinus), _p(mod), cols, _p(temb), _lib.current_stream_ptr()),
               "f5hip_op_time_table")
    return sinus, mod, temb


def call_op(name, *args):
    try:
        return getattr(torch_ops.ops(), name)(*args)
    except RuntimeError as e:
        raise _lib.F5HipError(str(e)) from e


def _per_request(op, what, values, dtype, n=None, per="request"):
    a = np.ascontiguousarray(np.asarray(values, dtype=dtype))
    if a.ndim < 1 or len(a) < 1 or (n is not None and len(a) != n):
        raise _lib.F5HipError(f"{op}: {what} needs one value per {per} ({'at least one' if n is None else n}), got {a.shape}")
    return a


def _check_dev_f32(op, t, name):
    if not (torch.is_tensor(t) and t.dtype == torch.float32 and t.is_contiguous() and t.is_cuda):
        raise _lib.F5HipError(f"{op}: {name} must be a contiguous fp32 tensor on the HIP device")


def pointer_table(op, tensors, what):
    for i, t in enumerate(tensors):
        if not (torch.is_tensor(t) and t.dtype == torch.float32 and t.is_cuda and t.dim() == 1 and t.is_contiguous() and t.device == tensors[0].device):
            raise _lib.F5HipError(f"{op}: {what} {i} must be a contiguous 1-D fp32 tensor on one HIP device (no CPU fallback)")
    return np.array([t.data_ptr() for t in tensors], dtype=np.uint64), np.array([t.numel() for t in tensors], dtype=np.int32)


def _pcm_requests(op, pcm, in_off, max_len, len_dev, several=False):
    tensors = list(pcm) if several and not torch.is_tensor(pcm) else [pcm]
    ml = _per_request(op, "max_len", max_len, np.int32)
    n = len(ml)
    io = _per_request(op, "in_off", in_off, np.int64, n)
    if len(tensors) not in (1, n):
        raise _lib.F5HipError(f"{op}: pcm is one tensor or one per request (got {len(tensors)} for {n})")
    for t in tensors:
        if not (torch.is_tensor(t) and t.dtype == torch.int16 and t.is_cuda and t.dim() == 1 and t.is_contiguous() and t.device == tensors[0].device):
            raise _lib.F5HipError(f"{op}: pcm must be contiguous 1-D int16 tensors on one HIP device")
    if len_dev is not None:
        if not (torch.is_tensor(len_dev) and len_dev.dtype == torch.int32 and len_dev.is_cuda and len_dev.numel() == n and len_dev.device == tensors[0].device):
            raise _lib.F5HipError(f"{op}: len_dev must be an int32 tensor with one value per request on the pcm's device")
        len_dev = len_dev.contiguous()
    return tensors, io, ml, n, len_dev


def _pcm_sources(op, tensors, io, ml):
    anchor = next((t for t in tensors if t.numel()), None)
    if anchor is None:
        anchor = torch.zeros(8, device=tensors[0].device, dtype=torch.int16)
    base, rel = anchor.data_ptr(), np.zeros(len(ml), dtype=np.int64)
    for i in range(len(ml)):
# ... 445 lines not shown
```

Measured before the change: 10330.

## Add thin-M gemm3 kernel, split GRN stats reduction, cache time table

Adds a 32-row-tile gemm3 kernel with warp-specialized async loads, chosen for small-M generic GEMMs so that few-workgroup launches fill more of the GPU. Rewrites the GRN stats kernel so that 8 waves split the row range per column and reduce the partial sums in shared memory, giving more parallelism over sequence length. Caches the precomputed time/adaLN table across sampling calls when the time points are unchanged, skipping redundant rebuilds. Also adds a gx tap and counters for testing. The caching holds per-model state and depends on the time grid being identical between calls.

```diff
diff --git a/include/f5hip.h b/include/f5hip.h
--- a/include/f5hip.h
+++ b/include/f5hip.h
@@ -132,6 +132,9 @@
                             float* out_dev, float* c1_dev, void* stream);
 int f5hip_op_convnext_block(int32_t n_seq, const int32_t* seq_len, int32_t Td, const float* x_dev, const float* const* params_host,
                             int32_t pad_nan, float* out_dev, float* tap_ln_dev, float* tap_ty_dev, float* tap_grn_dev, void* stream);
+int f5hip_op_convnext_block_gx(int32_t n_seq, const int32_t* seq_len, int32_t Td, const float* x_dev, const float* const* params_host,
+                               int32_t pad_nan, float* out_dev, float* tap_ln_dev, float* tap_ty_dev, float* tap_grn_dev, float* tap_gx_dev,
+                               void* stream);
 
 
 typedef struct f5hip_vocos_config {
diff --git a/tts-indic-server-f5_amd/_lib.py b/tts-indic-server-f5_amd/_lib.py
--- a/tts-indic-server-f5_amd/_lib.py
+++ b/tts-indic-server-f5_amd/_lib.py
@@ -87,6 +87,7 @@
     "f5hip_op_bigvgan_mel_rows": (C.c_int, [C.c_int32, C.c_void_p, C.c_void_p] + [C.c_int32] * 3 + [C.c_void_p, C.c_int32, C.c_void_p, C.c_void_p]),
     "f5hip_op_conv_pos_embed": (C.c_int, [C.c_int32, C.c_void_p, C.c_int32, C.c_int32] + [C.c_void_p] * 5 + [C.c_int32] * 3 + [C.c_void_p] * 3),
     "f5hip_op_convnext_block": (C.c_int, [C.c_int32, C.c_void_p, C.c_int32, C.c_void_p, C.c_void_p, C.c_int32] + [C.c_void_p] * 5),
+    "f5hip_op_convnext_block_gx": (C.c_int, [C.c_int32, C.c_void_p, C.c_int32, C.c_void_p, C.c_void_p, C.c_int32] + [C.c_void_p] * 6),
     "f5hip_vocos_create": (C.c_void_p, [C.POINTER(VocosConfig)]),
     "f5hip_vocos_destroy": (None, [C.c_void_p]),
     "f5hip_vocos_load_param": (C.c_int, [C.c_void_p, C.c_char_p, C.c_void_p, C.c_int64]),
diff --git a/tts-indic-server-f5_amd/csrc/cfm_sample.h b/tts-indic-server-f5_amd/csrc/cfm_sample.h
--- a/tts-indic-server-f5_amd/csrc/cfm_sample.h
+++ b/tts-indic-server-f5_amd/csrc/cfm_sample.h
@@ -210,7 +210,7 @@
     hipLaunchKernelGGL(split_rows_kernel, dim3(m->M), dim3(256), 0, st, m->xstate, mel, mel, m->M, m->d_row_frame, m->xs.hi, m->xs.lo, 128, 0);
     CKL("split x");
     CK(precompute_text_and_ce(m, a.cond_dev, st));
-    CK(precompute_time(m, P.pts.data(), (int)P.pts.size(), st));
+    CK(precompute_time(m, P.pts.data(), (int)P.pts.size(), st, a.last == nullptr));
 
     m->d_row_tp = T.row_tp;
     int n_act = n;
diff --git a/tts-indic-server-f5_amd/csrc/elementwise.h b/tts-indic-server-f5_amd/csrc/elementwise.h
--- a/tts-indic-server-f5_amd/csrc/elementwise.h
+++ b/tts-indic-server-f5_amd/csrc/elementwise.h
@@ -26,25 +26,36 @@
 
 __global__ __launch_bounds__(256) void grn_stats_kernel(const float* y, int ldy, int C, const int* seq_row0,
                                                         const int* seq_len, float* gx ) {
-    const int seq = blockIdx.y, c = blockIdx.x * 256 + threadIdx.x;
-    if (c >= C) return;
-    const int r0 = seq_row0[seq], n = seq_len[seq];
-    float a8[8] = {0.f, 0.f, 0.f, 0.f, 0.f, 0.f, 0.f, 0.f};
-    const float* col = y + (size_t)r0 * ldy + c;
-    int r = 0;
-    for (; r + 8 <= n; r += 8) {
-        float t[8];
+    __shared__ float part[8][32];
+    const int seq = blockIdx.y, cl = threadIdx.x & 31, u = threadIdx.x >> 5, c = blockIdx.x * 32 + cl;
+    const int r0 = seq_row0[seq], n = seq_len[seq], n8 = n & ~7;
+    float a = 0.f;
+    if (c < C) {
+        const float* col = y + (size_t)r0 * ldy + c;
+        int r = u;
+        for (; r + 56 < n8; r += 64) {
+            float t[8];
 #pragma unroll
-        for (int u = 0; u < 8; u++) t[u] = col[(size_t)(r + u) * ldy];
+            for (int i = 0; i < 8; i++) t[i] = col[(size_t)(r + 8 * i) * ldy];
 #pragma unroll
-        for (int u = 0; u < 8; u++) a8[u] += t[u] * t[u];
-    }
-    for (; r < n; r++) {
-        const float t = col[(size_t)r * ldy];
-        a8[0] += t * t;
-    }
-    const float acc = ((a8[0] + a8[1]) + (a8[2] + a8[3])) + ((a8[4] + a8[5]) + (a8[6] + a8[7]));
-    gx[(size_t)seq * C + c] = sqrtf(acc);
+            for (int i = 0; i < 8; i++) a = __builtin_fmaf(t[i], t[i], a);
+        }
+        for (; r < n8; r += 8) {
+            const float t = col[(size_t)r * ldy];
+            a = __builtin_fmaf(t, t, a);
+        }
+        if (u == 0)
+            for (r = n8; r < n; r++) {
+                const float t = col[(size_t)r * ldy];
+                a = __builtin_fmaf(t, t, a);
+            }
+    }
+    part[u][cl] = a;
+    __syncthreads();
+    if (u == 0 && c < C) {
+        const float acc = ((part[0][cl] + part[1][cl]) + (part[2][cl] + part[3][cl])) + ((part[4][cl] + part[5][cl]) + (part[6][cl] + part[7][cl]));
+        gx[(size_t)seq * C + c] = sqrtf(acc);
+    }
 }
 
 __global__ __launch_bounds__(256) void grn_apply_kernel(const float* y, int ldy, int C, int M, const int* row_seq,
diff --git a/tts-indic-server-f5_amd/csrc/f5hip.hip b/tts-indic-server-f5_amd/csrc/f5hip.hip
--- a/tts-indic-server-f5_amd/csrc/f5hip.hip
+++ b/tts-indic-server-f5_amd/csrc/f5hip.hip
@@ -78,6 +78,7 @@
     int *d_j_row0 = nullptr, *d_j_len = nullptr, *d_j_kvlen = nullptr, *d_j_kv_row0 = nullptr, *d_j_kv2_row0 = nullptr, *d_j_kv2_len = nullptr;
     bool any_masked = false;
     std::vector<int> h_seq_len;
+    std::vector<float> time_key;
 };
 
 static int ceil_to(int v, int m) { return (v + m - 1) / m * m; }
@@ -353,7 +354,8 @@
             for (auto& sb : m->skipbuf) sb = a.plane2(R * 2 * D);
             m->qk = a.bf16((R + 256) * 2 * D); m->vt = a.bf16((size_t)D * R);
             m->rk_k2 = a.f32(U * c.mel_dim); m->rk_k3 = a.f32(U * c.mel_dim);
-        })) { m->cap_rows = 0; return -5; }
+        })) { m->cap_rows = 0; m->time_key.clear(); return -5; }
+    m->time_key.clear();
     m->cap_rows = (int)R; m->cap_frames = (int)U; m->cap_seq = (int)S;
     const int need = (int)MetaLayout(R, S, U, m->arch == 2).total;
     if (need > m->meta_cap) {
@@ -485,9 +487,19 @@
        CNT_WAVE_FLAC_REQUESTS, CNT_WAVE_LOUDNESS_LAUNCHES, CNT_WAVE_LOUDNESS_REQUESTS, CNT_FLAC_DECODE_LAUNCHES, CNT_FLAC_DECODE_STREAMS,
        CNT_REF_PRESTEP_LAUNCHES, CNT_REF_PRESTEP_CLIPS, CNT_WAVE_PROSODY_LAUNCHES, CNT_WAVE_PROSODY_REQUESTS,
        CNT_REF_DENOISE_LAUNCHES, CNT_REF_DENOISE_CLIPS, CNT_WAVE_MARK_LAUNCHES, CNT_WAVE_MARK_REQUESTS, CNT_WATERMARK_DETECT_LAUNCHES,
-       CNT_WATERMARK_DETECT_CLIPS, CNT_REF_ASSESS_LAUNCHES, CNT_REF_ASSESS_CLIPS, CNT_COUNT };
+       CNT_WATERMARK_DETECT_CLIPS, CNT_REF_ASSESS_LAUNCHES, CNT_REF_ASSESS_CLIPS, CNT_GEMM3_THIN, CNT_TIME_TABLE_BUILDS, CNT_COUNT };
 static long long g_counters[CNT_COUNT] = {};
 
+static constexpr long long kThinMaxWorkgroups = 256;
+static int g_thin_force = -1;
+static hipError_t launch_gemm3_generic_or_thin(int prec, int epi, int bn, const GemmArgs& a, int mp, int np, hipStream_t st) {
+    const long long thin_wgs = (long long)((a.M + 31) / 32) * (np / 128);
+    const bool thin = epi == EPI_GENERIC && bn == 128 && (g_thin_force >= 0 ? g_thin_force != 0 : thin_wgs <= kThinMaxWorkgroups);
+    g_counters[CNT_GEMM3]++;
+    if (!thin) return f5_launch_gemm3(prec, epi, bn, a, mp, np, st);
+    g_counters[CNT_GEMM3_THIN]++;
+    return f5_launch_gemm3_thin(prec, a, np, st);
+}
 static int run_gemm_n(int nsplit, int mp, GemmArgs& a, const PackedW& W, int epi, bool conv, int bn, hipStream_t st) {
     hipError_t e;
     const int np = W.n_pad;
@@ -511,12 +523,10 @@
         } else {
             const bool wide = tiles128 >= 1024 && np % 256 == 0;
             if (wide) g_counters[CNT_GEMM3_WIDE]++;
-            g_counters[CNT_GEMM3]++;
-            e = f5_launch_gemm3(3, epi, wide ? 256 : 128, a, mp, np, st);
+            e = launch_gemm3_generic_or_thin(3, epi, wide ? 256 : 128, a, mp, np, st);
         }
     } else if (!conv && tiles128 <= 256 && epi != EPI_QKV) {
-        g_counters[CNT_GEMM3]++;
-        e = f5_launch_gemm3(nsplit, epi, 128, a, mp, np, st);
+        e = launch_gemm3_generic_or_thin(nsplit, epi, 128, a, mp, np, st);
     } else {
         g_counters[bn == 64 ? CNT_GEMM_REG_BN64 : CNT_GEMM_REG_BN128]++;
         e = f5_launch_gemm_reg(nsplit, bn, conv, epi, a, mp, np, st);
@@ -579,7 +589,7 @@
                                            "flac_decode_launches", "flac_decode_streams", "ref_prestep_launches", "ref_prestep_clips",
                                            "wave_prosody_launches", "wave_prosody_requests", "ref_denoise_launches", "ref_denoise_clips",
                                            "wave_mark_launches", "wave_mark_requests", "watermark_detect_launches", "watermark_detect_clips",
-                                           "ref_assess_launches", "ref_assess_clips"};
+                                           "ref_assess_launches", "ref_assess_clips", "gemm3_thin", "time_table_builds"};
     static const char* attn_names[F5_ATTN_CNT_COUNT] = {"attn_bal8", "attn_nw8_deep", "attn_nw8", "attn_nw6_deep", "attn_nw6", "attn_nw4", "attn_seg2"};
     long long* attn = f5_attn_counters();
     if (!name) return fail(-1, "get_counter: null name");
@@ -606,7 +616,7 @@
     g1.act = ACT_GELU_ERF; g1.out_f32 = ty; g1.ldo = 2 * Td;
     CK(run_gemm_n(b.pw1.f16 ? 3 : nsplit, M, g1, b.pw1, EPI_GENERIC, false, 128, st));
     prof_begin(PROF_OTHER, st);
-    hipLaunchKernelGGL(grn_stats_kernel, dim3((2 * Td + 255) / 256, n_seq), dim3(256), 0, st, ty, 2 * Td, 2 * Td, seq_row0, seq_len, gx);
+    hipLaunchKernelGGL(grn_stats_kernel, dim3((2 * Td + 31) / 32, n_seq), dim3(256), 0, st, ty, 2 * Td, 2 * Td, seq_row0, seq_len, gx);
     CKL("grn_stats");
     hipLaunchKernelGGL(grn_apply_kernel, dim3((M + 3) / 4), dim3(256), 0, st, ty, 2 * Td, 2 * Td, M, row_seq, gx, b.gamma, b.beta, tg.hi, tg.lo,
                        2 * Td);
@@ -653,10 +663,13 @@
     return 0;
 }
 
-static int precompute_time(f5hip_dit* m, const float* t_host, int n_t, hipStream_t st) {
+static int precompute_time(f5hip_dit* m, const float* t_host, int n_t, hipStream_t st, bool reuse = false) {
     const f5hip_dit_config& c = m->cfg;
     const int D = c.dim;
     if (n_t > kMaxTimePoints) return fail(-8, "at most %d time points per call (got %d)", kMaxTimePoints, n_t);
+    if (reuse && n_t > 0 && (int)m->time_key.size() == n_t && !memcmp(m->time_key.data(), t_host, sizeof(float) * n_t)) return 0;
+    m->time_key.clear();
+    g_counters[CNT_TIME_TABLE_BUILDS]++;
     const int t_pad = ceil_to(n_t, 128);
     std::vector<uint16_t> hi((size_t)t_pad * 256, 0), lo((size_t)t_pad * 256, 0);
     const float emb = logf(10000.0f) / (float)(128 - 1);
@@ -687,6 +700,7 @@
         g3.out_f32 = m->mod + (size_t)t0 * m->n_adaln; g3.ldo = m->n_adaln;
         CK(run_gemm(m, g3, m->adaln, EPI_GENERIC, false, 128, st, 128));
     }
+    m->time_key.assign(t_host, t_host + n_t);
     return 0;
 }
 
diff --git a/tts-indic-server-f5_amd/csrc/gemm3.h b/tts-indic-server-f5_amd/csrc/gemm3.h
--- a/tts-indic-server-f5_amd/csrc/gemm3.h
+++ b/tts-indic-server-f5_amd/csrc/gemm3.h
@@ -110,6 +110,119 @@
     gemm_epilogue8_consumer<EPI, TN>(p, acc, reinterpret_cast<float*>(smem) + wave * (64 * 32 * TN), m0 + wm * 64, n0 + wn * (32 * TN), n0, lane);
 }
 
+template <int NSPLIT>
+__global__ __launch_bounds__(512) __attribute__((amdgpu_waves_per_eu(2, 2))) void gemm3_thin_kernel(const GemmArgs p) {
+    constexpr int NPL = NSPLIT == 2 ? 2 : 1;
+    constexpr bool F16 = NSPLIT == 3;
+    constexpr int BM = 32, BN = 128, NST = 4;
+    constexpr int A_PLANE = BM * 64, B_PLANE = BN * 64, STAGE = NPL * (A_PLANE + B_PLANE);
+    constexpr int PIECES = STAGE / 1024, P = (PIECES + 3) / 4;
+    extern __shared__ __attribute__((aligned(16))) char smem[];
+
+    const int tid = threadIdx.x, lane = tid & 63;
+    const int wave = __builtin_amdgcn_readfirstlane(tid >> 6);
+    const int m0 = blockIdx.y * BM, n0 = blockIdx.x * BN;
+    const int nk = p.K >> 5;
+
+    if (wave >= 4) {
+        const int pw = wave - 4;
+        const char* gsrc[P];
+        int ldst[P];
+#pragma unroll
+        for (int j = 0; j < P; j++) {
+            const int off = ((pw * P + j) % PIECES) * 1024;
+            const bool isA = off < NPL * A_PLANE;
+            const int rel = isA ? off : off - NPL * A_PLANE;
+            const int plane_bytes = isA ? A_PLANE : B_PLANE;
+            const int pl = rel / plane_bytes;
+            const int row = (rel - pl * plane_bytes) / 64 + (lane >> 2);
+            const int chunk = (lane & 3) ^ ((row >> 2) & 3);
+            const __bf16* ap = (NPL == 2 && pl) ? p.A[1] : p.A[0];
+            const __bf16* wp = (NPL == 2 && pl) ? p.W[1] : p.W[0];
+            const __bf16* base = isA ? ap + (size_t)(m0 + row) * p.lda : wp + (size_t)(n0 + row) * p.ldw;
+            gsrc[j] = reinterpret_cast<const char*>(base + chunk * 8);
+            ldst[j] = off;
+        }
+        auto issue_tile = [&](int kt) {
+            char* dst = smem + (kt % NST) * STAGE;
+#pragma unroll
+            for (int j = 0; j < P; j++)
+                __builtin_amdgcn_global_load_lds((const __attribute__((address_space(1))) void*)(gsrc[j] + (size_t)kt * 64),
+                                                 (__attribute__((address_space(3))) void*)(dst + ldst[j]), 16, 0, 0);
+        };
+#pragma unroll
+        for (int t = 0; t < NST - 1; t++)
+            if (t < nk) issue_tile(t);
+        for (int kt = 0; kt < nk; kt++) {
+            const int newer = min(NST - 2, nk - 1 - kt);
+            if (newer >= 2) wait_vmcnt<2 * P>();
+            else if (newer == 1) wait_vmcnt<P>();
+            else wait_vmcnt<0>();
+            __builtin_amdgcn_s_barrier();
+            if (kt + NST - 1 < nk) issue_tile(kt + NST - 1);
+        }
+        __syncthreads();
+        __syncthreads();
+        return;
+    }
+
+    const int fr = lane & 31, fh = lane >> 5;
+    f32x16 acc;
+#pragma unroll
+    for (int g = 0; g < 16; g++) acc[g] = 0.0f;
+
+    bf16x8 fa[2][NPL], fb[2][NPL];
+    auto read_frags = [&](int buf, const char* st, int s) {
+        const int chunk = s * 2 + fh;
+#pragma unroll
+        for (int pl = 0; pl < NPL; pl++) {
+            fa[buf][pl] = *reinterpret_cast<const bf16x8*>(st + pl * A_PLANE + lds_off2(fr, chunk));
+            fb[buf][pl] = *reinterpret_cast<const bf16x8*>(st + NPL * A_PLANE + pl * B_PLANE + lds_off2(wave * 32 + fr, chunk));
+        }
+    };
+    auto mfma_frags = [&](int buf) {
+        if (NSPLIT == 2) {
+            acc = __builtin_amdgcn_mfma_f32_32x32x16_bf16(fa[buf][1], fb[buf][0], acc, 0, 0, 0);
+            acc = __builtin_amdgcn_mfma_f32_32x32x16_bf16(fa[buf][0], fb[buf][1], acc, 0, 0, 0);
+        }
+        acc = mfma_32x32x16<F16>(fa[buf][0], fb[buf][0], acc);
+    };
+    __builtin_amdgcn_s_barrier();
+    read_frags(0, smem, 0);
+    for (int kt = 0; kt < nk; kt++) {
+        const char* st = smem + (kt % NST) * STAGE;
+        read_frags(1, st, 1);
+        __builtin_amdgcn_sched_barrier(0);
+        mfma_frags(0);
+        __builtin_amdgcn_sched_barrier(0);
+        if (kt + 1 < nk) {
+            asm volatile("s_waitcnt lgkmcnt(0)" ::: "memory");
+            __builtin_amdgcn_s_barrier();
+            read_frags(0, smem + ((kt + 1) % NST) * STAGE, 0);
+            __builtin_amdgcn_sched_barrier(0);
+        }
+        mfma_frags(1);
+        __builtin_amdgcn_sched_barrier(0);
+    }
+    float* slab = reinterpret_cast<float*>(smem) + (wave >> 1) * (32 * 64);
+    __syncthreads();
+#pragma unroll
+    for (int g = 0; g < 16; g++) slab[((g & 3) + 8 * (g >> 2) + 4 * fh) * 64 + (wave & 1) * 32 + fr] = acc[g];
+    __syncthreads();
+    if (wave < 2) gemm_epilogue_rows32<EPI_GENERIC, 64>(p, reinterpret_cast<const float*>(smem) + wave * (32 * 64), m0, n0 + wave * 64, lane);
+}
+
+template <int NSPLIT>
+static hipError_t launch_gemm3_thin_t(const GemmArgs& a, int n_pad, hipStream_t st) {
+    constexpr int NPL = NSPLIT == 2 ? 2 : 1;
+    constexpr int LDS = 4 * NPL * (32 + 128) * 64;
+    static unsigned attr_mask = 0;
+    if (hipError_t e = f5_set_lds_attr(reinterpret_cast<const void*>(&gemm3_thin_kernel<NSPLIT>), LDS, attr_mask); e != hipSuccess) return e;
+    dim3 grid(n_pad / 128, (a.M + 31) / 32);
+    hipLaunchKernelGGL((gemm3_thin_kernel<NSPLIT>), grid, dim3(512), LDS, st, a);
+    return hipGetLastError();
+}
+
 template <int NSPLIT, int EPI, int BN = 128>
 static hipError_t launch_gemm3_t(const GemmArgs& a, int m_pad, int n_pad, hipStream_t st) {
     constexpr int NPL = NSPLIT == 2 ? 2 : 1;
diff --git a/tts-indic-server-f5_amd/csrc/gemm_launch.h b/tts-indic-server-f5_amd/csrc/gemm_launch.h
--- a/tts-indic-server-f5_amd/csrc/gemm_launch.h
+++ b/tts-indic-server-f5_amd/csrc/gemm_launch.h
@@ -6,6 +6,7 @@
 
 hipError_t f5_launch_gemm_reg(int prec, int bn, bool conv, int epi, const GemmArgs& a, int m_pad, int n_pad, hipStream_t st);
 hipError_t f5_launch_gemm3(int prec, int epi, int bn, const GemmArgs& a, int m_pad, int n_pad, hipStream_t st);
+hipError_t f5_launch_gemm3_thin(int prec, const GemmArgs& a, int n_pad, hipStream_t st);
 hipError_t f5_launch_gemm5_generic(const GemmArgs& a, int rb, int cb, int n_pad, hipStream_t st);
 hipError_t f5_launch_gemm5_qkv(const GemmArgs& a, int rb, int cb, int n_pad, hipStream_t st);
 hipError_t f5_launch_gemm5_rowmul(const GemmArgs& a, int rb, int cb, int n_pad, hipStream_t st);
diff --git a/tts-indic-server-f5_amd/csrc/tu_gemm3.hip b/tts-indic-server-f5_amd/csrc/tu_gemm3.hip
--- a/tts-indic-server-f5_amd/csrc/tu_gemm3.hip
+++ b/tts-indic-server-f5_amd/csrc/tu_gemm3.hip
@@ -17,3 +17,9 @@
     if (prec == 2) return qkv ? launch_gemm3_t<2, EPI_QKV>(a, m_pad, n_pad, st) : launch_gemm3_t<2, EPI_GENERIC>(a, m_pad, n_pad, st);
     return qkv ? launch_gemm3_t<1, EPI_QKV>(a, m_pad, n_pad, st) : launch_gemm3_t<1, EPI_GENERIC>(a, m_pad, n_pad, st);
 }
+
+hipError_t f5_launch_gemm3_thin(int prec, const GemmArgs& a, int n_pad, hipStream_t st) {
+    if (prec == 3) return launch_gemm3_thin_t<3>(a, n_pad, st);
+    if (prec == 2) return launch_gemm3_thin_t<2>(a, n_pad, st);
+    return launch_gemm3_thin_t<1>(a, n_pad, st);
+}
diff --git a/tts-indic-server-f5_amd/csrc/unit_ops.h b/tts-indic-server-f5_amd/csrc/unit_ops.h
--- a/tts-indic-server-f5_amd/csrc/unit_ops.h
+++ b/tts-indic-server-f5_amd/csrc/unit_ops.h
@@ -119,6 +119,10 @@
     const int M_pad = (M + 127) / 128 * 128, N_pad = (N + 127) / 128 * 128;
     const bool f16 = prec == 3;
     if (w_copies < 1) w_copies = 1;
+    struct ThinForce {
+        ThinForce() { const char* e = getenv("F5HIP_GEMM3_THIN"); g_thin_force = e && *e ? (atoi(e) != 0) : -1; }
+        ~ThinForce() { g_thin_force = -1; }
+    } thin_force;
     OpBufs b;
     Plane2 A;
     A.hi = b.get<__bf16>((size_t)M_pad * K); A.lo = b.get<__bf16>((size_t)M_pad * K);
@@ -748,8 +752,8 @@
     return rc;
 }
 
-extern "C" int f5hip_op_convnext_block(int32_t n_seq, const int32_t* seq_len, int32_t Td, const float* x_dev, const float* const* params_host,
-                                       int32_t pad_nan, float* out_dev, float* tap_ln_dev, float* tap_ty_dev, float* tap_grn_dev, void* stream) {
+static int op_convnext_block_run(int32_t n_seq, const int32_t* seq_len, int32_t Td, const float* x_dev, const float* const* params_host, int32_t pad_nan,
+                                 float* out_dev, float* tap_ln_dev, float* tap_ty_dev, float* tap_grn_dev, float* tap_gx_dev, void* stream) {
     if (n_seq <= 0 || !seq_len || Td <= 0 || Td % 32 || Td > 1536 || !x_dev || !params_host || !out_dev) return fail(-1, "op_convnext_block: bad argument");
     for (int i = 0; i < 10; i++) if (!params_host[i]) return fail(-1, "op_convnext_block: parameter %d is null", i);
     hipStream_t st = (hipStream_t)stream;
@@ -781,12 +785,22 @@
         if (tap_ty_dev) hipLaunchKernelGGL(gather_rows_kernel, dim3(L.frames), dim3(128), 0, st, ty, 2 * Td, 2 * Td, L.frames, L.frame_row, tap_ty_dev, 2 * Td);
         if (tap_grn_dev) hipLaunchKernelGGL(op_gather_planes_kernel, dim3(L.frames), dim3(256), 0, st, tg.hi, tg.lo, 2 * Td, 2 * Td, L.frames, L.frame_row,
                                             tap_grn_dev);
+        if (tap_gx_dev) (void)hipMemcpyAsync(tap_gx_dev, gx, sizeof(float) * (size_t)n_seq * 2 * Td, hipMemcpyDeviceToDevice, st);
         if (hipGetLastError() != hipSuccess) rc = fail(-7, "op_convnext_block: gather launch");
     }
     if (hipStreamSynchronize(st) != hipSuccess && !rc) rc = fail(-7, "op_convnext_block: %s", hipGetErrorString(hipGetLastError()));
     for (float* p : {tb.dw_w, tb.dw_b, tb.ln_w, tb.ln_b, tb.gamma, tb.beta}) dev_free(p);
     free_packed(tb.pw1); free_packed(tb.pw2);
     return rc;
+}
+extern "C" int f5hip_op_convnext_block(int32_t n_seq, const int32_t* seq_len, int32_t Td, const float* x_dev, const float* const* params_host,
+                                       int32_t pad_nan, float* out_dev, float* tap_ln_dev, float* tap_ty_dev, float* tap_grn_dev, void* stream) {
+    return op_convnext_block_run(n_seq, seq_len, Td, x_dev, params_host, pad_nan, out_dev, tap_ln_dev, tap_ty_dev, tap_grn_dev, nullptr, stream);
+}
+extern "C" int f5hip_op_convnext_block_gx(int32_t n_seq, const int32_t* seq_len, int32_t Td, const float* x_dev, const float* const* params_host,
+                                          int32_t pad_nan, float* out_dev, float* tap_ln_dev, float* tap_ty_dev, float* tap_grn_dev,
+                                          float* tap_gx_dev, void* stream) {
+    return op_convnext_block_run(n_seq, seq_len, Td, x_dev, params_host, pad_nan, out_dev, tap_ln_dev, tap_ty_dev, tap_grn_dev, tap_gx_dev, stream);
 }
 
 static int op_cfg_launch(const char* name, CfgBufs cb, int U, int rows, const int32_t* urow_c_host, const int32_t* urow_u_host, float cfg, int op,
diff --git a/tts-indic-server-f5_amd/ops.py b/tts-indic-server-f5_amd/ops.py
--- a/tts-indic-server-f5_amd/ops.py
+++ b/tts-indic-server-f5_amd/ops.py
@@ -257,9 +257,10 @@
     arr = (C.c_void_p * 10)(*(a.ctypes.data for a in hp))
     out = torch.empty(n, Td, dtype=torch.float32, device=dev)
     tp = {"ln": torch.empty(n, Td, dtype=torch.float32, device=dev), "ty": torch.empty(n, 2 * Td, dtype=torch.float32, device=dev),
-          "grn": torch.empty(n, 2 * Td, dtype=torch.float32, device=dev)} if taps else {}
-    _lib.check(_lib.lib().f5hip_op_convnext_block(len(sl), _p(sl), Td, _p(x), arr, int(pad_nan), _p(out), _p(tp.get("ln")), _p(tp.get("ty")),
-                                                  _p(tp.get("grn")), _lib.current_stream_ptr()), "f5hip_op_convnext_block")
+          "grn": torch.empty(n, 2 * Td, dtype=torch.float32, device=dev),
+          "gx": torch.empty(len(sl), 2 * Td, dtype=torch.float32, device=dev)} if taps else {}
+    _lib.check(_lib.lib().f5hip_op_convnext_block_gx(len(sl), _p(sl), Td, _p(x), arr, int(pad_nan), _p(out), _p(tp.get("ln")), _p(tp.get("ty")),
+                                                     _p(tp.get("grn")), _p(tp.get("gx")), _lib.current_stream_ptr()), "f5hip_op_convnext_block_gx")
     return (out, tp) if taps else out
 
 
```

Measured after the change: 10430 (median of 6 runs). No clear change (+1.0%).
